# niveathika/siddhi

Hardware: AMD Instinct MI355X
Metric: events/sec ingested + matches/sec (partitioned pattern, 1–8 GPU); % HBM peak (higher is better)
Workload: dtype f64; 1 GPU; P3; events_per_gpu=100000000, keys_per_gpu=10000000, micro_batch=50000896, call_size=1024, parallelism=key-sharded x1, input=prepartitioned

## Files before the change

siddhi_amd/csrc/engine.h:

```cpp
#pragma once
#include <algorithm>
#include <cstring>
#include <memory>
#include <vector>

#include "common.h"
#include "dev_expr.h"

namespace shd {

enum EngineKind { ENG_PATTERN = 1, ENG_WINDOW = 2, ENG_FILTER = 3, ENG_NFA = 4 };

struct OutputBuffer {
  int ncols = 0;
  int64_t count = 0, cap = 0;
  DevBuf chunk, type, ts, vals, nulls, seq, sidx;
  void init(int nc) { ncols = nc; }
  void ensure(int64_t extra, hipStream_t s);
  int64_t* d_chunk() { return chunk.as<int64_t>(); }
  int32_t* d_type() { return type.as<int32_t>(); }
  int64_t* d_ts() { return ts.as<int64_t>(); }
  uint64_t* d_vals() { return vals.as<uint64_t>(); }
  uint8_t* d_nulls() { return nulls.as<uint8_t>(); }
  int64_t* d_seq() { return seq.as<int64_t>(); }
  int32_t* d_sidx() { return sidx.as<int32_t>(); }
  DevBuf lvals, lnul;
  int64_t lcount = 0, lcap = 0;
  void ensure_list(int64_t extra, hipStream_t s);
};

struct Staged {
  int stream = 0;
  int64_t n = 0;
  ColSet cs{};
  std::vector<int64_t> call_offsets;
  bool advance_time = false;
  const uint8_t* skip_start = nullptr;
};

struct SnapW {
  std::vector<uint8_t> b;
  hipStream_t s = nullptr;
  template <class T> void put(const T& v) {
    const size_t o = b.size();
    b.resize(o + sizeof(T));
    std::memcpy(b.data() + o, &v, sizeof(T));
  }
  void bytes(const void* src, size_t n) {
    const size_t o = b.size();
    b.resize(o + n);
    if (n) std::memcpy(b.data() + o, src, n);
  }
  void dev(const void* p, size_t n) {
    put<uint64_t>(n);
    const size_t o = b.size();
    b.resize(o + n);
    if (n) {
      SHD_HIP(hipMemcpyAsync(b.data() + o, p, n, hipMemcpyDeviceToHost, s));
      SHD_HIP(hipStreamSynchronize(s));
    }
  }
};

struct SnapR {
  const uint8_t* p = nullptr;
  size_t n = 0, at = 0;
  hipStream_t s = nullptr;
  void need(size_t k) const {
    if (at + k > n) throw Error(SHD_E_ARG, "snapshot truncated or from a different plan");
  }
  template <class T> T get() {
    need(sizeof(T));
    T v;
    std::memcpy(&v, p + at, sizeof(T));
    at += sizeof(T);
    return v;
  }
  size_t dev(DevBuf& buf, size_t extra_cap = 0) {
    const size_t k = (size_t)get<uint64_t>();
    need(k);
    buf.reserve(std::max<size_t>(k, extra_cap));
    if (k) {
      SHD_HIP(hipMemcpyAsync(buf.p, p + at, k, hipMemcpyHostToDevice, s));
      SHD_HIP(hipStreamSynchronize(s));
    }
    at += k;
    return k;
  }
  void dev_into(void* dst, size_t expect) {
    const size_t k = (size_t)get<uint64_t>();
    if (k != expect) throw Error(SHD_E_ARG, "snapshot section size mismatch");
    need(k);
    if (k) {
      SHD_HIP(hipMemcpyAsync(dst, p + at, k, hipMemcpyHostToDevice, s));
      SHD_HIP(hipStreamSynchronize(s));
    }
    at += k;
  }
};

struct NeedNfa : Error {
  explicit NeedNfa(const std::string& m) : Error(SHD_E_UNSUPPORTED, m) {}
};

struct NeedDissolve : NeedNfa {
  explicit NeedDissolve(const std::string& m) : NeedNfa(m) {}
};

struct Replay {
  int stream = 0;
  int64_t n = 0;
  std::vector<int64_t> ts;
  std::vector<std::vector<uint8_t>> cols, nulls;
  std::vector<uint8_t> skip_start;
};

struct Engine {
  Plan plan;
  DevExprTable ex;
  hipStream_t stream = nullptr;
  OutputBuffer out;
  shd_counters counters{};
  int64_t seq = 0;
  int64_t now = INT64_MIN;
  int64_t chunk_seq = 0;
  hipEvent_t ev0 = nullptr, ev1 = nullptr;
  static constexpr int kMaxStages = 16;
  hipEvent_t sev[kMaxStages + 1] = {};
  const char* stage_name[kMaxStages] = {};
  int n_stages = 0;
  int64_t stage_ns[kMaxStages] = {};
  void stage_begin() { n_stages = 0; mark(nullptr); }
  void mark(const char* name_of_finished_stage);
  void stage_end();

  virtual ~Engine();
  virtual int kind() const = 0;
  virtual void push(const Staged& b) = 0;
  virtual void set_time(int64_t t) {
    if (t >= now) now = t;
  }
  virtual void reset() = 0;
  int64_t start_time = 0;
  int64_t layout_hint = 0;
  virtual void set_option(const std::string& key, int64_t v) {
    if (key == "start_time") {
      start_time = v;
      if (v > now) now = v;
      return;
    }
    throw Error(SHD_E_ARG, "unknown option '" + key + "' for this query");
  }
  virtual void on_loaded() {}
  virtual void save_state(SnapW&) { throw Error(SHD_E_UNSUPPORTED, "engine has no snapshot support"); }
  virtual void load_state(SnapR&) { throw Error(SHD_E_UNSUPPORTED, "engine has no snapshot support"); }
  virtual void export_replay(std::vector<Replay>&) {
    throw Error(SHD_E_UNSUPPORTED, "engine state cannot be handed over");
  }
  bool grouped = false;
  virtual void group_attach(const std::vector<Engine*>&) {
    throw Error(SHD_E_UNSUPPORTED, "this query's engine cannot lead a query group");
  }
  virtual void group_detach() {}
  virtual void group_dissolve() { throw Error(SHD_E_UNSUPPORTED, "this group cannot dissolve"); }

  static constexpr size_t kArgArena = size_t(1) << 20;
  DevBuf arg_dev;
  PinnedBuf arg_host;
  size_t arg_used = 0;
  void args_begin() {
    if (!arg_dev.p) {
      arg_dev.reserve(kArgArena);
      arg_host.reserve(kArgArena);
    }
    SHD_HIP(hipStreamSynchronize(stream));
    arg_used = 0;
  }
  template <class T> const T* dev_args(const T& a) {
    size_t off = (arg_used + 255) & ~size_t(255);
    if (!arg_dev.p || off + sizeof(T) > kArgArena) throw Error(SHD_E_CAPACITY, "kernel argument arena exhausted");
    std::memcpy(arg_host.as<char>() + off, &a, sizeof(T));
    SHD_HIP(hipMemcpyAsync(arg_dev.as<char>() + off, arg_host.as<char>() + off, sizeof(T), hipMemcpyHostToDevice,
                           stream));
    arg_used = off + sizeof(T);
    return reinterpret_cast<const T*>(arg_dev.as<char>() + off);
  }

  template <class... P, class... A>
  void launch_grid(void (*kernel)(P...), unsigned grid, A&&... args) {
    kernel<<<dim3(grid), dim3(kBlock), 0, stream>>>(std::forward<A>(args)...);
    SHD_CHECK_LAUNCH();
  }
  template <class... P, class... A>
  void launch(void (*kernel)(P...), int64_t n, A&&... args) {
    launch_grid(kernel, grid_cover(n), std::forward<A>(args)...);
  }

  uint32_t read_u32(const void* dev, uint32_t* pinned) {
    SHD_HIP(hipMemcpyAsync(pinned, dev, 4, hipMemcpyDeviceToHost, stream));
    SHD_HIP(hipStreamSynchronize(stream));
    return *pinned;
  }
  uint32_t scan(const uint32_t* in, uint32_t* outp, int64_t n, uint32_t* total_dev, uint32_t* total_pinned,
                DevBuf& scratch) {
    if (n <= 0) return 0;
    scan_exclusive_u32(in, outp, n, total_dev, scratch, stream);
    return read_u32(total_dev, total_pinned);
  }

  DExpr dexpr(int e) const { return DExpr{ex.off[e], ex.len[e]}; }
  DExprSet dset() const { return DExprSet{ex.ins.as<int4>(), ex.consts.as<uint64_t>(), ex.nins, ex.nconsts}; }
  DFilters dfilters(const std::vector<int>& ids) const;
  bool fast_atom(int expr_id, FAtom& out) const;
};

std::unique_ptr<Engine> make_pattern_engine(const Plan& p, std::string& why);
std::unique_ptr<Engine> make_logical_pattern_engine(const Plan& p, std::string& why);
std::unique_ptr<Engine> make_absent_engine(const Plan& p, std::string& why);
std::unique_ptr<Engine> make_single_engine(const Plan& p, std::string& why);
std::unique_ptr<Engine> make_window_x_engine(const Plan& p, std::string& why);
std::unique_ptr<Engine> make_nfa_engine(const Plan& p, std::string& why);
std::unique_ptr<Engine> make_nfa_engine(const Plan& p, std::string& why, int64_t list_hint);
void init_engine(Engine& e, const Plan& p);

}
```

siddhi_amd/csrc/engine_pattern.hip:

```cpp
#include <algorithm>
#include <unordered_map>
#include <cmath>
#include <cstdio>
#include <cstdlib>
#include <type_traits>

#include "engine.h"
#include "knobs.h"
#include "pattern_common.h"

namespace shd {

using namespace pat;

namespace {

template <bool FAST>
__global__ __launch_bounds__(kBlock) void k_prepare(const PrepArgs* __restrict__ ap, int64_t n_ext, int64_t stride,
                                                    uint32_t* __restrict__ k32, uint64_t* __restrict__ k64,
                                                    uint32_t* __restrict__ pv, int32_t* __restrict__ tso,
                                                    PrepAgg* __restrict__ blk) {
  const PrepArgs& a = *ap;
  const DExprSet es = a.es;
  PrepAcc acc;
  const int64_t tbase = a.x.batch.ts[0];
  for (int64_t r = (int64_t)blockIdx.x * kBlock + threadIdx.x; r < n_ext; r += stride) {
    uint64_t k;
    uint32_t f;
    int32_t t32;
    prep_row<FAST>(a, es, r, tbase, true, k, f, t32, acc);
    if (a.partitioned) {
      if (a.key64) k64[r] = k;
      else k32[r] = (uint32_t)k;
    }
    pv[r] = (f << kRowBits) | (uint32_t)r;
    tso[r] = t32;
  }
  prep_block_reduce<kBlock>(acc, blk, blockIdx.x);
}

__global__ __launch_bounds__(kBlock) void k_finish_prep(const PrepAgg* blk, int nblk, PrepAgg* out) {
  unsigned long long c = 0, km = 0, ov = 0, um = 0, kn = ULLONG_MAX;
  long long tmin = LLONG_MAX, tmax = LLONG_MIN, ctm = LLONG_MIN;
#pragma unroll 8
  for (int b = threadIdx.x; b < nblk; b += kBlock) {
    ov |= blk[b].ovf;
    um |= blk[b].unmono;
    kn = blk[b].kmin < kn ? blk[b].kmin : kn;
    ctm = blk[b].carry_tmax > ctm ? blk[b].carry_tmax : ctm;
    c += blk[b].n_cand;
    km = blk[b].kmax > km ? blk[b].kmax : km;
    tmin = blk[b].ts_min < tmin ? blk[b].ts_min : tmin;
    tmax = blk[b].ts_max > tmax ? blk[b].ts_max : tmax;
  }
  for (int o = 32; o > 0; o >>= 1) {
    c += __shfl_xor(c, o, 64);
    ov |= __shfl_xor(ov, o, 64);
    um |= __shfl_xor(um, o, 64);
  }
  km = wave_max(km);
  kn = wave_min(kn);
  tmin = wave_min(tmin);
  tmax = wave_max(tmax);
  ctm = wave_max(ctm);
  __shared__ PrepAgg wpart[kBlock / 64];
  if ((threadIdx.x & 63) == 0) wpart[threadIdx.x >> 6] = PrepAgg{c, km, tmin, tmax, ov, um, ctm, kn};
  __syncthreads();
  if (threadIdx.x == 0) {
    PrepAgg r = wpart[0];
    for (int w = 1; w < kBlock / 64; w++) {
      r.ovf |= wpart[w].ovf;
      r.unmono |= wpart[w].unmono;
      r.carry_tmax = wpart[w].carry_tmax > r.carry_tmax ? wpart[w].carry_tmax : r.carry_tmax;
      r.kmin = wpart[w].kmin < r.kmin ? wpart[w].kmin : r.kmin;
      r.n_cand += wpart[w].n_cand;
      r.kmax = wpart[w].kmax > r.kmax ? wpart[w].kmax : r.kmax;
      r.ts_min = wpart[w].ts_min < r.ts_min ? wpart[w].ts_min : r.ts_min;
      r.ts_max = wpart[w].ts_max > r.ts_max ? wpart[w].ts_max : r.ts_max;
    }
    *out = r;
  }
}

__global__ void k_narrow_keys(const uint64_t* in, uint32_t* out, int64_t n) {
  for (int64_t i = (int64_t)blockIdx.x * blockDim.x + threadIdx.x; i < n; i += (int64_t)gridDim.x * blockDim.x)
    out[i] = (uint32_t)in[i];
}

__global__ __launch_bounds__(kBlock) void k_sorted_ts64(const ExtRows* __restrict__ xp,
                                                        const uint32_t* __restrict__ spv, int64_t n,
                                                        int64_t* __restrict__ sts64) {
  const ExtRows& x = *xp;
  for (int64_t p = (int64_t)blockIdx.x * kBlock + threadIdx.x; p < n; p = n) sts64[p] = x.ts(pv_row(spv[p]));
}

__global__ __launch_bounds__(kBlock) void k_slice_coarsen(const ExtRows* __restrict__ xp,
                                                          const int64_t* __restrict__ slice_t, int64_t nslice,
                                                          int cbits, int32_t* __restrict__ ctab) {
  const int64_t tbase = xp->batch.ts[0];
  const int e = (int)blockIdx.x * kBlock + threadIdx.x;
  if (e >= kScanCoarse) return;
  const int64_t per = (int64_t)1 << (cbits - kKsSliceBits);
  const int64_t s0 = e * per, s1 = s0 + per < nslice ? s0 + per : nslice;
  int64_t lo = LLONG_MAX, hi = LLONG_MIN;
  for (int64_t i = s0; i < s1; i++) {
    const int64_t l = slice_t[i], h = slice_t[nslice + i];
    lo = l < lo ? l : lo;
    hi = h > hi ? h : hi;
  }
  ctab[e] = lo == LLONG_MAX ? INT32_MAX : (int32_t)(lo - tbase);
  ctab[kScanCoarse + e] = hi == LLONG_MIN ? INT32_MIN : (int32_t)(hi - tbase);
}

__global__ __launch_bounds__(kBlock) void k_sorted_ts32(const ExtRows* __restrict__ xp,
                                                        const uint32_t* __restrict__ spv, int64_t n,
                                                        int32_t* __restrict__ sts32) {
  const ExtRows& x = *xp;
  const int64_t tbase = x.batch.ts[0];
  for (int64_t p = (int64_t)blockIdx.x * kBlock + threadIdx.x; p < n; p = n)
    sts32[p] = (int32_t)(x.ts(pv_row(spv[p])) - tbase);
}

#include "pattern_walk.h"

__device__ __forceinline__ void scan_block_reduce(uint64_t steps, uint64_t pruned, uint32_t viol, uint32_t nm,
                                                  uint32_t no, ScanOut* blk, int slot, uint32_t* bcnt, int tile,
                                                  int ntile, bool add, uint32_t nd = 0) {
  for (int o2 = 32; o2 > 0; o2 >>= 1) {
    steps += __shfl_xor(steps, o2, 64);
    pruned += __shfl_xor(pruned, o2, 64);
    viol |= __shfl_xor(viol, o2, 64);
    nm += __shfl_xor(nm, o2, 64);
    no += __shfl_xor(no, o2, 64);
    nd += __shfl_xor(nd, o2, 64);
  }
  __shared__ ScanOut wpart[kBlock / 64];
  __shared__ uint32_t wcnt[3][kBlock / 64];
  if ((threadIdx.x & 63) == 0) {
    wpart[threadIdx.x >> 6] = ScanOut{steps, pruned, viol};
    wcnt[0][threadIdx.x >> 6] = nm;
    wcnt[1][threadIdx.x >> 6] = no;
    wcnt[2][threadIdx.x >> 6] = nd;
  }
  __syncthreads();
  if (threadIdx.x == 0) {
    ScanOut r = wpart[0];
    uint32_t tm = wcnt[0][0], to = wcnt[1][0], td = wcnt[2][0];
    for (int w = 1; w < kBlock / 64; w++) {
      r.steps += wpart[w].steps;
      r.pruned += wpart[w].pruned;
      r.violation |= wpart[w].violation;
      tm += wcnt[0][w];
      to += wcnt[1][w];
      td += wcnt[2][w];
    }
    blk[slot] = r;
    if (add) {
      if (tm) atomicAdd(&bcnt[tile], tm);
      if (to) atomicAdd(&bcnt[ntile + tile], to);
    } else {
      bcnt[tile] = tm;
      bcnt[ntile + tile] = to;
      bcnt[2 * ntile + tile] = td;
    }
  }
}

__device__ __forceinline__ void and_carried(const ScanArgs& a, int64_t r, uint32_t& fm, int64_t& ra, int64_t& rb) {
  fm = 0;
  ra = rb = -1;
  if (r < a.x.C) {
    fm = a.carry_half[r];
    const int64_t hr = a.x.C + a.x.batch.n + r;
    if (fm & 1u) ra = hr;
    if (fm & 2u) rb = hr;
  }
}
__device__ __forceinline__ int32_t and_code(uint32_t fm, int64_t ra, int64_t rb) {
  return fm == 0 ? 0 : (int32_t)((fm & 1u ? ra : rb) | ((int64_t)fm << kRowBits));
}
__device__ __forceinline__ int32_t and_open_code(const ScanArgs& a, int64_t r) {
  uint32_t fm;
  int64_t ra, rb;
  and_carried(a, r, fm, ra, rb);
  return and_code(fm, ra, rb);
}

template <bool K64, bool TS64, bool HASH>
__global__ __launch_bounds__(kBlock) void k_forward_scan(const ScanArgs* __restrict__ ap, int64_t n_ext,
                                                         int64_t tile, const uint32_t* __restrict__ skey32,
                                                         const uint64_t* __restrict__ skey64,
                                                         const uint32_t* __restrict__ spv,
                                                         const int32_t* __restrict__ sts32,
                                                         const int64_t* __restrict__ sts64,
                                                         int32_t* __restrict__ match_row, uint8_t* __restrict__ pst,
                                                         uint32_t* __restrict__ bcnt, ScanOut* __restrict__ blk) {
  const ScanArgs& a = *ap;
  const DExprSet es{};
  uint64_t steps = 0, pruned = 0;
  uint32_t viol = 0, nm = 0, no = 0, nd = 0;
  const int64_t t0 = (int64_t)blockIdx.x * tile;
  const int64_t t1 = t0 + tile < n_ext ? t0 + tile : n_ext;
  const int64_t tbase = TS64 ? 0 : a.x.batch.ts[0];
  auto visit = [&](int64_t p, const auto& ld) {
    uint32_t pvp, pq;
    int64_t tsi, tq;
    uint64_t k = 0, kq = 0;
    const int64_t q0 = p + 1 < n_ext ? p + 1 : n_ext - 1;
    ld(p, pvp, tsi, k);
    ld(q0, pq, tq, kq);
    uint8_t out = PS_NONE;
    if (pv_flags(pvp) & F_CAND) {
      int64_t q = p + 1;
      int32_t j = -1;
      uint32_t fm = 0;
      int64_t ra = -1, rb = -1;
      const uint8_t st = walk_partial<true, false, HASH ? 4 : 1>(a, es, n_ext, ld, pv_row(pvp), k, tsi, q, pq, tq,
                                                                 kq, tsi, false, j, steps, viol, fm, ra, rb);
      if (st == ST_DEFER) {
        out = PS_DEFER;
        match_row[p] = (int32_t)q;
        nd++;
      } else if (st == ST_OPEN) {
        out = PS_OPEN;
        no++;
        if (a.logical == 2) match_row[p] = and_open_code(a, pv_row(pvp));
      } else if (st == ST_PRUNED) {
        pruned++;
      }
    }
    pst[p] = out;
  };
  const GlobalPos<K64, TS64> ld{skey32, skey64, spv, sts32, sts64, tbase, a.partitioned};
  for (int64_t p = t0 + threadIdx.x; p < t1; p += kBlock) visit(p, ld);
  scan_block_reduce(steps, pruned, viol, nm, no, blk, blockIdx.x, bcnt, blockIdx.x, gridDim.x, false, nd);
}

constexpr int kSubPerTile = kBlock / 64;
constexpr uint32_t kRecDeferred = 0x80000000u;

constexpr int kRecRing = 128;
__device__ __forceinline__ void wave_lds_order() {
  __builtin_amdgcn_fence(__ATOMIC_RELEASE, "wavefront");
  __builtin_amdgcn_wave_barrier();
  __builtin_amdgcn_fence(__ATOMIC_ACQUIRE, "wavefront");
}
template <bool LEAN>
__global__ __launch_bounds__(kBlock) void k_forward_scan_rec(const ScanArgs* __restrict__ ap, int64_t n_ext,
                                                             int64_t tile, const uint32_t* __restrict__ skey32,
                                                             const uint32_t* __restrict__ spv,
                                                             const int32_t* __restrict__ sts32,
                                                             int32_t* __restrict__ match_row, uint8_t* __restrict__ pst,
                                                             uint32_t* __restrict__ bcnt, ScanOut* __restrict__ blk,
                                                             uint32_t* __restrict__ rkey, uint32_t* __restrict__ rpv,
                                                             int32_t* __restrict__ rts, uint32_t* __restrict__ rpos,
                                                             uint32_t* __restrict__ dlist, uint32_t* __restrict__ scnt) {
  const ScanArgs& a = *ap;
  const DExprSet es{};
  uint64_t steps = 0, pruned = 0;
  uint32_t viol = 0, no = 0, nd = 0;
  const int lane = threadIdx.x & 63, w = threadIdx.x >> 6;
  const int64_t sub = tile / kSubPerTile;
  const int64_t t0 = (int64_t)blockIdx.x * tile;
  const int64_t t1 = t0 + tile < n_ext ? t0 + tile : n_ext;
  const int64_t s0 = t0 + (int64_t)w * sub;
  const int64_t s1 = s0 + sub < t1 ? s0 + sub : t1;
  const int64_t tbase = a.x.batch.ts[0];
  const GlobalPos<false, false> ld{skey32, nullptr, spv, sts32, nullptr, tbase, a.partitioned};
  const RowPos ldr{skey32, spv, a.x.carry.ts, a.x.batch.ts, a.x.C, a.partitioned};
  __shared__ int32_t ctab[LEAN ? 2 * kScanCoarse : 1];
  if constexpr (LEAN) {
    const int nc = (int)((n_ext - 1) >> a.cbits) + 1;
    for (int i = threadIdx.x; i < nc; i += kBlock) {
      ctab[i] = a.ctab[i];
      ctab[kScanCoarse + i] = a.ctab[kScanCoarse + i];
    }
    __syncthreads();
  }
  constexpr int kRecPos = LEAN ? 2 : 3;
  const uint64_t below = ((uint64_t)1 << lane) - 1;
  uint32_t wrec = 0, wdef = 0;
  uint32_t wout = 0;
  __shared__ uint32_t ring[kSubPerTile][LEAN ? 3 : 4][kRecRing];
  uint32_t (*rg)[kRecRing] = ring[w];
  auto flush = [&](uint32_t cnt) {
    wave_lds_order();
    if ((uint32_t)lane < cnt) {
      const uint32_t sl = (wout + (uint32_t)lane) & (kRecRing - 1);
      const int64_t o = s0 + wout + lane;
      rkey[o] = rg[0][sl];
      rpv[o] = rg[1][sl];
      if constexpr (!LEAN) rts[o] = (int32_t)rg[2][sl];
      rpos[o] = rg[kRecPos][sl];
    }
    wave_lds_order();
  };
  for (int64_t c = s0; c < s1; c += 64) {
    const int64_t p = c + lane;
    uint8_t out = PS_NONE;
    uint32_t pvp = 0;
    int64_t tsi = 0;
    uint64_t k = 0;
    if (p < s1) {
      uint32_t pq;
      int64_t tq;
      uint64_t kq = 0;
      const int64_t q0 = p + 1 < n_ext ? p + 1 : n_ext - 1;
      if constexpr (LEAN) {
        pvp = spv[p];
        pq = spv[q0];
        k = skey32[p];
        kq = skey32[q0];
      } else {
        ld(p, pvp, tsi, k);
        ld(q0, pq, tq, kq);
      }
      if (pv_flags(pvp) & F_CAND) {
        int64_t q = p + 1;
        int32_t j = -1;
        uint32_t fm = 0;
        int64_t ra = -1, rb = -1;
        uint8_t st;
        if constexpr (LEAN) {
          const uint32_t fq = pv_flags(pq);
          const int64_t ri = pv_row(pvp), rq = pv_row(pq);
          if (q >= n_ext || (kq != k && !(fq & F_SKIP))) {
            st = ST_OPEN;
          } else {
            bool dead = false;
            if (kq == k && (fq & F_NEW) && !(fq & F_SKIP)) {
              const int64_t hi = ri >= a.x.C ? tbase + ctab[kScanCoarse + (ri >> a.cbits)] : a.carry_tmax;
              const int64_t lo = tbase + ctab[rq >> a.cbits];
              dead = lo > hi && (uint64_t)lo - (uint64_t)hi > (uint64_t)a.within;
            }
            if (dead) {
              st = ST_DEAD;
              steps++;
            } else {
              tsi = ldr.row_ts(ri);
              tq = ldr.row_ts(rq);
              st = walk_partial<true, false, 1>(a, es, n_ext, ldr, ri, k, tsi, q, pq, tq, kq, tsi, false, j, steps,
                                                viol, fm, ra, rb);
            }
          }
        } else {
          st = walk_partial<true, false, 1>(a, es, n_ext, ld, pv_row(pvp), k, tsi, q, pq, tq, kq, tsi, false, j, steps,
                                            viol, fm, ra, rb);
        }
        if (st == ST_DEFER) {
          out = PS_DEFER;
          match_row[p] = (int32_t)q;
          nd++;
        } else if (st == ST_OPEN) {
          out = PS_OPEN;
          no++;
        } else if (st == ST_PRUNED) {
          pruned++;
        }
      }
      pst[p] = out;
    }
    const bool def = out == PS_DEFER, rec = def || out == PS_OPEN;
    const uint64_t mrec = __ballot(rec), mdef = __ballot(def);
    if (rec) {
      const uint32_t sl = (wrec + (uint32_t)__popcll(mrec & below)) & (kRecRing - 1);
      rg[0][sl] = (uint32_t)k;
      rg[1][sl] = pvp;
      if constexpr (!LEAN) rg[2][sl] = (uint32_t)(int32_t)(tsi - tbase);
      rg[kRecPos][sl] = (uint32_t)p | (def ? kRecDeferred : 0u);
    }
    if (def) dlist[s0 + wdef + __popcll(mdef & below)] = (uint32_t)p;
    wrec += (uint32_t)__popcll(mrec);
    wdef += (uint32_t)__popcll(mdef);
    if (wrec - wout >= 64) {
      flush(64);
      wout += 64;
    }
  }
  if (wrec > wout) flush(wrec - wout);
  if (lane == 0) {
    const int64_t nsub = (int64_t)gridDim.x * kSubPerTile;
    const int64_t st = (int64_t)blockIdx.x * kSubPerTile + w;
    scnt[st] = wrec - wdef;
    scnt[nsub + st] = wdef;
    scnt[2 * nsub + st] = wrec;
  }
  scan_block_reduce(steps, pruned, viol, 0u, no, blk, blockIdx.x, bcnt, blockIdx.x, gridDim.x, false, nd);
}

__global__ __launch_bounds__(kBlock) void k_gather_bpos(const ExtRows* __restrict__ xp, const uint32_t* spv,
                                                       int64_t n_ext) {
  const ExtRows& x = *xp;
  for (int64_t p = (int64_t)blockIdx.x * kBlock + threadIdx.x; p < n_ext; p += (int64_t)gridDim.x * kBlock) {
    const int64_t r = pv_row(spv[p]);
    const uint32_t m = r < x.C ? x.apos_mask : (x.bpos_mask | x.apos_mask);
    for (int c = 0; c < x.batch.ncols; c++) {
      if (!((m >> c) & 1u)) continue;
      const Val v = r < x.C ? col_load(x.carry, r, c) : col_load(x.batch, r - x.C, c);
      switch (x.bpos.type[c]) {
        case SHD_T_STRING: case SHD_T_INT: case SHD_T_FLOAT: ((uint32_t*)x.bpos.col[c])[p] = (uint32_t)v.b; break;
        case SHD_T_LONG: case SHD_T_DOUBLE: ((uint64_t*)x.bpos.col[c])[p] = v.b; break;
        case SHD_T_BOOL: ((uint8_t*)x.bpos.col[c])[p] = (uint8_t)v.b; break;
      }
      ((uint8_t*)x.bpos.nul[c])[p] = (uint8_t)v.null;
    }
  }
}

__global__ __launch_bounds__(kBlock) void k_block_sum(const ScanArgs* __restrict__ ap, int64_t n_ext,
                                                     const uint32_t* __restrict__ skey32,
                                                     const uint32_t* __restrict__ spv,
                                                     const int32_t* __restrict__ sts32, BlockSum* __restrict__ out) {
  const ScanArgs& a = *ap;
  const ExtRows& x = a.x;
  const int lane = threadIdx.x & 63;
  const int64_t nblk = (n_ext + 63) >> 6;
  const int64_t tbase = x.batch.ts[0];
  const int attr = a.bs_attr;
  const bool usemax = a.bs_op == SHD_OP_GT || a.bs_op == SHD_OP_GE;
  for (int64_t b = ((int64_t)blockIdx.x * kBlock + threadIdx.x) >> 6; b < nblk;
       b += ((int64_t)gridDim.x * kBlock) >> 6) {
    const int64_t p = (b << 6) + lane;
    const bool valid = p < n_ext;
    const uint32_t pv = valid ? spv[p] : 0u;
    const int64_t t = valid ? tbase + (int64_t)sts32[p] : 0;
    const uint32_t key = (valid && a.partitioned) ? skey32[p] : 0u;
    const uint32_t f = pv_flags(pv);
    const bool keyed = valid && !(f & F_SKIP);
    const bool nw = keyed && (f & F_NEW);
    double dv = usemax ? -__builtin_inf() : __builtin_inf();
    if (nw && (f & F_B)) {
      const int64_t r = pv_row(pv);
      const Val v = ((x.bpos_mask >> attr) & 1u) ? col_load(x.bpos, p, attr)
                    : (r < x.C ? col_load(x.carry, r, attr) : col_load(x.batch, r - x.C, attr));
      if (!v.null) {
        const double d = v_f64(v.b);
        if (d == d) dv = d;
      }
    }
    dv = usemax ? wave_max(dv) : wave_min(dv);
    const uint64_t km = __ballot(keyed), nm = __ballot(nw);
    const uint32_t k0 = km ? __shfl(key, __ffsll((unsigned long long)km) - 1, 64) : 0u;
    const bool uniform = __ballot(keyed && key != k0) == 0;
    int64_t m = nw ? t : INT64_MIN;
#pragma unroll
    for (int o = 1; o < 64; o <<= 1) {
      const int64_t u = __shfl_up(m, o, 64);
      if (lane >= o) m = u > m ? u : m;
    }
    int64_t before = __shfl_up(m, 1, 64);
    if (lane == 0) before = INT64_MIN;
    const bool mono = __ballot(nw && t < before) == 0;
    const int64_t tfirst = nm ? __shfl(t, __ffsll((unsigned long long)nm) - 1, 64) : 0;
    const int64_t tlast = __shfl(m, 63, 64);
    if (lane == 0) {
      BlockSum o;
      o.key = k0;
      o.cnt = (uint16_t)__popcll(nm);
      o.flags = (uint8_t)((uniform ? 1u : 0u) | (mono ? 2u : 0u) | (km ? 0u : 4u));
      o.pad = 0;
      o.tfirst = tfirst;
      o.tlast = tlast;
      o.v = dv;
      o.newmask = nm;
      out[b] = o;
    }
  }
}

static bool block_skip_term(const FPred& fp, int s2, int& ci, int& side, int& op, int& attr) {
  auto is_e2 = [&](const FTerm& t) {
    return t.aop == 0 && t.a.kind == FA_LOAD && t.a.st == s2 && (t.a.idx == 0 || t.a.idx == SHD_IDX_CURRENT) &&
           t.a.cvt_to < 0;
  };
  auto no_e2 = [&](const FTerm& t) {
    auto ok = [&](const FAtom& x) { return x.kind != FA_LOAD || x.st == 0; };
    return ok(t.a) && (t.aop == 0 || ok(t.b));
  };
  auto flip = [](int o) {
    return o == SHD_OP_GT ? SHD_OP_LT : o == SHD_OP_LT ? SHD_OP_GT : o == SHD_OP_GE ? SHD_OP_LE : SHD_OP_GE;
  };
  for (int i = 0; i < fp.n && i < 4; i++) {
    const FCmp& c = fp.c[i];
    if (c.type != SHD_T_DOUBLE) continue;
    if (c.op != SHD_OP_GT && c.op != SHD_OP_GE && c.op != SHD_OP_LT && c.op != SHD_OP_LE) continue;
    if (is_e2(c.l) && no_e2(c.r)) {
      ci = i, side = 0, op = c.op, attr = c.l.a.attr;
      return true;
    }
    if (is_e2(c.r) && no_e2(c.l)) {
      ci = i, side = 1, op = flip(c.op), attr = c.r.a.attr;
      return true;
    }
  }
  return false;
}

static bool split_f2(const FPred& fp, int s2, const ExtRows& x, F2Split& sp) {
  sp = F2Split{};
  if (!fp.ok || fp.n > kSplitMax) return false;
  auto e2dep = [&](const FAtom& t) { return t.kind == FA_LOAD && t.st == s2; };
  auto dep = [&](const FTerm& t) { return e2dep(t.a) || (t.aop != 0 && e2dep(t.b)); };
  for (int i = 0; i < fp.n; i++) {
    const FCmp& c = fp.c[i];
    SplitCmp& o = sp.c[i];
    o.op = c.op;
    o.type = c.type;
    const bool dl = dep(c.l), dr = dep(c.r);
    if (!dl && !dr) {
      o.konst = 1;
      continue;
    }
    if (dl && dr) return false;
    const FTerm& e = dl ? c.l : c.r;
    if (e.aop != 0 || (e.a.idx != 0 && e.a.idx != SHD_IDX_CURRENT)) return false;
    const int attr = e.a.attr;
    if (attr < 0 || attr >= x.batch.ncols || attr >= kMaxCols) return false;
    o.swap = dr ? 1 : 0;
    o.pos = (x.bpos_mask >> attr) & 1u;
    const ColSet& cs = o.pos ? x.bpos : x.batch;
    o.col = cs.col[attr];
    o.nul = cs.nul[attr];
    o.ctype = cs.type[attr];
    o.cvt_from = e.a.cvt_from;
    o.cvt_to = e.a.cvt_to;
    const bool cvt = o.cvt_to >= 0 && o.cvt_to != o.cvt_from;
    const bool rel = c.op == SHD_OP_EQ || c.op == SHD_OP_NE || c.op == SHD_OP_GT || c.op == SHD_OP_GE ||
                     c.op == SHD_OP_LT || c.op == SHD_OP_LE;
    o.kind = SK_GENERIC;
    if (rel && c.type == SHD_T_DOUBLE && o.ctype == SHD_T_FLOAT && cvt && o.cvt_from == SHD_T_FLOAT &&
        o.cvt_to == SHD_T_DOUBLE)
      o.kind = SK_F32_F64;
    else if (rel && c.type == SHD_T_DOUBLE && o.ctype == SHD_T_DOUBLE && !cvt)
      o.kind = SK_F64;
    else if ((c.op == SHD_OP_EQ || c.op == SHD_OP_NE) && c.type == SHD_T_STRING && o.ctype == SHD_T_STRING && !cvt)
      o.kind = SK_STR_EQ;
    else if (rel && c.type == SHD_T_INT && o.ctype == SHD_T_INT && !cvt)
      o.kind = SK_I32;
    if (o.kind != SK_GENERIC && o.swap) {
      switch (c.op) {
        case SHD_OP_GT: o.op = SHD_OP_LT; break;
        case SHD_OP_GE: o.op = SHD_OP_LE; break;
        case SHD_OP_LT: o.op = SHD_OP_GT; break;
        case SHD_OP_LE: o.op = SHD_OP_GE; break;
      }
    }
  }
  sp.n = fp.n;
  sp.ok = 1;
  return true;
}

template <bool FAST, bool SKIP, class Ld>
__device__ __forceinline__ void coop_resume(const ScanArgs& a, const DExprSet& es, int64_t n_ext, const Ld& ld,
                                            int64_t p, bool cont, int32_t* __restrict__ match_row,
                                            int32_t* __restrict__ match_other, uint8_t* __restrict__ pst,
                                            uint64_t& steps, uint64_t& pruned,
                                            uint32_t& viol, uint32_t& nm, uint32_t& no) {
  const int lane = threadIdx.x & 63;
  uint32_t pvp, pd;
  int64_t tsi, td;
  uint64_t k = 0, kd = 0;
  ld(p, pvp, tsi, k);
  int64_t q0 = match_row[p];
  ld(cont ? q0 - 1 : q0, pd, td, kd);
  const int64_t r = pv_row(pvp);
  int64_t prev = td;
  if (cont && (!(pv_flags(pd) & F_NEW) || (pv_flags(pd) & F_SKIP) || (a.partitioned && kd != k))) prev = tsi;
  bool first = !cont;
  uint8_t st = ST_OPEN;
  int32_t j = -1;
  uint32_t fm = 0;
  int64_t ra = -1, rb = -1;
  int32_t other = -1;
  if (a.logical == 2) and_carried(a, r, fm, ra, rb);
  SplitThr sth;
  if (FAST && a.sp.ok && !a.logical) sth = split_prep(a, r, p);
  uint64_t wsteps = 0;
  bool wviol = false;
  bool thr_ok = false;
  Val thr;
  thr.b = 0;
  thr.null = 1;
  while (q0 < n_ext) {
    if (SKIP && !first && (q0 & 63) == 0 && q0 + 64 <= n_ext) {
      if (!thr_ok) {
        thr = skip_threshold(a, r, p);
        thr_ok = true;
      }
      const BlockSum bs = a.bsum[q0 >> 6];
      if (block_skippable(a, bs, k, tsi, prev, thr)) {
        wsteps += bs.cnt;
        if (bs.cnt) prev = bs.tlast;
        q0 += 64;
        continue;
      }
    }
    const int64_t qend = SKIP ? ((q0 | 63) + 1) : q0 + 64;
    const int64_t q = q0 + lane;
    const bool act = q < qend;
    const bool inb = act && q < n_ext;
    uint32_t pq = 0;
    int64_t tq = 0;
    uint64_t kq = 0;
    if (inb) ld(q, pq, tq, kq);
    const uint32_t fq = pv_flags(pq);
    const bool f0 = first && lane == 0;
    const bool skip = (fq & F_SKIP) != 0;
    const bool endkey = inb && !f0 && a.partitioned && kq != k && !skip;
    const bool isnew = inb && !f0 && !endkey && (fq & F_NEW) && !skip;
    int64_t m = isnew ? tq : INT64_MIN;
#pragma unroll
    for (int o = 1; o < 64; o <<= 1) {
      const int64_t t = __shfl_up(m, o, 64);
      if (lane >= o) m = t > m ? t : m;
    }
    int64_t before = __shfl_up(m, 1, 64);
    if (lane == 0) before = INT64_MIN;
    before = before > prev ? before : prev;
    const bool vio = isnew && a.within != INT64_MAX && tq < before;
    const bool expire = isnew && !vio && tq - tsi > a.within;
    const uint64_t stopm = __ballot(act && (!inb || endkey || vio || expire));
    const int sidx = stopm ? __ffsll((unsigned long long)stopm) - 1 : 64;
    bool hit = false;
    int32_t code = 0;
    if (a.logical == 2) {
      const bool cand = lane < sidx && (f0 || (isnew && (fq & F_B)));
      const int64_t r2 = pv_row(pq);
      bool ha = false, hb = false;
      if (cand && !(fm & 1u)) {
        PairCtx cx{&a.x, r, r2, a.s_first};
        cx.q2 = q;
        cx.q1 = p;
        ha = FAST ? eval_fpred(a.f2.fp, cx) : eval_filters(es, a.f2, cx);
      }
      if (cand && !(fm & 2u)) {
        PairCtx cx{&a.x, r, r2, a.s_second};
        cx.q2 = q;
        cx.q1 = p;
        hb = FAST ? eval_fpred(a.f3.fp, cx) : eval_filters(es, a.f3, cx);
      }
      const uint64_t am = __ballot(ha), bm = __ballot(hb);
      int ia = (fm & 1u) ? -1 : (am ? __ffsll((unsigned long long)am) - 1 : 64);
      int ib = (fm & 2u) ? -1 : (bm ? __ffsll((unsigned long long)bm) - 1 : 64);
      if (ia >= 0 && ia < 64) {
        fm |= 1u;
        ra = __shfl(r2, ia, 64);
      }
      if (ib >= 0 && ib < 64) {
        fm |= 2u;
        rb = __shfl(r2, ib, 64);
      }
      const int term2 = fm == 3u ? (ia > ib ? ia : ib) : sidx;
      const uint64_t upto2 = term2 >= 63 ? ~0ull : ((2ull << term2) - 1ull);
      wsteps += (uint64_t)__popcll(__ballot(isnew && !vio) & upto2);
      if (fm == 3u) {
        const int br = ib >= ia ? 1 : 0;
        st = ST_MATCH;
        j = (int32_t)__shfl(r2, term2, 64) | (br << kRowBits);
        other = (int32_t)(br ? ra : rb);
        break;
      }
      if (sidx < 64) {
        const int kind = __shfl(vio ? 2 : (expire ? 1 : 0), sidx, 64);
        if (kind == 2) wviol = true;
        else if (kind == 1) st = ST_DEAD;
        break;
      }
      prev = __shfl(m, 63, 64) > prev ? __shfl(m, 63, 64) : prev;
      first = false;
      q0 = qend;
      continue;
    }
    if (lane < sidx && (f0 || (isnew && (fq & F_B)))) {
      const int64_t r2 = pv_row(pq);
      PairCtx cx{&a.x, r, r2, a.s_first};
      cx.q2 = q;
      cx.q1 = p;
      if (FAST && a.sp.ok && !a.logical) hit = split_eval(a.sp, sth, r2 - a.x.C, q);
      else hit = FAST ? eval_fpred(a.f2.fp, cx) : eval_filters(es, a.f2, cx);
      int32_t br = 0;
      if (!hit && a.logical) {
        cx.s2 = a.s_second;
        hit = FAST ? eval_fpred(a.f3.fp, cx) : eval_filters(es, a.f3, cx);
        br = 1;
      }
      code = (int32_t)r2 | (br << kRowBits);
    }
    const uint64_t hm = __ballot(hit);
    const int fidx = hm ? __ffsll((unsigned long long)hm) - 1 : 64;
    const int term = fidx < sidx ? fidx : sidx;
    const uint64_t upto = term >= 63 ? ~0ull : ((2ull << term) - 1ull);
    wsteps += (uint64_t)__popcll(__ballot(isnew && !vio) & upto);
    if (fidx < sidx) {
      st = ST_MATCH;
      j = __shfl(code, fidx, 64);
      break;
    }
    if (sidx < 64) {
      const int kind = __shfl(vio ? 2 : (expire ? 1 : 0), sidx, 64);
      if (kind == 2) wviol = true;
      else if (kind == 1) st = ST_DEAD;
      break;
    }
    prev = __shfl(m, 63, 64) > prev ? __shfl(m, 63, 64) : prev;
    first = false;
    q0 = qend;
  }
  if (st == ST_OPEN && a.prune && a.t_end - tsi > a.within) st = ST_PRUNED;
  if (lane == 0) {
    steps += wsteps;
    if (wviol) viol = 1;
    uint8_t out = PS_NONE;
    if (st == ST_MATCH) {
      out = PS_MATCH;
      match_row[p] = j;
      if (a.logical == 2) match_other[p] = other;
      nm++;
    } else if (st == ST_OPEN) {
      out = PS_OPEN | PS_PEND;
      no++;
      if (a.logical == 2) match_row[p] = and_code(fm, ra, rb);
    } else if (st == ST_PRUNED) {
      pruned++;
    }
    pst[p] = out;
  }
}

template <bool K64, bool FAST, bool TS64, int MODE, bool SKIP = false>
__global__ __launch_bounds__(kBlock) void k_forward_resume(const ScanArgs* __restrict__ ap, int64_t n_ext,
                                                           int64_t tile, const uint32_t* __restrict__ skey32,
                                                           const uint64_t* __restrict__ skey64,
                                                           const uint32_t* __restrict__ spv,
                                                           const int32_t* __restrict__ sts32,
                                                           const int64_t* __restrict__ sts64,
                                                           int32_t* __restrict__ match_row,
                                                           int32_t* __restrict__ match_other,
                                                           uint8_t* __restrict__ pst, uint32_t* __restrict__ bcnt,
                                                           ScanOut* __restrict__ blk, int slot0) {
  const ScanArgs& a = *ap;
  const DExprSet es = a.es;
  uint64_t steps = 0, pruned = 0;
  uint32_t viol = 0, nm = 0, no = 0;
  const int64_t t0 = (int64_t)blockIdx.x * tile;
  const int64_t t1 = t0 + tile < n_ext ? t0 + tile : n_ext;
  const int64_t tbase = TS64 ? 0 : a.x.batch.ts[0];
  const GlobalPos<K64, TS64> ld{skey32, skey64, spv, sts32, sts64, tbase, a.partitioned};
  auto resume_one = [&](int64_t p) {
      int64_t q = match_row[p];
      uint32_t pvp, pq;
      int64_t tsi, tq;
      uint64_t k = 0, kq = 0;
      ld(p, pvp, tsi, k);
      ld(q, pq, tq, kq);
      int32_t j = -1;
      uint32_t fm = 0;
      int64_t ra = -1, rb = -1;
      if (a.logical == 2) and_carried(a, pv_row(pvp), fm, ra, rb);
      const uint8_t st = walk_partial<false, FAST, 1, GlobalPos<K64, TS64>, 0, SKIP>(a, es, n_ext, ld, pv_row(pvp), k, tsi, q, pq, tq, kq, tq, true,
                                                      j, steps, viol, fm, ra, rb, p);
      uint8_t out = PS_NONE;
      if (st == ST_MATCH) {
        out = PS_MATCH;
        match_row[p] = j;
        if (a.logical == 2) match_other[p] = (int32_t)((j >> kRowBits) ? ra : rb);
        nm++;
      } else if (st == ST_OPEN) {
        out = PS_OPEN | PS_PEND;
        no++;
        if (a.logical == 2) match_row[p] = and_code(fm, ra, rb);
      } else if (st == ST_PRUNED) {
        pruned++;
      }
      pst[p] = out;
  };
  if constexpr (MODE == 2) {
    const int lane = threadIdx.x & 63, w = threadIdx.x >> 6;
    for (int64_t base = t0 + (int64_t)w * 64; base < t1; base += kBlock) {
      const int64_t pp = base + lane;
      const uint8_t o = pp < t1 ? pst[pp] : (uint8_t)PS_NONE;
      uint64_t dm = __ballot(o == PS_DEFER || o == PS_CONT);
      const uint64_t cm = __ballot(o == PS_CONT);
      while (dm) {
        const int b = __ffsll((unsigned long long)dm) - 1;
        dm &= dm - 1;
        coop_resume<FAST, SKIP>(a, es, n_ext, ld, base + b, (cm >> b) & 1ull, match_row, match_other, pst, steps, pruned,
                          viol, nm, no);
      }
    }
  } else if constexpr (MODE == 3) {
    for (int64_t p = t0 + threadIdx.x; p < t1; p += kBlock) {
      if (pst[p] != PS_DEFER) continue;
      int64_t q = match_row[p];
      uint32_t pvp, pq;
      int64_t tsi, tq;
      uint64_t k = 0, kq = 0;
      ld(p, pvp, tsi, k);
      ld(q, pq, tq, kq);
      int32_t j = -1;
      uint32_t fm = 0;
      int64_t ra = -1, rb = -1;
      const uint8_t st = walk_partial<false, FAST, 1, GlobalPos<K64, TS64>, 64, SKIP>(
          a, es, n_ext, ld, pv_row(pvp), k, tsi, q, pq, tq, kq, tq, true, j, steps, viol, fm, ra, rb, p);
      uint8_t out = PS_NONE;
      if (st == ST_MATCH) {
        out = PS_MATCH;
        match_row[p] = j;
        nm++;
      } else if (st == ST_OPEN) {
        out = PS_OPEN | PS_PEND;
        no++;
      } else if (st == ST_PRUNED) {
        pruned++;
      } else if (st == ST_YIELD) {
        out = PS_CONT;
        match_row[p] = (int32_t)q;
      }
      pst[p] = out;
    }
  } else if constexpr (MODE == 1) {
    for (int64_t p = t0 + threadIdx.x; p < t1; p += kBlock)
      if (pst[p] == PS_DEFER) resume_one(p);
  } else {
    for (int64_t c0 = t0; c0 < t1; c0 += kBlock * 16) {
      const int64_t pb = c0 + (int64_t)threadIdx.x * 16;
      if (pb >= t1) continue;
      const uint4 raw = *reinterpret_cast<const uint4*>(pst + pb);
      const uint32_t wv[4] = {raw.x, raw.y, raw.z, raw.w};
      uint32_t hit = 0;
#pragma unroll
      for (int i = 0; i < 16; i++)
        if (((wv[i >> 2] >> ((i & 3) * 8)) & 255u) == PS_DEFER && pb + i < t1) hit |= 1u << i;
      while (hit) {
        const int64_t p = pb + __ffs(hit) - 1;
        hit &= hit - 1;
        resume_one(p);
      }
    }
  }
  scan_block_reduce(steps, pruned, viol, nm, no, blk, slot0 + blockIdx.x, bcnt, blockIdx.x, gridDim.x, true);
}

template <bool K64, bool FAST, bool TS64, bool SUB = false, bool ROWT = false>
__global__ __launch_bounds__(kBlock) void k_resume_list(const ScanArgs* __restrict__ ap, int64_t n_ext, int64_t tile,
                                                        int ntile, const uint32_t* __restrict__ skey32,
                                                        const uint64_t* __restrict__ skey64,
                                                        const uint32_t* __restrict__ spv,
                                                        const int32_t* __restrict__ sts32,
                                                        const int64_t* __restrict__ sts64,
                                                        int32_t* __restrict__ match_row,
                                                        int32_t* __restrict__ match_other, uint8_t* __restrict__ pst,
                                                        uint32_t* __restrict__ bcnt, ScanOut* __restrict__ blk,
                                                        int slot0, const uint32_t* __restrict__ dlist,
                                                        const uint32_t* __restrict__ dcount,
                                                        const uint32_t* __restrict__ doff, int nsub, int64_t sub,
                                                        uint32_t* __restrict__ sopen) {
  const ScanArgs& a = *ap;
  const DExprSet es = a.es;
  uint64_t steps = 0, pruned = 0;
  uint32_t viol = 0;
  const int64_t tbase = (TS64 || ROWT) ? 0 : a.x.batch.ts[0];
  typedef typename std::conditional<ROWT, RowPos, GlobalPos<K64, TS64>>::type Ld;
  const Ld ld = [&] {
    if constexpr (ROWT) return RowPos{skey32, spv, a.x.carry.ts, a.x.batch.ts, a.x.C, a.partitioned};
    else return GlobalPos<K64, TS64>{skey32, skey64, spv, sts32, sts64, tbase, a.partitioned};
  }();
  const int64_t cnt = *dcount;
  for (int64_t i = (int64_t)blockIdx.x * kBlock + threadIdx.x; i < cnt; i += (int64_t)gridDim.x * kBlock) {
    int sti = 0;
    int64_t p;
    if (SUB) {
      int lo = 0, hi = nsub;
      while (lo < hi) {
        const int mid = (lo + hi) >> 1;
        if ((int64_t)doff[mid] <= i) lo = mid + 1; else hi = mid;
      }
      sti = lo - 1;
      p = dlist[(int64_t)sti * sub + (i - (int64_t)doff[sti])];
    } else {
      p = dlist[i];
    }
    int64_t q = match_row[p];
    uint32_t pvp, pq;
    int64_t tsi, tq;
    uint64_t k = 0, kq = 0;
    ld(p, pvp, tsi, k);
    ld(q, pq, tq, kq);
    int32_t j = -1;
    uint32_t fm = 0;
    int64_t ra = -1, rb = -1;
    if (a.logical == 2) and_carried(a, pv_row(pvp), fm, ra, rb);
    const uint8_t st = walk_partial<false, FAST, 1, Ld, 0, false>(
        a, es, n_ext, ld, pv_row(pvp), k, tsi, q, pq, tq, kq, tq, true, j, steps, viol, fm, ra, rb, p);
    uint8_t out = PS_NONE;
    const int t = (int)(p / tile);
    if (st == ST_MATCH) {
      out = PS_MATCH;
      match_row[p] = j;
      if (a.logical == 2) match_other[p] = (int32_t)((j >> kRowBits) ? ra : rb);
      atomicAdd(&bcnt[t], 1u);
    } else if (st == ST_OPEN) {
      out = PS_OPEN | PS_PEND;
      if (a.logical == 2) match_row[p] = and_code(fm, ra, rb);
      if (SUB) atomicAdd(&sopen[sti], 1u);
      else atomicAdd(&bcnt[ntile + t], 1u);
    } else if (st == ST_PRUNED) {
      pruned++;
    }
    pst[p] = out;
  }
  scan_block_reduce(steps, pruned, viol, 0u, 0u, blk, slot0 + blockIdx.x, bcnt, 0, ntile, true);
}

template <bool TS64>
__global__ __launch_bounds__(kBlock, 8) void k_lockstep_walk(const ScanArgs* __restrict__ ap, int64_t n_ext, int64_t tile,
                                                          const uint32_t* __restrict__ skey32,
                                                          const uint32_t* __restrict__ spv,
                                                          const int32_t* __restrict__ sts32,
                                                          const int64_t* __restrict__ sts64,
                                                          int32_t* __restrict__ match_row, uint8_t* __restrict__ pst,
                                                          uint32_t* __restrict__ bcnt, ScanOut* __restrict__ blk) {
  const ScanArgs& a = *ap;
  uint64_t steps = 0, pruned = 0;
  uint32_t viol = 0, nm = 0, no = 0;
  const int64_t t0 = (int64_t)blockIdx.x * tile;
  const int64_t t1 = t0 + tile < n_ext ? t0 + tile : n_ext;
  const int64_t tbase = TS64 ? 0 : a.x.batch.ts[0];
  const GlobalPos<false, TS64> ld{skey32, nullptr, spv, sts32, sts64, tbase, a.partitioned};
  for (int64_t p = t0 + threadIdx.x; p < t1; p += kBlock) {
    uint32_t pvp;
    int64_t tsi;
    uint64_t k = 0;
    ld(p, pvp, tsi, k);
    uint8_t out = PS_NONE;
    if (pv_flags(pvp) & F_CAND) {
      const int64_t r = pv_row(pvp);
      uint8_t st = ST_OPEN;
      bool metb = false;
      SplitThr sth;
      if (a.sp.ok) sth = split_prep(a, r, p);
      int32_t j = -1;
      int64_t prev = tsi;
      int64_t q = p + 1;
      uint32_t pn = 0;
      int64_t tn = 0;
      uint64_t kn = 0;
      if (q < n_ext) ld(q, pn, tn, kn);
      for (int d = 0; q < n_ext; q++, d++) {
        if (d >= 64 && metb) {
          st = ST_YIELD;
          break;
        }
        const uint32_t pq = pn;
        const int64_t tq = tn;
        const uint64_t kq = kn;
        if (q + 1 < n_ext) ld(q + 1, pn, tn, kn);
        const uint32_t fq = pv_flags(pq);
        if (fq & F_SKIP) continue;
        if (kq != k) break;
        if (!(fq & F_NEW)) continue;
        if (a.within != INT64_MAX && tq < prev) {
          viol = 1;
          break;
        }
        prev = tq;
        steps++;
        if (tq - tsi > a.within) {
          st = ST_DEAD;
          break;
        }
        if (fq & F_B) {
          bool hit;
          if (a.sp.ok) {
            hit = split_eval(a.sp, sth, (int64_t)pv_row(pq) - a.x.C, q);
          } else {
            PairCtx cx{&a.x, r, (int64_t)pv_row(pq), a.s_first};
            cx.q2 = q;
            cx.q1 = p;
            hit = eval_fpred(a.f2.fp, cx);
          }
          metb = true;
          if (hit) {
            st = ST_MATCH;
            j = (int32_t)pv_row(pq);
            break;
          }
        }
      }
      if (st == ST_OPEN && a.prune && a.t_end - tsi > a.within) st = ST_PRUNED;
      if (st == ST_MATCH) {
        out = PS_MATCH;
        match_row[p] = j;
        nm++;
      } else if (st == ST_OPEN) {
        out = metb ? (uint8_t)(PS_OPEN | PS_PEND) : (uint8_t)PS_OPEN;
        no++;
      } else if (st == ST_PRUNED) {
        pruned++;
      } else if (st == ST_YIELD) {
        out = PS_CONT;
        match_row[p] = (int32_t)q;
      }
    }
    pst[p] = out;
  }
  scan_block_reduce(steps, pruned, viol, nm, no, blk, blockIdx.x, bcnt, blockIdx.x, gridDim.x, false);
}

__global__ __launch_bounds__(kBlock) void k_tile_count(const uint8_t* __restrict__ pst, int64_t n, int64_t tile,
                                                       uint32_t* __restrict__ bcnt) {
  const int64_t t0 = (int64_t)blockIdx.x * tile;
  const int64_t t1 = t0 + tile < n ? t0 + tile : n;
  uint32_t nm = 0, no = 0;
  for (int64_t pb = t0 + (int64_t)threadIdx.x * 16; pb < t1; pb += kBlock * 16) {
    const uint4 raw = *reinterpret_cast<const uint4*>(pst + pb);
    const uint32_t wv[4] = {raw.x, raw.y, raw.z, raw.w};
#pragma unroll
    for (int i = 0; i < 16; i++) {
      const uint32_t o = (wv[i >> 2] >> ((i & 3) * 8)) & 255u;
      const bool in = pb + i < t1;
      nm += (in && o == PS_MATCH) ? 1u : 0u;
      no += (in && (o & 0x7Fu) == PS_OPEN) ? 1u : 0u;
    }
  }
  for (int o = 32; o > 0; o >>= 1) {
    nm += __shfl_xor(nm, o, 64);
    no += __shfl_xor(no, o, 64);
  }
  __shared__ uint32_t ws[2][kBlock / 64];
  if ((threadIdx.x & 63) == 0) {
    ws[0][threadIdx.x >> 6] = nm;
    ws[1][threadIdx.x >> 6] = no;
  }
  __syncthreads();
  if (threadIdx.x == 0) {
    uint32_t a = 0, b = 0;
    for (int k = 0; k < kBlock / 64; k++) {
      a += ws[0][k];
      b += ws[1][k];
    }
    bcnt[blockIdx.x] = a;
    bcnt[gridDim.x + blockIdx.x] = b;
  }
}

constexpr int kCompactPad = kBlock * 16;
template <class F>
__device__ __forceinline__ void tile_compact(const uint8_t* __restrict__ pst, int64_t t0, int64_t t1, uint8_t want,
                                             uint32_t base, F&& emit) {
  __shared__ uint32_t wsum[kBlock / 64];
  const int lane = threadIdx.x & 63, w = threadIdx.x >> 6;
  for (int64_t c0 = t0; c0 < t1; c0 += kBlock * 16) {
    const int64_t pb = c0 + (int64_t)threadIdx.x * 16;
    uint32_t wv[4] = {0u, 0u, 0u, 0u};
    if (pb < t1) {
      const uint4 raw = *reinterpret_cast<const uint4*>(pst + pb);
      wv[0] = raw.x;
      wv[1] = raw.y;
      wv[2] = raw.z;
      wv[3] = raw.w;
    }
    uint32_t hit = 0;
#pragma unroll
    for (int i = 0; i < 16; i++)
      if (((wv[i >> 2] >> ((i & 3) * 8)) & 127u) == want && pb + i < t1) hit |= 1u << i;
    const uint32_t cnt = (uint32_t)__popc(hit);
    uint32_t inc = cnt;
#pragma unroll
    for (int o = 1; o < 64; o <<= 1) {
      const uint32_t t = __shfl_up(inc, o, 64);
      if (lane >= o) inc += t;
    }
    if (lane == 63) wsum[w] = inc;
    __syncthreads();
    uint32_t pre = base + inc - cnt, tot = 0;
#pragma unroll
    for (int k = 0; k < kBlock / 64; k++) {
      if (k < w) pre += wsum[k];
      tot += wsum[k];
    }
    while (hit) {
      const int i = __ffs(hit) - 1;
      hit &= hit - 1;
      emit(pb + i, pre++);
    }
    base += tot;
    __syncthreads();
  }
}

__global__ __launch_bounds__(kBlock) void k_finish_scan(const ScanOut* blk, int nblk, ScanOut* out) {
  unsigned long long st = 0, pr = 0;
  uint32_t v = 0;
#pragma unroll 8
  for (int b = threadIdx.x; b < nblk; b += kBlock) {
    st += blk[b].steps;
    pr += blk[b].pruned;
    v |= blk[b].violation;
  }
  for (int o = 32; o > 0; o >>= 1) {
    st += __shfl_xor(st, o, 64);
    pr += __shfl_xor(pr, o, 64);
    v |= __shfl_xor(v, o, 64);
  }
  __shared__ ScanOut wpart[kBlock / 64];
  if ((threadIdx.x & 63) == 0) wpart[threadIdx.x >> 6] = ScanOut{st, pr, v};
  __syncthreads();
  if (threadIdx.x == 0) {
    ScanOut r = wpart[0];
    for (int w = 1; w < kBlock / 64; w++) {
      r.steps += wpart[w].steps;
      r.pruned += wpart[w].pruned;
      r.violation |= wpart[w].violation;
    }
    *out = r;
  }
}

__global__ __launch_bounds__(kBlock) void k_emit_pairs(const uint8_t* pst, const uint32_t* boff,
                                                       const int32_t* match_row, const uint32_t* spv, int64_t n,
                                                       int64_t tile, int logical, const int32_t* match_other,
                                                       uint32_t* pj, uint32_t* pi, uint32_t* se1, int32_t* sot) {
  const int64_t t0 = (int64_t)blockIdx.x * tile;
  const int64_t t1 = t0 + tile < n ? t0 + tile : n;
  tile_compact(pst, t0, t1, PS_MATCH, boff[blockIdx.x], [&](int64_t p, uint32_t o) {
    const uint32_t mr = (uint32_t)match_row[p];
    pj[o] = logical ? ((mr & kRowMask) << 1) | (mr >> kRowBits) : mr;
    if (logical == 2) {
      pi[o] = o;
      se1[o] = pv_row(spv[p]);
      sot[o] = match_other[p];
      return;
    }
    pi[o] = pv_row(spv[p]);
  });
}

struct ProjArgs {
  ExtRows x;
  DExprSet es;
  DExpr outs[kMaxCols];
  int nout;
  int multi;
  int logical;
  int s_first, s_second;
  const uint32_t* se1;
  const int32_t* sot;
  int64_t chunk0;
  int64_t row0;
  int fast;
  FAtom oat[kMaxCols];
};

__global__ __launch_bounds__(kBlock) void k_project(const ProjArgs* __restrict__ ap, const uint32_t* pj,
                                                    const uint32_t* pi, int64_t m, int64_t* o_chunk, int32_t* o_type,
                                                    int64_t* o_ts, uint64_t* o_vals, uint8_t* o_nul, int64_t* o_seq,
                                                    int32_t* o_sidx) {
  const ProjArgs& a = *ap;
  const DExprSet es = a.es;
  const ExtRows& x = a.x;
  for (int64_t k = (int64_t)blockIdx.x * kBlock + threadIdx.x; k < m; k = m) {
    int64_t j = pj[k], i = pi[k];
    int br = 0;
    if (a.logical) {
      br = (int)(j & 1);
      j >>= 1;
    }
    int64_t other = -1;
    if (a.logical == 2) {
      other = a.sot[i];
      i = a.se1[i];
    }
    PairCtx cx{&x, i, j, br ? a.s_second : a.s_first, true, other, br ? a.s_first : a.s_second};
    int64_t row = a.row0 + k;
    for (int c = 0; c < a.nout; c++) {
      const Val v = a.fast ? fp_atom(a.oat[c], cx) : eval_expr(es.ins + a.outs[c].off, a.outs[c].len, es.consts, cx);
      o_vals[row * a.nout + c] = v.b;
      o_nul[row * a.nout + c] = (uint8_t)v.null;
    }
    o_ts[row] = x.ts(j);
    o_type[row] = 0;
    o_seq[row] = x.seq(j);
    o_sidx[row] = br ? a.s_second : a.s_first;
    o_chunk[row] = a.logical ? 2 * x.seq(j) + br : (a.multi ? x.seq(j) : a.chunk0 + k);
  }
}

constexpr int kGroupMax = 64;
constexpr int kGroupWaveItems = 8;

struct GroupSelArgs {
  ExtRows x;
  int G;
  DExprSet es[kGroupMax];
  DFilters f1[kGroupMax];
};

__global__ __launch_bounds__(kBlock) void k_group_mask(const GroupSelArgs* __restrict__ ap, const uint32_t* pi,
                                                       int64_t m, uint64_t* __restrict__ mask) {
  const GroupSelArgs& a = *ap;
  for (int64_t k = (int64_t)blockIdx.x * kBlock + threadIdx.x; k < m; k = m) {
    PairCtx cx{&a.x, (int64_t)pi[k], -1, 1, false, -1, -1};
    uint64_t b = 0;
    for (int g = 0; g < a.G; g++)
      if (eval_filters(a.es[g], a.f1[g], cx)) b |= 1ull << g;
    mask[k] = b;
  }
}

template <bool SCATTER>
__global__ __launch_bounds__(kBlock) void k_group_split(const uint64_t* __restrict__ mask, const uint32_t* pj,
                                                        const uint32_t* pi, int64_t m, int G, int64_t nw,
                                                        uint32_t* __restrict__ cnt, uint32_t* __restrict__ gpj,
                                                        uint32_t* __restrict__ gpi) {
  const int lane = threadIdx.x & 63;
  const int64_t w = ((int64_t)blockIdx.x * kBlock + threadIdx.x) >> 6;
  if (w >= nw) return;
  const uint64_t below = (1ull << lane) - 1ull;
  uint64_t mk[kGroupWaveItems];
  uint32_t vj[kGroupWaveItems], vi[kGroupWaveItems];
  for (int s = 0; s < kGroupWaveItems; s++) {
    const int64_t k = w * (64 * kGroupWaveItems) + s * 64 + lane;
    mk[s] = k < m ? mask[k] : 0ull;
    if (SCATTER) {
      vj[s] = k < m ? pj[k] : 0u;
      vi[s] = k < m ? pi[k] : 0u;
    }
  }
  for (int g = 0; g < G; g++) {
    uint32_t base = SCATTER ? cnt[(int64_t)g * nw + w] : 0u;
    for (int s = 0; s < kGroupWaveItems; s++) {
      const bool on = (mk[s] >> g) & 1ull;
      const uint64_t bal = __ballot(on);
      if (SCATTER && on) {
        const uint32_t pos = base + (uint32_t)__popcll(bal & below);
        gpj[pos] = vj[s];
        gpi[pos] = vi[s];
      }
      base += (uint32_t)__popcll(bal);
    }
    if (!SCATTER && lane == 0) cnt[(int64_t)g * nw + w] = base;
  }
}

__global__ void k_group_bases(const uint32_t* __restrict__ off, const uint32_t* __restrict__ cnt, int G, int64_t nw,
                              uint32_t* __restrict__ bases) {
  const int g = threadIdx.x;
  if (g < G) bases[g] = off[(int64_t)g * nw];
  if (g == G) bases[G] = off[(int64_t)G * nw - 1] + cnt[(int64_t)G * nw - 1];
}

struct GatherArgs {
  ExtRows x;
  int ncols;
  int partitioned;
  int key64;
  int32_t types[kMaxCols];
  void* dcol[kMaxCols];
  uint8_t* dnul[kMaxCols];
  int64_t* dts;
  uint64_t* dkey;
  int64_t* dseq;
  uint32_t amask;
  const int32_t* sts32;
  const int64_t* sts64;
  int key_attr;
  uint8_t* dpend;
  const uint8_t* pend_old;
  int and_mode;
  const int32_t* match_row;
  uint8_t* dhalf;
  int ncolsB;
  int32_t typesB[kMaxCols];
  void* dcolB[kMaxCols];
  uint8_t* dnulB[kMaxCols];
  int64_t* dtsB;
  int64_t* dseqB;
};

__device__ __forceinline__ void store_col(void* dst, int type, int64_t o, uint64_t b) {
  switch (type) {
    case SHD_T_STRING: case SHD_T_INT: case SHD_T_FLOAT: ((uint32_t*)dst)[o] = (uint32_t)b; break;
    case SHD_T_LONG: case SHD_T_DOUBLE: ((uint64_t*)dst)[o] = b; break;
    case SHD_T_BOOL: ((uint8_t*)dst)[o] = (uint8_t)b; break;
  }
}

__global__ __launch_bounds__(kBlock) void k_gather_carry(const GatherArgs* __restrict__ ap, const uint8_t* pst,
                                                         const uint32_t* boff, const uint32_t* spv,
                                                         const uint32_t* skey32, const uint64_t* skey64, int64_t n,
                                                         int64_t tile) {
  const GatherArgs& a = *ap;
  const ExtRows& x = a.x;
  const int64_t t0 = (int64_t)blockIdx.x * tile;
  const int64_t t1 = t0 + tile < n ? t0 + tile : n;
  tile_compact(pst, t0, t1, PS_OPEN, boff[gridDim.x + blockIdx.x], [&](int64_t p, uint32_t o32) {
    const int64_t o = o32;
    int64_t r = pv_row(spv[p]);
    const ColSet& cs = x.cs(r);
    int64_t row = x.row(r);
    for (int c = 0; c < a.ncols; c++) {
      Val v = col_load(cs, row, c);
      switch (a.types[c]) {
        case SHD_T_STRING: case SHD_T_INT: case SHD_T_FLOAT: ((uint32_t*)a.dcol[c])[o] = (uint32_t)v.b; break;
        case SHD_T_LONG: case SHD_T_DOUBLE: ((uint64_t*)a.dcol[c])[o] = v.b; break;
        case SHD_T_BOOL: ((uint8_t*)a.dcol[c])[o] = (uint8_t)v.b; break;
      }
      a.dnul[c][o] = (uint8_t)v.null;
    }
    a.dts[o] = x.ts(r);
    a.dkey[o] = !a.partitioned ? 0 : (a.key64 ? skey64[p] : (uint64_t)skey32[p]);
    a.dseq[o] = x.seq(r);
    a.dpend[o] = (uint8_t)(((pst[p] & PS_PEND) || (r < x.C && a.pend_old[r])) ? 1 : 0);
    if (a.and_mode) {
      const uint32_t mr = (uint32_t)a.match_row[p];
      const uint32_t fm = mr >> kRowBits;
      a.dhalf[o] = (uint8_t)fm;
      if (fm) {
        const int64_t hr = mr & kRowMask;
        const ColSet& hc = x.cs(hr);
        const int64_t hrow = x.row(hr);
        for (int c = 0; c < a.ncolsB; c++) {
          const Val v = col_load(hc, hrow, c);
          store_col(a.dcolB[c], a.typesB[c], o, v.b);
          a.dnulB[c][o] = (uint8_t)v.null;
        }
        a.dtsB[o] = x.ts(hr);
        a.dseqB[o] = x.seq(hr);
      }
    }
  });
}

__global__ __launch_bounds__(kBlock) void k_open_list(const uint8_t* __restrict__ pst, const uint32_t* __restrict__ boff,
                                                      int64_t n, int64_t tile, uint32_t* __restrict__ olist,
                                                      uint32_t val, int which) {
  const int64_t t0 = (int64_t)blockIdx.x * tile;
  const int64_t t1 = t0 + tile < n ? t0 + tile : n;
  constexpr int kOlU = 4;
  constexpr int kW = kBlock / 64;
  constexpr int kChunk = 4 * kBlock;
  __shared__ uint32_t wsum[kOlU][kW];
  const int lane = threadIdx.x & 63, w = threadIdx.x >> 6;
  uint32_t base = boff[which * gridDim.x + blockIdx.x];
  for (int64_t c0 = t0; c0 < t1; c0 += kOlU * kChunk) {
    uint32_t word[kOlU];
#pragma unroll
    for (int u = 0; u < kOlU; u++) {
      const int64_t p = c0 + u * kChunk + 4 * threadIdx.x;
      word[u] = p < t1 ? *reinterpret_cast<const uint32_t*>(pst + p) : 0u;
    }
    uint32_t hm[kOlU], ex[kOlU];
#pragma unroll
    for (int u = 0; u < kOlU; u++) {
      const int64_t p = c0 + u * kChunk + 4 * threadIdx.x;
      uint32_t m = 0;
#pragma unroll
      for (int b = 0; b < 4; b++)
        m |= ((((word[u] >> (8 * b)) & 0x7Fu) == val) && p + b < t1 ? 1u : 0u) << b;
      hm[u] = m;
      const uint32_t c = (uint32_t)__popc(m);
      uint32_t inc = c;
#pragma unroll
      for (int o = 1; o < 64; o <<= 1) {
        const uint32_t t = __shfl_up(inc, o, 64);
        if (lane >= o) inc += t;
      }
      ex[u] = inc - c;
      if (lane == 63) wsum[u][w] = inc;
    }
    __syncthreads();
#pragma unroll
    for (int u = 0; u < kOlU; u++) {
      uint32_t pre = 0, tot = 0;
#pragma unroll
      for (int k = 0; k < kW; k++) {
        pre += k < w ? wsum[u][k] : 0u;
        tot += wsum[u][k];
      }
      uint32_t o = base + pre + ex[u];
      const uint32_t p = (uint32_t)(c0 + u * kChunk + 4 * threadIdx.x);
#pragma unroll
      for (int b = 0; b < 4; b++)
        if ((hm[u] >> b) & 1u) olist[o++] = p + (uint32_t)b;
      base += tot;
    }
    __syncthreads();
  }
}

__device__ __forceinline__ void gather_open_row(const GatherArgs& a, int64_t o, int64_t r, uint64_t kk, bool sts,
                                                bool pend_now) {
  const ExtRows& x = a.x;
  if (r < x.C) {
    for (int c = 0; c < a.ncols; c++) {
      if (!((a.amask >> c) & 1u)) continue;
      if (c == a.key_attr) {
        store_col(a.dcol[c], a.types[c], o, kk);
        a.dnul[c][o] = 0;
        continue;
      }
      const Val v = col_load(x.carry, r, c);
      store_col(a.dcol[c], a.types[c], o, v.b);
      a.dnul[c][o] = (uint8_t)v.null;
    }
    if (!sts) a.dts[o] = gld(x.carry.ts, r);
    a.dseq[o] = x.carry_seq[r];
  } else {
    const int64_t br = r - x.C;
    for (int c = 0; c < a.ncols; c++) {
      if (!((a.amask >> c) & 1u)) continue;
      if (c == a.key_attr) {
        store_col(a.dcol[c], a.types[c], o, kk);
        a.dnul[c][o] = 0;
        continue;
      }
      const Val v = col_load(x.batch, br, c);
      store_col(a.dcol[c], a.types[c], o, v.b);
      a.dnul[c][o] = (uint8_t)v.null;
    }
    if (!sts) a.dts[o] = gld(x.batch.ts, br);
    a.dseq[o] = x.seq0 + br;
  }
  a.dkey[o] = kk;
  a.dpend[o] = (uint8_t)((pend_now || (r < x.C && a.pend_old[r])) ? 1 : 0);
}

__global__ __launch_bounds__(kBlock) void k_gather_list(const GatherArgs* __restrict__ ap,
                                                        const uint32_t* __restrict__ olist, int64_t n_open,
                                                        const uint8_t* __restrict__ pst,
                                                        const uint32_t* __restrict__ spv,
                                                        const uint32_t* __restrict__ skey32,
                                                        const uint64_t* __restrict__ skey64) {
  const GatherArgs& a = *ap;
  const ExtRows& x = a.x;
  for (int64_t oi = (int64_t)blockIdx.x * kBlock + threadIdx.x; oi < n_open; oi = n_open) {
    const int64_t p = olist[oi];
    const int64_t o = oi;
    const int64_t r = pv_row(spv[p]);
    const uint64_t kk = !a.partitioned ? 0 : (a.key64 ? skey64[p] : (uint64_t)skey32[p]);
    const bool sts = a.sts32 || a.sts64;
    gather_open_row(a, o, r, kk, sts, (pst[p] & PS_PEND) != 0);
    if (sts) a.dts[o] = a.sts64 ? a.sts64[p] : gld(x.batch.ts, 0) + (int64_t)a.sts32[p];
  }
}

template <bool LEAN>
__global__ __launch_bounds__(kBlock) void k_gather_rec(const GatherArgs* __restrict__ ap, int64_t sub, int nsub,
                                                       const uint32_t* __restrict__ rkey,
                                                       const uint32_t* __restrict__ rpv,
                                                       const int32_t* __restrict__ rts,
                                                       const uint32_t* __restrict__ rpos,
                                                       const uint32_t* __restrict__ scnt,
                                                       const uint32_t* __restrict__ soff,
                                                       const uint8_t* __restrict__ pst) {
  const GatherArgs& a = *ap;
  const int lane = threadIdx.x & 63;
  const int st = (int)blockIdx.x * kSubPerTile + (threadIdx.x >> 6);
  const int64_t base = (int64_t)st * sub;
  const uint32_t nrec = scnt[2 * (int64_t)nsub + st];
  const int64_t tbase = LEAN ? 0 : gld(a.x.batch.ts, 0);
  const uint64_t below = ((uint64_t)1 << lane) - 1;
  int64_t o0 = soff[st];
  for (uint32_t i0 = 0; i0 < nrec; i0 += 64) {
    const uint32_t i = i0 + lane;
    bool valid = false, pend = false;
    if (i < nrec) {
      const uint32_t rp = rpos[base + i];
      valid = true;
      if (rp & kRecDeferred) {
        const uint8_t ps = pst[rp & ~kRecDeferred];
        valid = (ps & 0x7Fu) == PS_OPEN;
        pend = (ps & PS_PEND) != 0;
      }
    }
    const uint64_t mv = __ballot(valid);
    if (valid) {
      const int64_t o = o0 + __popcll(mv & below);
      gather_open_row(a, o, pv_row(rpv[base + i]), a.partitioned ? (uint64_t)rkey[base + i] : 0, !LEAN, pend);
      if constexpr (!LEAN) a.dts[o] = tbase + (int64_t)rts[base + i];
    }
    o0 += __popcll(mv);
  }
}

struct CarryTable {
  DevBuf col[kMaxCols], nul[kMaxCols], ts, key, seq;
  DevBuf pend;
  DevBuf half, bcol[kMaxCols], bnul[kMaxCols], bts, bseq;
  void reserve_b(int64_t n, const std::vector<int>& types) {
    n = std::max<int64_t>(n, 1);
    half.reserve(n);
    for (size_t c = 0; c < types.size(); c++) {
      bcol[c].reserve(n * type_size(types[c]));
      bnul[c].reserve(n);
    }
    bts.reserve(n * 8);
    bseq.reserve(n * 8);
  }
  ColSet colset_b(const std::vector<int>& types, int64_t n) const {
    ColSet cs{};
    cs.ncols = (int)types.size();
    for (size_t c = 0; c < types.size(); c++) {
      cs.col[c] = bcol[c].p;
      cs.nul[c] = bnul[c].as<uint8_t>();
      cs.type[c] = (int32_t)types[c];
    }
    cs.ts = bts.as<int64_t>();
    cs.n = n;
    return cs;
  }
  void reserve(int64_t n, const std::vector<int>& types) {
    for (size_t c = 0; c < types.size(); c++) {
      col[c].reserve(std::max<int64_t>(n, 1) * type_size(types[c]));
      nul[c].reserve(std::max<int64_t>(n, 1));
    }
    ts.reserve(std::max<int64_t>(n, 1) * 8);
    key.reserve(std::max<int64_t>(n, 1) * 8);
    seq.reserve(std::max<int64_t>(n, 1) * 8);
    pend.reserve(std::max<int64_t>(n, 1));
  }
  ColSet colset(const std::vector<int>& types) const {
    ColSet cs{};
    cs.ncols = (int)types.size();
    for (size_t c = 0; c < types.size(); c++) {
      cs.col[c] = col[c].p;
      cs.nul[c] = nul[c].as<uint8_t>();
      cs.type[c] = (int32_t)types[c];
    }
    cs.ts = ts.as<int64_t>();
    return cs;
  }
};

bool expr_reads_only(const Plan& p, int e, int st) {
  for (auto& in : p.exprs[e])
    if ((in.op == SHD_OP_LOAD || in.op == SHD_OP_EVNULL || in.op == SHD_OP_TS) && in.a != st) return false;
  return true;
}

int plain_load_attr(const Plan& p, int e) {
  auto& code = p.exprs[e];
  if (code.size() == 1 && code[0].op == SHD_OP_LOAD) return code[0].c & 0xFFFF;
  return -1;
}

bool find_key_equality(const Plan& p, const std::vector<int>& filters, int& attr_a, int& attr_b, int& type) {
  for (int e : filters) {
    const auto& code = p.exprs[e];
    std::vector<int> st;
    std::vector<std::pair<int, int>> kid(code.size(), {-1, -1});
    bool ok = true;
    for (int i = 0; i < (int)code.size() && ok; i++) {
      const int op = code[i].op;
      if (op == SHD_OP_LOAD || op == SHD_OP_CONST || op == SHD_OP_NULL || op == SHD_OP_EVNULL || op == SHD_OP_TS ||
          op == SHD_OP_AGG) {
        st.push_back(i);
      } else if (op == SHD_OP_CVT || op == SHD_OP_NOT || op == SHD_OP_ISNULL) {
        if (st.empty()) ok = false;
        else { kid[i].first = st.back(); st.back() = i; }
      } else if (op >= SHD_OP_ADD && op <= SHD_OP_OR) {
        if (st.size() < 2) { ok = false; break; }
        kid[i] = {st[st.size() - 2], st.back()};
        st.pop_back();
        st.back() = i;
      } else if (op != SHD_OP_END) {
        ok = false;
      }
    }
    if (!ok || st.size() != 1) continue;
    std::vector<int> todo{st[0]};
    while (!todo.empty()) {
      const int n = todo.back();
      todo.pop_back();
      const Instr& in = code[n];
      if (in.op == SHD_OP_AND) {
        todo.push_back(kid[n].first);
        todo.push_back(kid[n].second);
        continue;
      }
      if (in.op != SHD_OP_EQ) continue;
      const Instr& l = code[kid[n].first];
      const Instr& r = code[kid[n].second];
      if (l.op != SHD_OP_LOAD || r.op != SHD_OP_LOAD) continue;
      auto cur = [](const Instr& x) { return x.b == 0 || x.b == SHD_IDX_CURRENT; };
      if (!cur(l) || !cur(r)) continue;
      const Instr& la = l.a == 0 ? l : r;
      const Instr& lb = l.a == 0 ? r : l;
      if (la.a != 0 || lb.a != 1) continue;
      const int ta = la.c >> 16, tb = lb.c >> 16;
      if (ta != tb || in.a != ta || !(ta == SHD_T_STRING || ta == SHD_T_INT || ta == SHD_T_LONG)) continue;
      attr_a = la.c & 0xFFFF;
      attr_b = lb.c & 0xFFFF;
      type = ta;
      return true;
    }
  }
  return false;
}


}

struct PatternEngine : Engine {
  int sA = 0, sB = 0;
  std::vector<int> f1, f2;
  int logical = 0;
  std::vector<int> f3;
  std::vector<int> typesB;
  bool and_indep = false;
  uint32_t bpos_mask = 0;
  uint32_t apos_mask = 0;
  DevBuf d_bpos[kMaxCols], d_bpos_nul[kMaxCols];
  DevBuf d_bsum;
  int s_first = 1, s_second = -1;
  int64_t W = INT64_MAX;
  bool partitioned = false;
  bool implicit_key = false;
  int key_expr[2] = {-1, -1}, key_col[2] = {-1, -1}, key_type[2] = {0, 0};
  std::vector<int> outs;
  std::vector<int> typesA;
  CarryTable carry[2];
  int cur = 0;
  int64_t C = 0;
  bool have_horizon = false;
  int64_t horizon = INT64_MIN;
  int64_t t_last = INT64_MIN;
  int64_t last_b_seq = -1;
  static constexpr int64_t kPruneMinRows = 1 << 16;
  DevBuf d_kps;
  DevBuf d_slice;
  DevBuf d_ctab;
  hipEvent_t ev_pg = nullptr, ev_pt = nullptr;
  const int32_t* fin_sts32 = nullptr;
  const int64_t* fin_sts64 = nullptr;
  struct ScanRecs {
    bool on = false;
    uint32_t *key = nullptr, *pv = nullptr, *pos = nullptr;
    int32_t* ts = nullptr;
    bool lean = false;
    int64_t sub = 0;
    int nsub = 0;
  } fin_rec;
  DevBuf d_k32, d_k32_alt, d_k64, d_k64_alt, d_pv, d_pv_alt, d_ts, d_ts_alt, d_ts64, d_match, d_pst, d_bcnt, d_boff, d_pj,
      d_pi, d_pj_alt, d_pi_alt, d_sort, d_scan, d_blk, d_mother, d_se1, d_sot, d_olist, d_dlist;
  uint32_t carry_mask = ~0u;
  ReadbackBlock<PatternTotals, PatternTotalsHost> agg;

  int kind() const override { return ENG_PATTERN; }

  void reset() override {
    C = 0;
    last_b_seq = -1;
    seq = 0;
    now = INT64_MIN;
    chunk_seq = 0;
    out.count = 0;
    counters = shd_counters{};
    have_horizon = false;
    horizon = INT64_MIN;
    t_last = INT64_MIN;
  }

  void export_replay(std::vector<Replay>& parts) override {
    SHD_HIP(hipStreamSynchronize(stream));
    const CarryTable& t = carry[cur];
    std::vector<int64_t> ts(C), sq(C);
    if (C > 0) {
      SHD_HIP(hipMemcpy(ts.data(), t.ts.p, C * 8, hipMemcpyDeviceToHost));
      SHD_HIP(hipMemcpy(sq.data(), t.seq.p, C * 8, hipMemcpyDeviceToHost));
    }
    auto host_cols = [&](const std::vector<int>& types, const DevBuf* dcol, const DevBuf* dnul,
                         std::vector<std::vector<uint8_t>>& col, std::vector<std::vector<uint8_t>>& nul) {
      col.assign(types.size(), {});
      nul.assign(types.size(), {});
      for (size_t c = 0; c < types.size(); c++) {
        col[c].resize((size_t)C * type_size(types[c]));
        nul[c].resize((size_t)C);
        if (C > 0) {
          SHD_HIP(hipMemcpy(col[c].data(), dcol[c].p, col[c].size(), hipMemcpyDeviceToHost));
          SHD_HIP(hipMemcpy(nul[c].data(), dnul[c].p, (size_t)C, hipMemcpyDeviceToHost));
        }
      }
    };
    std::vector<std::vector<uint8_t>> col, nul, bcol, bnul;
    host_cols(typesA, t.col, t.nul, col, nul);
    std::vector<uint8_t> half;
    std::vector<int64_t> bts, bsq;
    if (logical == 2 && C > 0) {
      half.resize(C);
      bts.resize(C);
      bsq.resize(C);
      SHD_HIP(hipMemcpy(half.data(), t.half.p, C, hipMemcpyDeviceToHost));
      SHD_HIP(hipMemcpy(bts.data(), t.bts.p, C * 8, hipMemcpyDeviceToHost));
      SHD_HIP(hipMemcpy(bsq.data(), t.bseq.p, C * 8, hipMemcpyDeviceToHost));
      host_cols(typesB, t.bcol, t.bnul, bcol, bnul);
    }
    std::vector<uint8_t> pend(C, 0);
    if (C > 0) SHD_HIP(hipMemcpy(pend.data(), t.pend.p, C, hipMemcpyDeviceToHost));
    std::vector<uint64_t> keyv(C, 0);
    if (C > 0 && partitioned) SHD_HIP(hipMemcpy(keyv.data(), t.key.p, C * 8, hipMemcpyDeviceToHost));
    struct Ev { int64_t seq; int src; int64_t i; };
    std::vector<Ev> evs;
    std::unordered_map<uint64_t, int64_t> newest;
    for (int64_t i = 0; i < C; i++) {
      if (!(partitioned || W == INT64_MAX || t_last == INT64_MIN || !(t_last - ts[i] > W))) continue;
      evs.push_back({sq[i], 0, i});
      if (!half.empty() && half[i]) evs.push_back({bsq[i], 1, i});
      const uint64_t k = partitioned ? keyv[i] : 0;
      auto it = newest.find(k);
      if (it == newest.end() || sq[i] > sq[it->second]) newest[k] = i;
    }
    for (auto& kv : newest) {
      const int64_t i = kv.second;
      const bool moved = partitioned ? pend[i] != 0 : (last_b_seq >= 0 && last_b_seq > sq[i]);
      if (moved) evs.push_back({sq[i], 2, i});
    }
    std::stable_sort(evs.begin(), evs.end(), [](const Ev& a, const Ev& b) {
      return a.seq != b.seq ? a.seq < b.seq : a.src < b.src;
    });
    parts.clear();
    for (size_t k = 0; k < evs.size(); k++) {
      const Ev& e = evs[k];
      if (k > 0 && evs[k - 1].seq == e.seq && e.src != 2) continue;
      const int stream_e = e.src == 1 ? sB : sA;
      const std::vector<int>& types = e.src == 1 ? typesB : typesA;
      const auto& cc = e.src == 1 ? bcol : col;
      const auto& nn = e.src == 1 ? bnul : nul;
      if (parts.empty() || parts.back().stream != stream_e) {
        parts.emplace_back();
        Replay& r = parts.back();
        r.stream = stream_e;
        r.cols.assign(types.size(), {});
        r.nulls.assign(types.size(), {});
      }
      Replay& r = parts.back();
      r.ts.push_back(e.src == 1 ? bts[e.i] : ts[e.i]);
      for (size_t c = 0; c < types.size(); c++) {
        const int w = type_size(types[c]);
        r.cols[c].insert(r.cols[c].end(), cc[c].begin() + e.i * w, cc[c].begin() + (e.i + 1) * w);
        r.nulls[c].push_back(nn[c][e.i]);
      }
      r.skip_start.push_back((uint8_t)e.src);
      r.n++;
    }
  }

  void save_state(SnapW& w) override {
    w.put<int64_t>(C);
    w.put<int32_t>(have_horizon ? 1 : 0);
    w.put<int64_t>(horizon);
    w.put<int64_t>(t_last);
    w.put<int64_t>(last_b_seq);
    w.put<int32_t>((int32_t)typesA.size());
    const CarryTable& t = carry[cur];
    for (size_t c = 0; c < typesA.size(); c++) {
      w.dev(t.col[c].p, (size_t)C * type_size(typesA[c]));
      w.dev(t.nul[c].p, (size_t)C);
    }
    w.dev(t.ts.p, (size_t)C * 8);
    w.dev(t.key.p, (size_t)C * 8);
    w.dev(t.seq.p, (size_t)C * 8);
    w.dev(t.pend.p, (size_t)C);
    if (logical == 2) {
      w.dev(t.half.p, (size_t)C);
      for (size_t c = 0; c < typesB.size(); c++) {
        w.dev(t.bcol[c].p, (size_t)C * type_size(typesB[c]));
        w.dev(t.bnul[c].p, (size_t)C);
      }
      w.dev(t.bts.p, (size_t)C * 8);
      w.dev(t.bseq.p, (size_t)C * 8);
    }
  }
  void load_state(SnapR& r) override {
    const int64_t c0 = r.get<int64_t>();
    have_horizon = r.get<int32_t>() != 0;
    horizon = r.get<int64_t>();
    t_last = r.get<int64_t>();
    last_b_seq = r.get<int64_t>();
    if (r.get<int32_t>() != (int32_t)typesA.size() || c0 < 0) throw Error(SHD_E_ARG, "snapshot of a different plan");
    cur = 0;
    CarryTable& t = carry[0];
    t.reserve(c0, typesA);
    for (size_t c = 0; c < typesA.size(); c++) {
      r.dev_into(t.col[c].p, (size_t)c0 * type_size(typesA[c]));
      r.dev_into(t.nul[c].p, (size_t)c0);
    }
    r.dev_into(t.ts.p, (size_t)c0 * 8);
    r.dev_into(t.key.p, (size_t)c0 * 8);
    r.dev_into(t.seq.p, (size_t)c0 * 8);
    r.dev_into(t.pend.p, (size_t)c0);
    if (logical == 2) {
      t.reserve_b(c0, typesB);
      r.dev_into(t.half.p, (size_t)c0);
      for (size_t c = 0; c < typesB.size(); c++) {
        r.dev_into(t.bcol[c].p, (size_t)c0 * type_size(typesB[c]));
        r.dev_into(t.bnul[c].p, (size_t)c0);
      }
      r.dev_into(t.bts.p, (size_t)c0 * 8);
      r.dev_into(t.bseq.p, (size_t)c0 * 8);
    }
    C = c0;
    counters.carry = C;
  }

  ColSet carry_cs() const {
    ColSet cs = carry[cur].colset(typesA);
    cs.n = C;
    return cs;
  }

  static bool type_key64(int t) { return t == SHD_T_LONG || t == SHD_T_DOUBLE || t == SHD_T_FLOAT; }

  int hashed_bucket_bits(const PrepAgg& pg, int64_t n_ext, int key_bits, bool prune) const {
    if (knob_on(Knob::NO_HASH)) return 0;
    if (!prune || pg.unmono || (C > 0 && pg.carry_tmax > pg.ts_min) || pg.ts_max < pg.ts_min) return 0;
    if (int b; knob_int(Knob::HASH_BITS, b)) {
      return b > 0 && b <= 32 ? b : 0;
    }
    const int exact_passes = (key_bits + 7) / 8;
    const double span = (double)(pg.ts_max - pg.ts_min) + 1.0;
    const double per_w = std::min((double)n_ext, (double)n_ext * ((double)W + 1.0) / span);
    double best = exact_passes;
    int best_b = 0;
    for (int p = 1; p < exact_passes; p++) {
      const double e = per_w / std::ldexp(1.0, 8 * p);
      const double cost = p + 0.7 * e;
      if (cost < best) {
        best = cost;
        best_b = 8 * p;
      }
    }
    return best_b;
  }

  ~PatternEngine() override {
    if (ev_pg) (void)hipEventDestroy(ev_pg);
    if (ev_pt) (void)hipEventDestroy(ev_pt);
  }

  void push(const Staged& b) override {
    if (b.n <= 0) return;
    fin_sts32 = nullptr;
    fin_sts64 = nullptr;
    fin_rec = ScanRecs{};
    sort_push(b);
  }

  void sort_push(const Staged& b) {
    const int64_t n = b.n;
    if (n <= 0) return;
    const bool isA = b.stream == sA, isB = b.stream == sB;
    const int64_t n_ext = C + n;
    if (n_ext + (logical == 2 ? C : 0) > (int64_t)kRowMask)
      throw Error(SHD_E_CAPACITY, "pattern batch + carried partials exceed 2^28 rows");
    hipStream_t s = stream;
    SHD_HIP(hipEventRecord(ev0, s));
    stage_begin();
    const int slot = isA ? 0 : 1;
    const bool keyed = partitioned || implicit_key;
    const bool key64 = keyed && type_key64(key_type[slot]);
    d_pv.reserve(n_ext * 4);
    d_ts.reserve(n_ext * 4);
    if (keyed) {
      if (key64) d_k64.reserve(n_ext * 8);
      d_k32.reserve(n_ext * 4);
    }
    d_match.reserve(n_ext * 4);
    d_pst.reserve(n_ext + kCompactPad);
    agg.reserve();

    ExtRows x{};
    x.carry = carry_cs();
    x.batch = b.cs;
    x.C = C;
    x.seq0 = seq;
    x.carry_seq = carry[cur].seq.as<int64_t>();
    if (logical == 2) {
      carry[cur].reserve_b(C, typesB);
      x.half = carry[cur].colset_b(typesB, C);
      x.half_seq = carry[cur].bseq.as<int64_t>();
      d_mother.reserve(n_ext * 4);
    }

    PrepArgs pa{};
    pa.x = x;
    pa.es = dset();
    pa.f1 = dfilters(f1);
    pa.is_a = isA;
    pa.is_b = isB;
    pa.partitioned = keyed;
    pa.null_skip = partitioned;
    pa.key64 = key64;
    if (keyed) {
      if (key_expr[slot] >= 0) pa.key_expr = dexpr(key_expr[slot]);
      pa.key_col = key_col[slot];
      pa.key_type = key_type[slot];
    } else {
      pa.key_col = -1;
    }
    pa.carry_key = carry[cur].key.as<uint64_t>();
    PrepAgg init{0, 0, LLONG_MAX, LLONG_MIN, 0, 0, LLONG_MIN, ULLONG_MAX};
    PatternTotalsHost& h_agg = agg.host();
    PrepAgg* d_pa = &agg.dev()->prep;
    ScanOut* d_so = &agg.dev()->scan;
    h_agg.prep = init;
    h_agg.scan = ScanOut{};
    SHD_HIP(hipMemcpyAsync(agg.dev(), &h_agg, offsetof(PatternTotals, n_match), hipMemcpyHostToDevice, s));
    const int nblk = grid_for(n_ext, 1, 4096);
    d_blk.reserve((size_t)3 * nblk * std::max(sizeof(PrepAgg), sizeof(ScanOut)));
    const PrepArgs* d_pa_args = dev_args(pa);
    const bool fast1 = (!isA || pa.f1.fp.ok) && (!keyed || pa.key_col >= 0);
    const int fs_force = knob_force(Knob::FUSED_SORT);
    const int fattr = keyed_sort_f1_attr(pa.f1, isA);
    const bool fused = partitioned && !key64 && pa.key_col >= 0 && fattr >= -1 &&
                       (key_type[slot] == SHD_T_STRING || key_type[slot] == SHD_T_INT) && n_ext >= 2 &&
                       (fs_force >= 0 ? fs_force != 0 : n_ext >= ((int64_t)1 << 20));
    KsInfo* d_ksi = &agg.dev()->ks;
    int lean_mode = KS_LEAN_OFF;
    if (fused && !knob_on(Knob::NO_LEAN_SORT)) {
      int m = 0;
      const bool scan_lists = W != INT64_MAX && logical != 2 && !knob_on(Knob::TS64) &&
                              !knob_on(Knob::NO_RESUME_LIST) && !knob_on(Knob::NO_SCAN_LISTS) &&
                              knob_force(Knob::LOCKSTEP) <= 0 && (!knob_int(Knob::RESUME_MODE, m) || m == 0);
      lean_mode = knob_on(Knob::LEAN_SORT) ? KS_LEAN_ON : (scan_lists ? KS_LEAN_AUTO : KS_LEAN_OFF);
    }
    bool lean = false;
    if (fused) {
      if (!ev_pg) SHD_HIP(hipEventCreateWithFlags(&ev_pg, hipEventDisableTiming));
      if (!ev_pt) SHD_HIP(hipEventCreateWithFlags(&ev_pt, hipEventDisableTiming));
      keyed_sort_front(s, d_pa_args, pa, n_ext, d_kps, d_pa, d_ksi, lean_mode, W);
      agg.fetch(&PatternTotals::prep, s);
      if (lean_mode != KS_LEAN_OFF) {
        agg.fetch(&PatternTotals::ks, s);
        d_slice.reserve((size_t)2 * keyed_sort_slices(n_ext) * sizeof(int64_t));
      }
      SHD_HIP(hipEventRecord(ev_pg, s));
      keyed_sort_pass0(s, d_pa_args, pa, fattr, n_ext, d_kps, d_ksi, d_k32.as<uint32_t>(), d_pv.as<uint32_t>(),
                       d_ts.as<uint32_t>(), d_slice.as<int64_t>(), d_pa);
      SHD_HIP(hipMemcpyAsync(&h_agg.prep_pass0, d_pa, sizeof(PrepAgg), hipMemcpyDeviceToHost, s));
      SHD_HIP(hipEventRecord(ev_pt, s));
      SHD_HIP(hipEventSynchronize(ev_pg));
      lean = lean_mode != KS_LEAN_OFF && h_agg.ks.lean != 0;
    } else if (fast1)
      hipLaunchKernelGGL(k_prepare<true>, dim3(nblk), dim3(kBlock), 0, s, d_pa_args, n_ext, (int64_t)nblk * kBlock,
                         d_k32.as<uint32_t>(), d_k64.as<uint64_t>(), d_pv.as<uint32_t>(), d_ts.as<int32_t>(),
                         d_blk.as<PrepAgg>());
    else
      hipLaunchKernelGGL(k_prepare<false>, dim3(nblk), dim3(kBlock), 0, s, d_pa_args, n_ext, (int64_t)nblk * kBlock,
                         d_k32.as<uint32_t>(), d_k64.as<uint64_t>(), d_pv.as<uint32_t>(), d_ts.as<int32_t>(),
                         d_blk.as<PrepAgg>());
    if (!fused) {
      SHD_CHECK_LAUNCH();
      hipLaunchKernelGGL(k_finish_prep, dim3(1), dim3(kBlock), 0, s, (const PrepAgg*)d_blk.as<PrepAgg>(), nblk, d_pa);
      SHD_CHECK_LAUNCH();
      agg.fetch(&PatternTotals::prep, s);
      SHD_HIP(hipStreamSynchronize(s));
    }
    PrepAgg pg = h_agg.prep;
    mark("prepare");
    if (have_horizon && (int64_t)pg.ts_min < horizon)
      throw NeedNfa("pattern engine: an event precedes the retirement horizon of an earlier push");

    const uint32_t* skey32 = nullptr;
    const uint64_t* skey64 = nullptr;
    const uint32_t* spv = d_pv.as<uint32_t>();
    const int32_t* sts32 = d_ts.as<int32_t>();
    const int64_t* sts64 = nullptr;
    bool sorted64 = false;
    const bool prune = n_ext >= kPruneMinRows && W != INT64_MAX && !partitioned;
    const bool grouped = partitioned || (implicit_key && !pg.unmono && (C == 0 || pg.carry_tmax <= pg.ts_min));
    uint32_t hash_mask = 0;
    bool sorted_alt = false;
    counters.group_bits = 0;
    if (grouped) {
      const uint64_t kmin = pg.kmin <= pg.kmax ? pg.kmin : 0;
      uint64_t kmax = pg.kmax;
      int bits = 0;
      while (bits < 64 && (kmax >> bits)) bits++;
      uint32_t kbase = 0;
      if (bits <= 32 && !type_key64(key_type[slot])) {
        int rb = 0;
        while (rb < 64 && ((kmax - kmin) >> rb)) rb++;
        if (rb < bits) {
          bits = rb > 0 ? rb : 1;
          kbase = (uint32_t)kmin;
        }
      }
      bool in_alt = false;
      if (bits <= 32) {
        const int hb = hashed_bucket_bits(pg, n_ext, bits, prune && !partitioned);
        if (hb > 0) {
          bits = hb;
          hash_mask = hb >= 32 ? 0xFFFFFFFFu : ((1u << hb) - 1u);
        }
      }
      d_pv_alt.reserve(n_ext * 4);
      if (!lean) d_ts_alt.reserve(n_ext * 4);
      if (key64 && bits <= 32) {
        hipLaunchKernelGGL(k_narrow_keys, dim3(grid_for(n_ext)), dim3(kBlock), 0, s, d_k64.as<uint64_t>(),
                           d_k32.as<uint32_t>(), n_ext);
        SHD_CHECK_LAUNCH();
      }
      if (fused && (hash_mask || bits > 32))
        throw Error(SHD_E_DEVICE, "pattern engine: fused key sort on a hashed or wide key");
      if (bits <= 32) {
        d_k32_alt.reserve(n_ext * 4);
        if (fused)
          keyed_sort_rest(s, n_ext, bits, kbase, d_k32.as<uint32_t>(), d_pv.as<uint32_t>(), d_ts.as<uint32_t>(),
                          d_k32_alt.as<uint32_t>(), d_pv_alt.as<uint32_t>(), d_ts_alt.as<uint32_t>(), d_kps, d_sort,
                          in_alt, lean);
        else
          radix_sort_triples_u32(d_k32.as<uint32_t>(), d_pv.as<uint32_t>(), d_ts.as<uint32_t>(),
                                 d_k32_alt.as<uint32_t>(), d_pv_alt.as<uint32_t>(), d_ts_alt.as<uint32_t>(), n_ext,
                                 bits, d_sort, s, in_alt, hash_mask != 0, hash_mask ? 0u : kbase);
        skey32 = in_alt ? d_k32_alt.as<uint32_t>() : d_k32.as<uint32_t>();
      } else {
        d_k64_alt.reserve(n_ext * 8);
        radix_sort_triples_u64(d_k64.as<uint64_t>(), d_pv.as<uint32_t>(), d_ts.as<uint32_t>(),
                               d_k64_alt.as<uint64_t>(), d_pv_alt.as<uint32_t>(), d_ts_alt.as<uint32_t>(), n_ext,
                               bits, d_sort, s, in_alt);
        skey64 = in_alt ? d_k64_alt.as<uint64_t>() : d_k64.as<uint64_t>();
        sorted64 = true;
      }
      spv = in_alt ? d_pv_alt.as<uint32_t>() : d_pv.as<uint32_t>();
      sts32 = in_alt ? d_ts_alt.as<int32_t>() : d_ts.as<int32_t>();
      sorted_alt = in_alt;
      mark("key_sort");
      counters.group_bits = bits;
    }
    if (fused) {
      SHD_HIP(hipEventSynchronize(ev_pt));
      pg = h_agg.prep_pass0;
    }
    if (pg.ovf || knob_on(Knob::TS64)) {
      d_ts64.reserve(n_ext * 8);
      hipLaunchKernelGGL(k_sorted_ts64, dim3(grid_cover(n_ext)), dim3(kBlock), 0, s, dev_args(x), spv, n_ext,
                         d_ts64.as<int64_t>());
      SHD_CHECK_LAUNCH();
      sts64 = d_ts64.as<int64_t>();
    }

    ScanArgs sa{};
    sa.x = x;
    sa.es = dset();
    sa.f2 = dfilters(f2);
    sa.logical = logical;
    sa.s_first = s_first;
    sa.s_second = s_second;
    if (logical) sa.f3 = dfilters(f3);
    if (logical == 2) sa.carry_half = carry[cur].half.as<uint8_t>();
    sa.within = W;
    sa.partitioned = grouped;
    sa.prune = prune;
    sa.hash_mask = hash_mask;
    const int64_t t_end = (int64_t)pg.ts_max;
    sa.t_end = t_end;
    if (lean) {
      int cbits = kKsSliceBits;
      while (((n_ext - 1) >> cbits) >= kScanCoarse) cbits++;
      d_ctab.reserve((size_t)2 * kScanCoarse * sizeof(int32_t));
      sa.ctab = d_ctab.as<int32_t>();
      sa.cbits = cbits;
      sa.carry_tmax = (int64_t)pg.carry_tmax;
    }
    const bool fast2 = sa.f2.fp.ok != 0 && (!logical || sa.f3.fp.ok != 0);
    const int64_t tile = ceil_div(ceil_div(n_ext, nblk), kBlock) * kBlock;
    const int ntile = (int)ceil_div(n_ext, tile);
    const int nsub = ntile * kSubPerTile;
    d_bcnt.reserve(((size_t)3 * ntile + (size_t)3 * nsub) * 4);
    d_boff.reserve(((size_t)3 * ntile + (size_t)3 * nsub) * 4);
    uint32_t* d_scnt = d_bcnt.as<uint32_t>() + 3 * ntile;
    uint32_t* d_soff = d_boff.as<uint32_t>() + 3 * ntile;
    const bool ts64 = sts64 != nullptr;
    bool dense = !grouped;
    double e_key = 0.0;
    if (grouped) {
      const double span = (double)(pg.ts_max - pg.ts_min) + 1.0;
      const double per_w = W == INT64_MAX ? (double)n_ext : std::min((double)n_ext, (double)n_ext * ((double)W + 1.0) / span);
      const double nkeys = hash_mask ? (double)hash_mask + 1.0 : (double)(pg.kmax - std::min(pg.kmin, pg.kmax)) + 1.0;
      e_key = per_w / nkeys;
      dense = e_key >= 0.25;
    }
    int rmode = dense ? (hash_mask ? 1 : (logical != 2 ? 3 : (and_indep ? 2 : 1))) : 0;
    if (int m; knob_int(Knob::RESUME_MODE, m)) {
      if (m >= 0 && m <= 3 && !(m >= 2 && (hash_mask || (logical == 2 && (m == 3 || !and_indep))))) rmode = m;
    }
    const int ls_force = knob_force(Knob::LOCKSTEP);
    const bool lockstep = grouped && !hash_mask && !sorted64 && logical == 0 && isB && fast2 && e_key < 64.0 &&
                          (ls_force >= 0 ? ls_force != 0 : rmode == 3);
    if (grouped && (rmode != 0 || lockstep) && isB && bpos_mask && !knob_on(Knob::NO_BPOS) &&
        (e_key >= 8.0 || knob_on(Knob::BPOS))) {
      uint32_t apos = apos_mask & carry_mask;
      for (int c = 0; c < kMaxCols; c++)
        if (((apos >> c) & 1u) && (c >= b.cs.ncols || c >= (int)typesA.size() || typesA[c] != b.cs.type[c]))
          apos &= ~(1u << c);
      sa.x.bpos = b.cs;
      sa.x.bpos.n = n_ext;
      sa.x.apos_mask = apos;
      for (int c = 0; c < b.cs.ncols; c++) {
        if (!(((bpos_mask | apos) >> c) & 1u)) continue;
        d_bpos[c].reserve(n_ext * type_size(b.cs.type[c]));
        d_bpos_nul[c].reserve(n_ext);
        sa.x.bpos.col[c] = d_bpos[c].p;
        sa.x.bpos.nul[c] = d_bpos_nul[c].as<uint8_t>();
      }
      sa.x.bpos_mask = bpos_mask;
      hipLaunchKernelGGL(k_gather_bpos, dim3(grid_for(n_ext, 1, 4096)), dim3(kBlock), 0, s, dev_args(sa.x), spv, n_ext);
      SHD_CHECK_LAUNCH();
    }
    sa.sp = F2Split{};
    if (fast2 && logical == 0 && !knob_on(Knob::NO_SPLIT)) split_f2(sa.f2.fp, s_first, sa.x, sa.sp);
    sa.bsum = nullptr;
    const bool skip_ok = grouped && !hash_mask && !sorted64 && !ts64 && isB && logical == 0 && rmode != 0 && !lockstep &&
                         sa.f2.fp.ok && !knob_on(Knob::NO_BLOCK_SKIP) && (e_key >= 64.0 || knob_on(Knob::BLOCK_SKIP));
    if (skip_ok && block_skip_term(sa.f2.fp, s_first, sa.bs_ci, sa.bs_side, sa.bs_op, sa.bs_attr)) {
      d_bsum.reserve(ceil_div(n_ext, 64) * (int64_t)sizeof(BlockSum));
      sa.bsum = d_bsum.as<BlockSum>();
    }
    const ScanArgs* d_sa = dev_args(sa);
    const bool rlist = rmode == 0 && !lockstep && !sa.bsum && !sorted64 && !knob_on(Knob::NO_RESUME_LIST);
    const bool slists = rlist && grouped && !hash_mask && !ts64 && logical != 2 && !knob_on(Knob::NO_SCAN_LISTS);
    const bool lean_scan = lean && slists && !prune && W != INT64_MAX;
    if (lean && !lean_scan && !ts64) {
      d_ts.reserve(n_ext * 4);
      d_ts_alt.reserve(n_ext * 4);
      int32_t* ts_out = sorted_alt ? d_ts_alt.as<int32_t>() : d_ts.as<int32_t>();
      hipLaunchKernelGGL(k_sorted_ts32, dim3(grid_cover(n_ext)), dim3(kBlock), 0, s, dev_args(x), spv, n_ext, ts_out);
      SHD_CHECK_LAUNCH();
      sts32 = ts_out;
    }
    if (lean_scan) {
      sts32 = nullptr;
      hipLaunchKernelGGL(k_slice_coarsen, dim3(kScanCoarse / kBlock), dim3(kBlock), 0, s, dev_args(x),
                         (const int64_t*)d_slice.as<int64_t>(), keyed_sort_slices(n_ext), sa.cbits, d_ctab.as<int32_t>());
      SHD_CHECK_LAUNCH();
    }
    const int nlb = (int)std::max<int64_t>(1, std::min<int64_t>(1024, ceil_div(n_ext, (int64_t)64 * kBlock)));
    if (sa.bsum) {
      hipLaunchKernelGGL(k_block_sum, dim3(grid_for(ceil_div(n_ext, 64) * 64, 1, 4096)), dim3(kBlock), 0, s, d_sa,
                         n_ext, skey32, spv, sts32, d_bsum.as<BlockSum>());
      SHD_CHECK_LAUNCH();
    }
#define SHD_LAUNCH_SCAN(K64, TS64, H)                                                                           \
  hipLaunchKernelGGL((k_forward_scan<K64, TS64, H>), dim3(ntile), dim3(kBlock), 0, s, d_sa, n_ext, tile, skey32,    \
                     skey64, spv, sts32, sts64, d_match.as<int32_t>(), d_pst.as<uint8_t>(), d_bcnt.as<uint32_t>(), \
                     d_blk.as<ScanOut>())
#define SHD_LAUNCH_RESUME_D(K64, FAST, TS64, D, SLOT)                                                           \
  hipLaunchKernelGGL((k_forward_resume<K64, FAST, TS64, D>), dim3(ntile), dim3(kBlock), 0, s, d_sa, n_ext, tile, \
                     skey32, skey64, spv, sts32, sts64, d_match.as<int32_t>(), d_mother.as<int32_t>(),           \
                     d_pst.as<uint8_t>(), d_bcnt.as<uint32_t>(), d_blk.as<ScanOut>(), SLOT)
#define SHD_LAUNCH_RESUME(K64, FAST, TS64)                                                                      \
  do {                                                                                                          \
    if (rmode == 3) {                                                                                           \
      SHD_LAUNCH_RESUME_D(K64, FAST, TS64, 3, ntile);                                                           \
      SHD_CHECK_LAUNCH();                                                                                       \
      SHD_LAUNCH_RESUME_D(K64, FAST, TS64, 2, 2 * ntile);                                                       \
    } else if (rmode == 2) SHD_LAUNCH_RESUME_D(K64, FAST, TS64, 2, ntile);                                      \
    else if (rmode == 1) SHD_LAUNCH_RESUME_D(K64, FAST, TS64, 1, ntile);                                        \
    else SHD_LAUNCH_RESUME_D(K64, FAST, TS64, 0, ntile);                                                        \
  } while (0)
#define SHD_LAUNCH_RESUME2(K64, FAST) \
  if (ts64) SHD_LAUNCH_RESUME(K64, FAST, true); else SHD_LAUNCH_RESUME(K64, FAST, false)
#define SHD_LAUNCH_SKIP(D, SLOT)                                                                                 \
  hipLaunchKernelGGL((k_forward_resume<false, true, false, D, true>), dim3(ntile), dim3(kBlock), 0, s, d_sa, n_ext, \
                     tile, skey32, skey64, spv, sts32, sts64, d_match.as<int32_t>(), d_mother.as<int32_t>(),      \
                     d_pst.as<uint8_t>(), d_bcnt.as<uint32_t>(), d_blk.as<ScanOut>(), SLOT)
    if (sorted64) {
      if (ts64) SHD_LAUNCH_SCAN(true, true, false); else SHD_LAUNCH_SCAN(true, false, false);
      SHD_CHECK_LAUNCH();
      if (fast2) { SHD_LAUNCH_RESUME2(true, true); }
      else { SHD_LAUNCH_RESUME2(true, false); }
    } else {
      if (lockstep) {
        if (ts64)
          hipLaunchKernelGGL(k_lockstep_walk<true>, dim3(ntile), dim3(kBlock), 0, s, d_sa, n_ext, tile, skey32, spv,
                             sts32, sts64, d_match.as<int32_t>(), d_pst.as<uint8_t>(), d_bcnt.as<uint32_t>(),
                             d_blk.as<ScanOut>());
        else
          hipLaunchKernelGGL(k_lockstep_walk<false>, dim3(ntile), dim3(kBlock), 0, s, d_sa, n_ext, tile, skey32, spv,
                             sts32, sts64, d_match.as<int32_t>(), d_pst.as<uint8_t>(), d_bcnt.as<uint32_t>(),
                             d_blk.as<ScanOut>());
      } else if (hash_mask) {
        if (ts64) SHD_LAUNCH_SCAN(false, true, true); else SHD_LAUNCH_SCAN(false, false, true);
      } else if (slists) {
        fin_rec.on = true;
        fin_rec.key = sorted_alt ? d_k32.as<uint32_t>() : d_k32_alt.as<uint32_t>();
        fin_rec.pv = sorted_alt ? d_pv.as<uint32_t>() : d_pv_alt.as<uint32_t>();
        fin_rec.lean = lean_scan;
        fin_rec.ts = lean_scan ? nullptr : (sorted_alt ? d_ts.as<int32_t>() : d_ts_alt.as<int32_t>());
        d_olist.reserve((size_t)n_ext * 4);
        d_dlist.reserve((size_t)n_ext * 4);
        fin_rec.pos = d_olist.as<uint32_t>();
        fin_rec.sub = tile / kSubPerTile;
        fin_rec.nsub = nsub;
#define SHD_LAUNCH_SCAN_REC(LEAN)                                                                                  \
  hipLaunchKernelGGL(k_forward_scan_rec<LEAN>, dim3(ntile), dim3(kBlock), 0, s, d_sa, n_ext, tile, skey32, spv,    \
                     sts32, d_match.as<int32_t>(), d_pst.as<uint8_t>(), d_bcnt.as<uint32_t>(),                     \
                     d_blk.as<ScanOut>(), fin_rec.key, fin_rec.pv, fin_rec.ts, fin_rec.pos, d_dlist.as<uint32_t>(), \
                     d_scnt)
        if (lean_scan) SHD_LAUNCH_SCAN_REC(true); else SHD_LAUNCH_SCAN_REC(false);
#undef SHD_LAUNCH_SCAN_REC
      } else {
        if (ts64) SHD_LAUNCH_SCAN(false, true, false); else SHD_LAUNCH_SCAN(false, false, false);
      }
      SHD_CHECK_LAUNCH();
      if (lockstep) {
        if (ts64) SHD_LAUNCH_RESUME_D(false, true, true, 2, ntile);
        else SHD_LAUNCH_RESUME_D(false, true, false, 2, ntile);
      } else if (sa.bsum) {
        if (rmode == 3) {
          SHD_LAUNCH_SKIP(3, ntile);
          SHD_CHECK_LAUNCH();
          SHD_LAUNCH_SKIP(2, 2 * ntile);
        } else if (rmode == 2) SHD_LAUNCH_SKIP(2, ntile);
        else SHD_LAUNCH_SKIP(1, ntile);
      } else if (slists) {
        uint32_t* d_ndef = &agg.dev()->n_deferred;
        scan_exclusive_u32(d_scnt + nsub, d_soff + nsub, nsub, d_ndef, d_scan, s);
#define SHD_LAUNCH_RSUB(FAST, ROWT)                                                                                \
  hipLaunchKernelGGL((k_resume_list<false, FAST, false, true, ROWT>), dim3(nlb), dim3(kBlock), 0, s, d_sa, n_ext, tile, \
                     ntile, skey32, skey64, spv, sts32, sts64, d_match.as<int32_t>(), d_mother.as<int32_t>(),      \
                     d_pst.as<uint8_t>(), d_bcnt.as<uint32_t>(), d_blk.as<ScanOut>(), ntile,                       \
                     (const uint32_t*)d_dlist.as<uint32_t>(), (const uint32_t*)d_ndef,                             \
                     (const uint32_t*)(d_soff + nsub), nsub, fin_rec.sub, d_scnt)
        if (lean_scan) {
          if (fast2) SHD_LAUNCH_RSUB(true, true); else SHD_LAUNCH_RSUB(false, true);
        } else {
          if (fast2) SHD_LAUNCH_RSUB(true, false); else SHD_LAUNCH_RSUB(false, false);
        }
#undef SHD_LAUNCH_RSUB
      } else if (rlist) {
        uint32_t* d_ndef = &agg.dev()->n_deferred;
        scan_exclusive_u32(d_bcnt.as<uint32_t>() + 2 * ntile, d_boff.as<uint32_t>() + 2 * ntile, ntile, d_ndef, d_scan,
                           s);
        d_dlist.reserve((size_t)n_ext * 4);
        hipLaunchKernelGGL(k_open_list, dim3(ntile), dim3(kBlock), 0, s, (const uint8_t*)d_pst.as<uint8_t>(),
                           (const uint32_t*)d_boff.as<uint32_t>(), n_ext, tile, d_dlist.as<uint32_t>(),
                           (uint32_t)PS_DEFER, 2);
        SHD_CHECK_LAUNCH();
#define SHD_LAUNCH_RLIST(FAST, TS64)                                                                               \
  hipLaunchKernelGGL((k_resume_list<false, FAST, TS64>), dim3(nlb), dim3(kBlock), 0, s, d_sa, n_ext, tile, ntile,     \
                     skey32, skey64, spv, sts32, sts64, d_match.as<int32_t>(), d_mother.as<int32_t>(),              \
                     d_pst.as<uint8_t>(), d_bcnt.as<uint32_t>(), d_blk.as<ScanOut>(), ntile,                        \
                     (const uint32_t*)d_dlist.as<uint32_t>(), (const uint32_t*)d_ndef, (const uint32_t*)nullptr, 0,  \
                     (int64_t)0, (uint32_t*)nullptr)
        if (fast2) {
          if (ts64) SHD_LAUNCH_RLIST(true, true); else SHD_LAUNCH_RLIST(true, false);
        } else {
          if (ts64) SHD_LAUNCH_RLIST(false, true); else SHD_LAUNCH_RLIST(false, false);
        }
#undef SHD_LAUNCH_RLIST
      } else if (fast2) { SHD_LAUNCH_RESUME2(false, true); }
      else { SHD_LAUNCH_RESUME2(false, false); }
    }
#undef SHD_LAUNCH_RESUME2
#undef SHD_LAUNCH_SKIP
#undef SHD_LAUNCH_RESUME_D
#undef SHD_LAUNCH_RESUME
#undef SHD_LAUNCH_SCAN
    SHD_CHECK_LAUNCH();
    hipLaunchKernelGGL(k_finish_scan, dim3(1), dim3(kBlock), 0, s, (const ScanOut*)d_blk.as<ScanOut>(),
                       rlist ? ntile + nlb : (rmode == 3 && !lockstep ? 3 : 2) * ntile,
                       d_so);
    SHD_CHECK_LAUNCH();
    mark("forward_scan");

    scan_exclusive_u32(d_bcnt.as<uint32_t>(), d_boff.as<uint32_t>(), ntile, &agg.dev()->n_match, d_scan, s);
    if (slists)
      scan_exclusive_u32(d_scnt, d_soff, nsub, &agg.dev()->n_open, d_scan, s);
    else
      scan_exclusive_u32(d_bcnt.as<uint32_t>() + ntile, d_boff.as<uint32_t>() + ntile, ntile, &agg.dev()->n_open,
                         d_scan, s);
    mark("compact");
    agg.fetch(&PatternTotals::scan, &PatternTotals::tail_, s);
    SHD_HIP(hipMemcpyAsync(&h_agg.t_last, b.cs.ts + (n - 1), 8, hipMemcpyDeviceToHost, s));
    SHD_HIP(hipStreamSynchronize(s));
    const ScanOut so = h_agg.scan;
    const uint32_t m = h_agg.n_match;
    const uint32_t n_open = h_agg.n_open;
    if (so.violation)
      throw NeedNfa("pattern engine: event timestamps decrease within a key under `within`");
    if (so.pruned) {
      have_horizon = true;
      horizon = std::max(horizon, t_end);
    }
    fin_sts32 = sts32;
    fin_sts64 = sts64;
    finish(b, x, n_ext, tile, ntile, spv, skey32, skey64, sorted64, keyed, grouped, key64, m, n_open, so, t_end,
           pg.n_cand);
  }

  void finish(const Staged& b, const ExtRows& x, int64_t n_ext, int64_t tile, int ntile, const uint32_t* spv,
              const uint32_t* skey32, const uint64_t* skey64, bool sorted64, bool keyed, bool grouped, bool key64,
              uint32_t m, uint32_t n_open, const ScanOut& so, int64_t t_end, uint64_t n_cand) {
    hipStream_t s = stream;
    const int64_t n = b.n;
    if (m > 0) {
      d_pj.reserve((int64_t)m * 4);
      d_pi.reserve((int64_t)m * 4);
      d_pj_alt.reserve((int64_t)m * 4);
      d_pi_alt.reserve((int64_t)m * 4);
      if (logical == 2) {
        d_se1.reserve((int64_t)m * 4);
        d_sot.reserve((int64_t)m * 4);
      }
      hipLaunchKernelGGL(k_emit_pairs, dim3(ntile), dim3(kBlock), 0, s, (const uint8_t*)d_pst.as<uint8_t>(),
                         (const uint32_t*)d_boff.as<uint32_t>(), (const int32_t*)d_match.as<int32_t>(), spv, n_ext,
                         tile, logical, (const int32_t*)d_mother.as<int32_t>(), d_pj.as<uint32_t>(),
                         d_pi.as<uint32_t>(), d_se1.as<uint32_t>(), d_sot.as<int32_t>());
      SHD_CHECK_LAUNCH();
      int bits = 0;
      while (bits < 32 && ((uint64_t)n_ext >> bits)) bits++;
      if (logical) bits++;
      bool in_alt = false;
      radix_sort_pairs_u32(d_pj.as<uint32_t>(), d_pi.as<uint32_t>(), d_pj_alt.as<uint32_t>(),
                           d_pi_alt.as<uint32_t>(), m, bits, d_sort, s, in_alt);
      const uint32_t* pj = in_alt ? d_pj_alt.as<uint32_t>() : d_pj.as<uint32_t>();
      const uint32_t* pi = in_alt ? d_pi_alt.as<uint32_t>() : d_pi.as<uint32_t>();
      if (!gmembers.empty()) {
        group_emit(b, x, pj, pi, m);
        mark("order_project");
      } else {
        out.ensure(m, s);
        ProjArgs pr{};
        pr.x = x;
        pr.es = dset();
        pr.nout = (int)outs.size();
        pr.fast = 1;
        for (size_t c = 0; c < outs.size(); c++) {
          pr.outs[c] = dexpr(outs[c]);
          if (!fast_atom(outs[c], pr.oat[c])) pr.fast = 0;
        }
        pr.multi = (sA == sB);
        pr.logical = logical;
        pr.s_first = s_first;
        pr.s_second = s_second;
        pr.se1 = d_se1.as<uint32_t>();
        pr.sot = d_sot.as<int32_t>();
        pr.chunk0 = chunk_seq;
        pr.row0 = out.count;
        hipLaunchKernelGGL(k_project, dim3(grid_cover(m)), dim3(kBlock), 0, s, dev_args(pr), pj, pi, (int64_t)m,
                           out.d_chunk(), out.d_type(), out.d_ts(), out.d_vals(), out.d_nulls(), out.d_seq(),
                           out.d_sidx());
        SHD_CHECK_LAUNCH();
        out.count += m;
        if (sA != sB && !logical) chunk_seq += m;
        mark("order_project");
      }
    }

    int nxt = cur ^ 1;
    carry[nxt].reserve(n_open, typesA);
    if (n_open > 0) {
      GatherArgs ga{};
      ga.x = x;
      ga.ncols = (int)typesA.size();
      ga.partitioned = keyed;
      ga.key64 = sorted64;
      for (size_t c = 0; c < typesA.size(); c++) {
        ga.types[c] = (int32_t)typesA[c];
        ga.dcol[c] = carry[nxt].col[c].p;
        ga.dnul[c] = carry[nxt].nul[c].as<uint8_t>();
      }
      ga.dts = carry[nxt].ts.as<int64_t>();
      ga.dkey = carry[nxt].key.as<uint64_t>();
      ga.dseq = carry[nxt].seq.as<int64_t>();
      carry[cur].pend.reserve(std::max<int64_t>(C, 1));
      ga.dpend = carry[nxt].pend.as<uint8_t>();
      ga.pend_old = carry[cur].pend.as<uint8_t>();
      if (logical == 2) {
        carry[nxt].reserve_b(n_open, typesB);
        ga.and_mode = 1;
        ga.match_row = d_match.as<int32_t>();
        ga.dhalf = carry[nxt].half.as<uint8_t>();
        ga.ncolsB = (int)typesB.size();
        for (size_t c = 0; c < typesB.size(); c++) {
          ga.typesB[c] = (int32_t)typesB[c];
          ga.dcolB[c] = carry[nxt].bcol[c].p;
          ga.dnulB[c] = carry[nxt].bnul[c].as<uint8_t>();
        }
        ga.dtsB = carry[nxt].bts.as<int64_t>();
        ga.dseqB = carry[nxt].bseq.as<int64_t>();
      }
      if (keyed && !grouped) {
        ga.key64 = key64;
        skey32 = d_k32.as<uint32_t>();
        skey64 = d_k64.as<uint64_t>();
      }
      if (logical != 2) {
        ga.amask = carry_mask;
        if (grouped) {
          ga.sts32 = fin_sts32;
          ga.sts64 = fin_sts64;
          ga.key_attr = (partitioned && !sorted64 && key_col[0] >= 0 &&
                         (key_type[0] == SHD_T_STRING || key_type[0] == SHD_T_INT)) ? key_col[0] : -1;
        } else {
          ga.key_attr = -1;
        }
        if (fin_rec.on) {
#define SHD_LAUNCH_GATHER_REC(LEAN)                                                                               \
  hipLaunchKernelGGL(k_gather_rec<LEAN>, dim3(ntile), dim3(kBlock), 0, s, dev_args(ga), fin_rec.sub, fin_rec.nsub, \
                     (const uint32_t*)fin_rec.key, (const uint32_t*)fin_rec.pv, (const int32_t*)fin_rec.ts,        \
                     (const uint32_t*)fin_rec.pos, (const uint32_t*)(d_bcnt.as<uint32_t>() + 3 * ntile),           \
                     (const uint32_t*)(d_boff.as<uint32_t>() + 3 * ntile), (const uint8_t*)d_pst.as<uint8_t>())
          if (fin_rec.lean) SHD_LAUNCH_GATHER_REC(true); else SHD_LAUNCH_GATHER_REC(false);
#undef SHD_LAUNCH_GATHER_REC
        } else {
          d_olist.reserve((size_t)n_open * 4);
          hipLaunchKernelGGL(k_open_list, dim3(ntile), dim3(kBlock), 0, s, (const uint8_t*)d_pst.as<uint8_t>(),
                             (const uint32_t*)d_boff.as<uint32_t>(), n_ext, tile, d_olist.as<uint32_t>(),
                             (uint32_t)PS_OPEN, 1);
          SHD_CHECK_LAUNCH();
          hipLaunchKernelGGL(k_gather_list, dim3(grid_cover((int64_t)n_open)), dim3(kBlock), 0, s, dev_args(ga),
                             (const uint32_t*)d_olist.as<uint32_t>(), (int64_t)n_open,
                             (const uint8_t*)d_pst.as<uint8_t>(), spv, skey32, skey64);
        }
      } else {
        hipLaunchKernelGGL(k_gather_carry, dim3(ntile), dim3(kBlock), 0, s, dev_args(ga),
                           (const uint8_t*)d_pst.as<uint8_t>(), (const uint32_t*)d_boff.as<uint32_t>(), spv, skey32,
                           skey64, n_ext, tile);
      }
      SHD_CHECK_LAUNCH();
      mark("carry");
    }
    SHD_HIP(hipEventRecord(ev1, s));
    stage_end();
    SHD_HIP(hipEventSynchronize(ev1));
    float ms = 0.f;
    SHD_HIP(hipEventElapsedTime(&ms, ev0, ev1));
    cur = nxt;
    C = n_open;
    if (b.stream == sB) last_b_seq = seq + n - 1;
    seq += n;
    if (b.advance_time && t_end > now) now = t_end;
    t_last = agg.host().t_last;
    counters.events += n;
    counters.matches += m;
    counters.partial_scans += (int64_t)so.steps;
    counters.carry = C;
    counters.kernel_ns = (int64_t)(ms * 1e6);
    counters.partials += (int64_t)n_cand;
    for (PatternEngine* g : gmembers) {
      g->seq = seq;
      if (b.advance_time && t_end > g->now) g->now = t_end;
      g->counters.events += n;
      g->counters.kernel_ns = 0;
    }
  }

  std::vector<PatternEngine*> gmembers;
  DevBuf d_gmask, d_gcnt, d_goff, d_gscan, d_gpj, d_gpi, d_gbase;
  PinnedBuf h_gbase;

  static bool same_expr(const Plan& p, int e, const Plan& q, int f) {
    if (e < 0 || f < 0) return e == f;
    const auto& A = p.exprs[e];
    const auto& B = q.exprs[f];
    if (A.size() != B.size()) return false;
    for (size_t i = 0; i < A.size(); i++) {
      if (A[i].op != B[i].op || A[i].b != B[i].b || A[i].c != B[i].c) return false;
      if (A[i].op == SHD_OP_CONST ? p.consts[A[i].a] != q.consts[B[i].a] : A[i].a != B[i].a) return false;
    }
    return true;
  }

  void group_attach(const std::vector<Engine*>& ms) override {
    if (grouped) throw Error(SHD_E_ARG, "the leader already belongs to a group");
    if (ms.empty() || ms.size() > (size_t)kGroupMax) throw Error(SHD_E_ARG, "a group holds 1..64 member queries");
    if (logical != 0) throw Error(SHD_E_UNSUPPORTED, "query groups: logical patterns are not shared");
    if (counters.events != 0 || C != 0) throw Error(SHD_E_ARG, "the group leader must be fresh");
    std::vector<PatternEngine*> v;
    for (Engine* e : ms) {
      auto* m = dynamic_cast<PatternEngine*>(e);
      if (!m || m == this || m->grouped) throw Error(SHD_E_ARG, "group member: not a free pattern-engine query");
      for (PatternEngine* o : v)
        if (o == m) throw Error(SHD_E_ARG, "group member listed twice");
      bool ok = m->logical == 0 && m->sA == sA && m->sB == sB && m->W == W && m->partitioned == partitioned &&
                m->implicit_key == implicit_key && m->typesA == typesA && m->f2.size() == f2.size() &&
                m->plan.stream_types == plan.stream_types && (m->carry_mask & ~carry_mask) == 0;
      for (int k = 0; ok && k < 2; k++)
        ok = m->key_col[k] == key_col[k] && m->key_type[k] == key_type[k] &&
             same_expr(plan, key_expr[k], m->plan, m->key_expr[k]);
      for (size_t k = 0; ok && k < f2.size(); k++) ok = same_expr(plan, f2[k], m->plan, m->f2[k]);
      if (!ok)
        throw Error(SHD_E_ARG, "group member differs from the leader beyond the e1 filter and the selector");
      if (m->counters.events != 0 || m->C != 0 || m->out.count != 0)
        throw Error(SHD_E_ARG, "group members must be fresh (reset, no unpolled rows)");
      v.push_back(m);
    }
    gmembers = v;
    grouped = true;
    for (PatternEngine* m : gmembers) m->grouped = true;
  }

  void group_detach() override {
    for (PatternEngine* m : gmembers) m->grouped = false;
    gmembers.clear();
    grouped = false;
  }

  void group_emit(const Staged& b, const ExtRows& x, const uint32_t* pj, const uint32_t* pi, uint32_t m) {
    hipStream_t s = stream;
    const int G = (int)gmembers.size();
    if ((uint64_t)m * (uint64_t)G >= (1ull << 32))
      throw Error(SHD_E_CAPACITY, "query group: too many matches in one push for 32-bit pair lists (split the batch)");
    const int64_t per_wave = 64 * kGroupWaveItems;
    const int64_t nw = ((int64_t)m + per_wave - 1) / per_wave;
    GroupSelArgs ga{};
    ga.x = x;
    ga.G = G;
    for (int g = 0; g < G; g++) {
      ga.es[g] = gmembers[g]->dset();
      ga.f1[g] = gmembers[g]->dfilters(gmembers[g]->f1);
    }
    d_gmask.reserve((size_t)m * 8);
    d_gcnt.reserve((size_t)G * nw * 4);
    d_goff.reserve((size_t)G * nw * 4);
    d_gbase.reserve((size_t)(G + 1) * 4);
    h_gbase.reserve((size_t)(G + 1) * 4);
    hipLaunchKernelGGL(k_group_mask, dim3(grid_cover(m)), dim3(kBlock), 0, s, dev_args(ga), pi, (int64_t)m,
                       d_gmask.as<uint64_t>());
    SHD_CHECK_LAUNCH();
    const int split_blocks = (int)((nw * 64 + kBlock - 1) / kBlock);
    hipLaunchKernelGGL(k_group_split<false>, dim3(split_blocks), dim3(kBlock), 0, s,
                       (const uint64_t*)d_gmask.as<uint64_t>(), pj, pi, (int64_t)m, G, nw, d_gcnt.as<uint32_t>(),
                       (uint32_t*)nullptr, (uint32_t*)nullptr);
    SHD_CHECK_LAUNCH();
    scan_exclusive_u32(d_gcnt.as<uint32_t>(), d_goff.as<uint32_t>(), (int64_t)G * nw, nullptr, d_gscan, s);
    hipLaunchKernelGGL(k_group_bases, dim3(1), dim3(128), 0, s, (const uint32_t*)d_goff.as<uint32_t>(),
                       (const uint32_t*)d_gcnt.as<uint32_t>(), G, nw, d_gbase.as<uint32_t>());
    SHD_CHECK_LAUNCH();
    SHD_HIP(hipMemcpyAsync(h_gbase.p, d_gbase.p, (size_t)(G + 1) * 4, hipMemcpyDeviceToHost, s));
    SHD_HIP(hipStreamSynchronize(s));
    const uint32_t* base = h_gbase.as<uint32_t>();
    const uint32_t total = base[G];
    if (total == 0) return;
    d_gpj.reserve((size_t)total * 4);
    d_gpi.reserve((size_t)total * 4);
    hipLaunchKernelGGL(k_group_split<true>, dim3(split_blocks), dim3(kBlock), 0, s,
                       (const uint64_t*)d_gmask.as<uint64_t>(), pj, pi, (int64_t)m, G, nw, d_goff.as<uint32_t>(),
                       d_gpj.as<uint32_t>(), d_gpi.as<uint32_t>());
    SHD_CHECK_LAUNCH();
    for (int g = 0; g < G; g++) {
      PatternEngine& e = *gmembers[g];
      const uint32_t mq = base[g + 1] - base[g];
      if (mq == 0) continue;
      e.out.ensure(mq, s);
      ProjArgs pr{};
      pr.x = x;
      pr.es = e.dset();
      pr.nout = (int)e.outs.size();
      pr.fast = 1;
      for (size_t c = 0; c < e.outs.size(); c++) {
        pr.outs[c] = e.dexpr(e.outs[c]);
        if (!e.fast_atom(e.outs[c], pr.oat[c])) pr.fast = 0;
      }
      pr.multi = (sA == sB);
      pr.logical = 0;
      pr.s_first = e.s_first;
      pr.s_second = e.s_second;
      pr.chunk0 = e.chunk_seq;
      pr.row0 = e.out.count;
      hipLaunchKernelGGL(k_project, dim3(grid_cover(mq)), dim3(kBlock), 0, s, dev_args(pr),
                         (const uint32_t*)d_gpj.as<uint32_t>() + base[g], (const uint32_t*)d_gpi.as<uint32_t>() + base[g],
                         (int64_t)mq, e.out.d_chunk(), e.out.d_type(), e.out.d_ts(), e.out.d_vals(), e.out.d_nulls(),
                         e.out.d_seq(), e.out.d_sidx());
      SHD_CHECK_LAUNCH();
      e.out.count += mq;
      if (sA != sB) e.chunk_seq += mq;
      e.counters.matches += mq;
    }
    (void)b;
  }
};

std::unique_ptr<Engine> finish_pattern_engine(const Plan& p, const PNode& a, const PNode& b, const PNode* c,
                                              std::string& why);

std::unique_ptr<Engine> make_pattern_engine(const Plan& p, std::string& why) {
  if (p.kind != SHD_KIND_STATE || p.state_type != 0) { why = "not a pattern"; return nullptr; }
  const PNode& r = p.root;
  if (r.kind != SHD_NODE_NEXT || r.kids.size() != 2) { why = "not a two-state chain"; return nullptr; }
  const PNode& ev = r.kids[0];
  const PNode& b = r.kids[1];
  if (ev.kind != SHD_NODE_EVERY || ev.kids.size() != 1 || ev.kids[0].kind != SHD_NODE_STREAM ||
      b.kind != SHD_NODE_STREAM) {
    why = "not every e1 -> e2";
    return nullptr;
  }
  const PNode& a = ev.kids[0];
  if (a.absent || b.absent || a.state_id != 0 || b.state_id != 1) { why = "absent / unexpected state ids"; return nullptr; }
  return finish_pattern_engine(p, a, b, nullptr, why);
}

std::unique_ptr<Engine> make_logical_pattern_engine(const Plan& p, std::string& why) {
  if (p.kind != SHD_KIND_STATE || p.state_type != 0) { why = "not a pattern"; return nullptr; }
  const PNode& r = p.root;
  if (r.kind != SHD_NODE_NEXT || r.kids.size() != 2) { why = "not a two-state chain"; return nullptr; }
  const PNode& ev = r.kids[0];
  const PNode& lg = r.kids[1];
  if (ev.kind != SHD_NODE_EVERY || ev.kids.size() != 1 || ev.kids[0].kind != SHD_NODE_STREAM ||
      lg.kind != SHD_NODE_LOGICAL || (lg.ltype != 0 && lg.ltype != 1) || lg.kids.size() != 2) {
    why = "not every e1 -> (e2 or|and e3)";
    return nullptr;
  }
  const PNode& a = ev.kids[0];
  const PNode& b = lg.kids[0];
  const PNode& c = lg.kids[1];
  if (b.kind != SHD_NODE_STREAM || c.kind != SHD_NODE_STREAM || a.absent || b.absent || c.absent ||
      a.state_id != 0 || b.stream != c.stream) {
    why = "logical operands: absent / different streams";
    return nullptr;
  }
  return finish_pattern_engine(p, a, b, &c, why);
}

std::unique_ptr<Engine> finish_pattern_engine(const Plan& p, const PNode& a, const PNode& b, const PNode* c,
                                              std::string& why) {
  if (!p.aggs.empty() || !p.group_by.empty() || p.having >= 0) { why = "aggregating selector"; return nullptr; }
  if (!p.current_on) { why = "pattern without current events output"; return nullptr; }
  if (p.outputs.size() > (size_t)kMaxCols || a.filters.size() > 4 || b.filters.size() > 4 ||
      (c && c->filters.size() > 4)) {
    why = "too many outputs / filters";
    return nullptr;
  }
  for (int f : a.filters)
    if (!expr_reads_only(p, f, 0)) { why = "e1 filter reads other states"; return nullptr; }
  if (p.stream_types[a.stream].size() > (size_t)kMaxCols || p.stream_types[b.stream].size() > (size_t)kMaxCols) {
    why = "too many attributes";
    return nullptr;
  }
  auto e = std::make_unique<PatternEngine>();
  e->sA = a.stream;
  e->sB = b.stream;
  e->f1 = a.filters;
  e->f2 = b.filters;
  if (c) {
    e->logical = p.root.kids[1].ltype == 1 ? 1 : 2;
    e->f3 = c->filters;
    e->typesB = p.stream_types[b.stream];
    auto reads_only = [&](const std::vector<int>& fs, int own) {
      for (int f : fs)
        for (auto& in : p.exprs[f])
          if ((in.op == SHD_OP_LOAD || in.op == SHD_OP_EVNULL || in.op == SHD_OP_TS) && in.a != 0 && in.a != own)
            return false;
      return true;
    };
    e->and_indep = reads_only(b.filters, b.state_id) && reads_only(c->filters, c->state_id);
    e->s_first = b.state_id;
    e->s_second = c->state_id;
  }
  e->W = p.within >= 0 ? p.within : INT64_MAX;
  e->typesA = p.stream_types[a.stream];
  {
    auto scan = [&](const std::vector<int>& fs, int st) {
      for (int f : fs)
        for (auto& in : p.exprs[f])
          if (in.op == SHD_OP_LOAD && in.a == st && (in.c & 0xFFFF) < kMaxCols) e->bpos_mask |= 1u << (in.c & 0xFFFF);
    };
    scan(b.filters, b.state_id);
    if (c) scan(c->filters, c->state_id);
    for (const std::vector<int>* fs : {&b.filters, c ? &c->filters : nullptr})
      if (fs)
        for (int f : *fs)
          for (auto& in : p.exprs[f])
            if (in.op == SHD_OP_LOAD && in.a == 0 && (in.c & 0xFFFF) < kMaxCols) e->apos_mask |= 1u << (in.c & 0xFFFF);
  }
  for (auto& o : p.outputs) e->outs.push_back(o.second);
  e->partitioned = !p.part_keys.empty();
  if (!e->partitioned && !c && !knob_on(Knob::NO_IMPLICIT_KEY)) {
    int aa, ab, t;
    if (find_key_equality(p, b.filters, aa, ab, t) && (a.stream != b.stream || aa == ab)) {
      e->implicit_key = true;
      e->key_col[0] = aa;
      e->key_col[1] = ab;
      e->key_type[0] = e->key_type[1] = t;
    }
  }
  if (e->partitioned) {
    int cls = -1;
    for (auto& pk : p.part_keys) {
      int slot = pk.first == a.stream ? 0 : (pk.first == b.stream ? 1 : -1);
      if (slot < 0) continue;
      int t = expr_result_type(p, pk.second, {});
      if (cls >= 0 && t != cls) { why = "partition keys of different types"; return nullptr; }
      cls = t;
      e->key_expr[slot] = pk.second;
      e->key_col[slot] = plain_load_attr(p, pk.second);
      e->key_type[slot] = t;
      if (a.stream == b.stream) {
        e->key_expr[1 - slot] = pk.second;
        e->key_col[1 - slot] = e->key_col[slot];
        e->key_type[1 - slot] = t;
      }
    }
    if (e->key_expr[0] < 0 || e->key_expr[1] < 0) { why = "partition key missing for a stream"; return nullptr; }
  }
  uint32_t mask = 0;
  auto add = [&](int ex) {
    if (ex < 0) return;
    for (const Instr& in : p.exprs[ex])
      if (in.op == SHD_OP_LOAD && in.a == 0) mask |= 1u << (in.c & 0xFFFF);
  };
  for (int f : e->f1) add(f);
  for (int f : e->f2) add(f);
  for (int f : e->f3) add(f);
  for (int o : e->outs) add(o);
  add(e->key_expr[0]);
  add(e->key_expr[1]);
  e->carry_mask = mask;
  return e;
}

}
```

siddhi_amd/csrc/knobs.h:

```cpp
#pragma once
#include <cassert>
#include <cstdlib>

namespace shd {

#define SHD_KNOBS(X)                                                                                                  \
                                                                                                     \
  X(SYNC_CHECK, "SHD_SYNC_CHECK", FLAG, PROCESS, "synchronize after every kernel launch so a fault names its launch") \
  X(NO_FAST_PRED, "SHD_NO_FAST_PRED", FLAG, PUSH, "filters run on the expression interpreter, never pre-decoded")     \
  X(FORCE_NFA, "SHD_FORCE_NFA", FLAG, LOAD, "every state plan runs on the generic NFA engine")                        \
  X(NO_LOGICAL_SCAN, "SHD_NO_LOGICAL_SCAN", FLAG, LOAD, "`every e1 -> (e2 or/and e3)` runs on the generic NFA engine") \
  X(NO_ABSENT_SCAN, "SHD_NO_ABSENT_SCAN", FLAG, LOAD, "`every e1 -> not X for t` runs on the generic NFA engine")     \
                                                                                              \
  X(NO_HASH, "SHD_NO_HASH", FLAG, PUSH, "pattern: never sort by hashed buckets")                                      \
  X(HASH_BITS, "SHD_HASH_BITS", INT, PUSH, "pattern: sort by this many hashed-bucket bits (outside 1..32: none)")     \
  X(FUSED_SORT, "SHD_FUSED_SORT", TRISTATE, PUSH, "pattern: fused prepare + first sort pass off / on at any push size") \
  X(TS64, "SHD_TS64", FLAG, PUSH, "pattern: 64-bit sorted timestamps even when 32-bit offsets fit")                   \
  X(RESUME_MODE, "SHD_RESUME_MODE", INT, PUSH, "pattern: deferred-walk mode 0..3 (ignored where the mode cannot run)") \
  X(LOCKSTEP, "SHD_LOCKSTEP", TRISTATE, PUSH, "pattern: lockstep walks off / on wherever they can run")               \
  X(NO_BPOS, "SHD_NO_BPOS", FLAG, PUSH, "pattern: never copy e2 attributes into position order (wins over SHD_BPOS)") \
  X(BPOS, "SHD_BPOS", FLAG, PUSH, "pattern: position-major e2 attributes whenever walks are dense")                   \
  X(NO_SPLIT, "SHD_NO_SPLIT", FLAG, PUSH, "pattern: f2 through eval_fpred per step, not split per comparison")        \
  X(NO_BLOCK_SKIP, "SHD_NO_BLOCK_SKIP", FLAG, PUSH, "pattern: walks never skip 64-position blocks (wins over SHD_BLOCK_SKIP)") \
  X(BLOCK_SKIP, "SHD_BLOCK_SKIP", FLAG, PUSH, "pattern: block skipping at any key density")                           \
  X(NO_RESUME_LIST, "SHD_NO_RESUME_LIST", FLAG, PUSH, "pattern: sparse deferred walks without the compacted list")    \
  X(NO_SCAN_LISTS, "SHD_NO_SCAN_LISTS", FLAG, PUSH, "pattern: open and deferred lists by the list passes, not from the scan") \
  X(NO_IMPLICIT_KEY, "SHD_NO_IMPLICIT_KEY", FLAG, LOAD, "pattern: a key equality in f2 does not partition the plan")  \
  X(NO_LEAN_SORT, "SHD_NO_LEAN_SORT", FLAG, PUSH, "pattern: never the lean (two-word) key sort (wins over SHD_LEAN_SORT)") \
  X(LEAN_SORT, "SHD_LEAN_SORT", FLAG, PUSH, "pattern: the lean key sort wherever it can run, at any key density")     \
                                                                                                  \
  X(KS_GENERIC_F1, "SHD_KS_GENERIC_F1", FLAG, PUSH, "fused sort: f1 through eval_fpred per row, not pre-decoded")     \
                                                                                                  \
  X(NFA_DEBUG, "SHD_NFA_DEBUG", FLAG, LOAD, "NFA: print window-lane decisions (and phase clocks in the prof build)")  \
  X(NFA_CHUNK, "SHD_NFA_CHUNK", INT, PUSH, "NFA: window-lane chunk length in events (at least 1)")                    \
  X(NFA_HASH1_ZERO, "SHD_NFA_HASH1_ZERO", FLAG, PUSH, "NFA: zero the first window-lane state hash (forces the fallback)") \
  X(NFA_WINDOW, "SHD_NFA_WINDOW", TRISTATE, LOAD, "NFA: 0 turns window lanes off")                                    \
  X(NFA_LIST, "SHD_NFA_LIST", INT, LOAD, "NFA: pending-list capacity per key (> 0)")                                  \
  X(NFA_PARTIALS, "SHD_NFA_PARTIALS", INT, LOAD, "NFA: partial capacity per key (> 0)")                               \
  X(NFA_EVENTS, "SHD_NFA_EVENTS", INT, LOAD, "NFA: event capacity per key (> 0)")                                     \
  X(NFA_RECORDS, "SHD_NFA_RECORDS", INT, LOAD, "NFA: record capacity per key (> 0)")                                  \
  X(NFA_TIMERS, "SHD_NFA_TIMERS", INT, LOAD, "NFA: timer capacity per key (> 0)")                                     \
                                                                                               \
  X(DEBUG_ARGS, "SHD_DEBUG_ARGS", FLAG, PUSH, "filter: print k_filter's arguments and stop before the launch")        \
  X(WCHUNK, "SHD_WCHUNK", FLAG, PUSH, "windows: the chunked walk (opt-in)")                                           \
  X(NO_WCHUNK, "SHD_NO_WCHUNK", FLAG, PUSH, "windows: never the chunked walk (wins over SHD_WCHUNK)")                 \
  X(NO_CALLWIN, "SHD_NO_CALLWIN", FLAG, PUSH, "windows: never the call-window path")                                  \
  X(FOLD_LANE, "SHD_FOLD_LANE", FLAG, PUSH, "group fold: one lane per group at any segment length")                   \
  X(FOLD_GENERIC, "SHD_FOLD_GENERIC", FLAG, PUSH, "group fold: the generic fold, not the sum + count one")            \
  X(EXACT_AGGREGATES, "SHD_EXACT_AGGREGATES", FLAG, LOAD, "aggregates: the in-order running fold, not segmented scans") \
  X(GROUP_DICT, "SHD_GROUP_DICT", FLAG, LOAD, "group by: the group dictionary for every key, dense ids for none")

enum class Knob : int {
#define X(id, name, kind, when, doc) id,
  SHD_KNOBS(X)
#undef X
};

enum class KnobKind { FLAG, TRISTATE, INT };
enum class KnobWhen { PROCESS, LOAD, PUSH };

struct KnobInfo {
  const char* name;
  KnobKind kind;
  KnobWhen when;
  const char* doc;
};

inline constexpr KnobInfo kKnobs[] = {
#define X(id, name, kind, when, doc) {name, KnobKind::kind, KnobWhen::when, doc},
    SHD_KNOBS(X)
#undef X
};
inline constexpr int kNumKnobs = (int)(sizeof(kKnobs) / sizeof(kKnobs[0]));

inline const char* knob_value(Knob k, KnobKind kind) {
  const KnobInfo& info = kKnobs[(int)k];
  assert(info.kind == kind);
  (void)kind;
  const char* v = std::getenv(info.name);
  return v && *v ? v : nullptr;
}

inline bool knob_on(Knob k) {
  const char* v = knob_value(k, KnobKind::FLAG);
  return v && *v != '0';
}

inline int knob_force(Knob k) {
  const char* v = knob_value(k, KnobKind::TRISTATE);
  return !v ? -1 : *v == '0' ? 0 : 1;
}

inline bool knob_int(Knob k, int& out) {
  const char* v = knob_value(k, KnobKind::INT);
  if (v) out = std::atoi(v);
  return v != nullptr;
}

}
```

siddhi_amd/csrc/pattern_common.h:

```cpp
#pragma once
#include "engine.h"

namespace shd {
namespace pat {

enum : uint32_t { F_CAND = 1, F_NEW = 2, F_B = 4, F_SKIP = 8 };
enum : uint8_t { ST_NONE = 0, ST_OPEN = 1, ST_DEAD = 2, ST_MATCH = 3, ST_DEFER = 4, ST_PRUNED = 5, ST_YIELD = 6 };
enum : uint8_t { PS_NONE = 0, PS_OPEN = 1, PS_MATCH = 2, PS_DEFER = 3, PS_CONT = 4 };
constexpr uint8_t PS_PEND = 0x80;

constexpr int kRowBits = 28;
constexpr uint32_t kRowMask = (1u << kRowBits) - 1;
__device__ __forceinline__ uint32_t pv_row(uint32_t pv) { return pv & kRowMask; }
__device__ __forceinline__ uint32_t pv_flags(uint32_t pv) { return pv >> kRowBits; }

struct ExtRows {
  ColSet carry;
  ColSet batch;
  int64_t C;
  int64_t seq0;
  const int64_t* carry_seq;
  ColSet half;
  const int64_t* half_seq;
  ColSet bpos;
  uint32_t bpos_mask;
  uint32_t apos_mask;
  __device__ __forceinline__ const ColSet& cs(int64_t r) const { return r < C ? carry : (r < C + batch.n ? batch : half); }
  __device__ __forceinline__ int64_t row(int64_t r) const { return r < C ? r : (r < C + batch.n ? r - C : r - C - batch.n); }
  __device__ __forceinline__ int64_t ts(int64_t r) const {
#ifdef SHD_DEBUG
    if (r < 0 || r >= C + batch.n) {
      printf("SHD_DEBUG ExtRows.ts: row %lld C %lld n %lld\n", (long long)r, (long long)C, (long long)batch.n);
      return 0;
    }
#endif
    if (r < C) return gld(carry.ts, r);
    if (r < C + batch.n) return gld(batch.ts, r - C);
    return gld(half.ts, r - C - batch.n);
  }
  __device__ __forceinline__ int64_t seq(int64_t r) const {
    return r < C ? carry_seq[r] : (r < C + batch.n ? seq0 + (r - C) : half_seq[r - C - batch.n]);
  }
};

struct PairCtx {
  const ExtRows* x;
  int64_t r1, r2;
  int s2 = 1;
  bool matched = false;
  int64_t r3 = -1;
  int s3 = -1;
  int64_t q2 = -1;
  int64_t q1 = -1;
  __device__ __forceinline__ int64_t slot(int st, int idx) const {
    int64_t r = st == 0 ? r1 : (st == s2 ? r2 : (st == s3 ? r3 : -1));
    if (r < 0) return -1;
    return (idx == 0 || idx == SHD_IDX_CURRENT) ? r : -1;
  }
  __device__ __forceinline__ Val load(int st, int idx, int attr) const {
    int64_t r = slot(st, idx);
    if (r < 0) {
      Val v;
      v.b = 0;
      v.null = 1;
      return v;
    }
    if (st == s2 && q2 >= 0 && ((x->bpos_mask >> attr) & 1u)) return col_load(x->bpos, q2, attr);
    if (st == 0 && q1 >= 0 && ((x->apos_mask >> attr) & 1u)) return col_load(x->bpos, q1, attr);
    if (r < x->C) return col_load(x->carry, r, attr);
    if (r < x->C + x->batch.n) return col_load(x->batch, r - x->C, attr);
    return col_load(x->half, r - x->C - x->batch.n, attr);
  }
  __device__ __forceinline__ bool evnull(int st, int idx) const { return slot(st, idx) < 0; }
  __device__ __forceinline__ int64_t ts(int, int) const { return x->ts(matched ? r2 : r1); }
  __device__ __forceinline__ Val agg(int) const {
    Val v;
    v.b = 0;
    v.null = 1;
    return v;
  }
};

struct BlockSum {
  uint32_t key;
  uint16_t cnt;
  uint8_t flags, pad;
  int64_t tfirst, tlast;
  double v;
  uint64_t newmask;
};

struct SplitCmp {
  const void* col;
  const uint8_t* nul;
  int32_t ctype, pos, cvt_from, cvt_to;
  int32_t op, type;
  int32_t swap;
  int32_t konst;
  int32_t kind;
};
enum : int32_t { SK_GENERIC = 0, SK_F32_F64 = 1, SK_F64 = 2, SK_STR_EQ = 3, SK_I32 = 4 };
constexpr int kSplitMax = 3;
struct F2Split {
  int32_t ok, n;
  SplitCmp c[kSplitMax];
};

constexpr int kKsSliceBits = 10;
struct ScanArgs {
  ExtRows x;
  DExprSet es;
  DFilters f2;
  DFilters f3;
  int logical;
  int s_first, s_second;
  const uint8_t* carry_half;
  int64_t within;
  int partitioned;
  int prune;
  int64_t t_end;
  uint32_t hash_mask;
  const BlockSum* bsum;
  int bs_ci, bs_side, bs_op, bs_attr;
  F2Split sp;
  const int32_t* ctab;
  int cbits;
  int64_t carry_tmax;
};
constexpr int kScanCoarse = 2048;

struct ScanOut {
  unsigned long long steps;
  unsigned long long pruned;
  uint32_t violation;
};
struct BatchRowCtx {
  const ColSet* cs;
  int64_t row;
  __device__ __forceinline__ Val load(int st, int idx, int attr) const {
    if (st != 0 || !(idx == 0 || idx == SHD_IDX_CURRENT)) {
      Val v;
      v.b = 0;
      v.null = 1;
      return v;
    }
    return col_load(*cs, row, attr);
  }
  __device__ __forceinline__ bool evnull(int st, int idx) const { return !(st == 0 && (idx == 0 || idx == SHD_IDX_CURRENT)); }
  __device__ __forceinline__ int64_t ts(int st, int idx) const { return evnull(st, idx) ? 0 : cs->ts[row]; }
  __device__ __forceinline__ Val agg(int) const {
    Val v;
    v.b = 0;
    v.null = 1;
    return v;
  }
};

__device__ __forceinline__ uint64_t canon_key(Val v, int type) {
  switch (type) {
    case SHD_T_FLOAT: return p_f64((double)v_f32(v.b));
    default: return v.b;
  }
}

struct PrepAgg {
  unsigned long long n_cand;
  unsigned long long kmax;
  long long ts_min;
  long long ts_max;
  unsigned long long ovf;
  unsigned long long unmono;
  long long carry_tmax;
  unsigned long long kmin;
};

struct PrepArgs {
  ExtRows x;
  DExprSet es;
  DFilters f1;
  int is_a, is_b;
  int partitioned;
  int null_skip;
  int key64;
  DExpr key_expr;
  int key_type;
  int key_col;
  const uint64_t* carry_key;
};

template <class T>
__device__ __forceinline__ T wave_max(T v) {
  for (int o = 32; o > 0; o >>= 1) {
    T t = __shfl_xor(v, o, 64);
    v = t > v ? t : v;
  }
  return v;
}
template <class T>
__device__ __forceinline__ T wave_min(T v) {
  for (int o = 32; o > 0; o >>= 1) {
    T t = __shfl_xor(v, o, 64);
    v = t < v ? t : v;
  }
  return v;
}

struct PrepAcc {
  unsigned long long created = 0, kmax = 0, ovf = 0, unmono = 0, kmin = ULLONG_MAX;
  long long tmin = LLONG_MAX, tmax = LLONG_MIN, ctmax = LLONG_MIN;
};

template <bool FAST>
__device__ __forceinline__ void prep_row(const PrepArgs& a, const DExprSet& es, int64_t r, int64_t tbase,
                                         bool count, uint64_t& k, uint32_t& f, int32_t& tso, PrepAcc& acc) {
  const ExtRows& x = a.x;
  long long t;
  k = 0;
  if (r < x.C) {
    k = a.partitioned ? gld(a.carry_key, r) : 0;
    f = F_CAND;
    t = (long long)gld(x.carry.ts, r);
    if (count) acc.ctmax = t > acc.ctmax ? t : acc.ctmax;
  } else {
    const int64_t br = r - x.C;
    BatchRowCtx cx{&x.batch, br};
    t = (long long)gld(x.batch.ts, br);
    const long long tprev = br > 0 ? (long long)gld(x.batch.ts, br - 1) : t;
    Val kv;
    kv.b = 0;
    kv.null = 0;
    if (a.partitioned) {
      if (FAST || a.key_col >= 0) kv = col_load(x.batch, br, a.key_col);
      else kv = eval_expr(es.ins + a.key_expr.off, a.key_expr.len, es.consts, cx);
    }
    const bool p1 = a.is_a && (FAST ? eval_fpred(a.f1.fp, cx) : eval_filters(es, a.f1, cx));
    f = F_NEW;
    if (kv.null && a.null_skip) {
      f |= F_SKIP;
      k = (uint64_t)r;
    } else {
      if (a.is_b) f |= F_B;
      if (p1) {
        f |= F_CAND;
        acc.created += count ? 1u : 0u;
      }
      k = kv.null ? 0 : canon_key(kv, a.key_type);
    }
    if (count) {
      acc.tmin = t < acc.tmin ? t : acc.tmin;
      acc.tmax = t > acc.tmax ? t : acc.tmax;
      acc.unmono |= tprev > t;
    }
  }
  if (a.partitioned) {
    if (!a.key64) k = (uint32_t)k;
    if (count && !(f & F_SKIP)) {
      acc.kmax = k > acc.kmax ? k : acc.kmax;
      acc.kmin = k < acc.kmin ? k : acc.kmin;
    }
  }
  const int64_t dt = (int64_t)t - tbase;
  if (count) acc.ovf |= dt != (int64_t)(int32_t)dt;
  tso = (int32_t)dt;
}

template <int NT>
__device__ __forceinline__ void prep_block_reduce(PrepAcc acc, PrepAgg* blk, int slot) {
  for (int o = 32; o > 0; o >>= 1) {
    acc.created += __shfl_xor(acc.created, o, 64);
    acc.ovf |= __shfl_xor(acc.ovf, o, 64);
    acc.unmono |= __shfl_xor(acc.unmono, o, 64);
  }
  acc.kmax = wave_max(acc.kmax);
  acc.kmin = wave_min(acc.kmin);
  acc.tmin = wave_min(acc.tmin);
  acc.tmax = wave_max(acc.tmax);
  acc.ctmax = wave_max(acc.ctmax);
  __shared__ PrepAgg wpart[NT / 64];
  if ((threadIdx.x & 63) == 0)
    wpart[threadIdx.x >> 6] = PrepAgg{acc.created, acc.kmax, acc.tmin, acc.tmax, acc.ovf, acc.unmono, acc.ctmax, acc.kmin};
  __syncthreads();
  if (threadIdx.x == 0) {
    PrepAgg r = wpart[0];
    for (int w = 1; w < NT / 64; w++) {
      r.ovf |= wpart[w].ovf;
      r.unmono |= wpart[w].unmono;
      r.carry_tmax = wpart[w].carry_tmax > r.carry_tmax ? wpart[w].carry_tmax : r.carry_tmax;
      r.kmin = wpart[w].kmin < r.kmin ? wpart[w].kmin : r.kmin;
      r.n_cand += wpart[w].n_cand;
      r.kmax = wpart[w].kmax > r.kmax ? wpart[w].kmax : r.kmax;
      r.ts_min = wpart[w].ts_min < r.ts_min ? wpart[w].ts_min : r.ts_min;
      r.ts_max = wpart[w].ts_max > r.ts_max ? wpart[w].ts_max : r.ts_max;
    }
    blk[slot] = r;
  }
}

struct KsInfo {
  uint32_t kb;
  int32_t bits;
  int32_t lean;
  int32_t pad_;
};
enum : int { KS_LEAN_OFF = 0, KS_LEAN_AUTO = 1, KS_LEAN_ON = 2 };

struct PatternTotals {
  PrepAgg prep;
  ScanOut scan;
  char scan_pad_[64 - sizeof(ScanOut)];
  uint32_t n_match;
  uint32_t n_open;
  uint32_t tail_[2];
  char pad_[232 - 144];
  KsInfo ks;
  uint32_t n_deferred;
};
static_assert(offsetof(PatternTotals, prep) == 0 && offsetof(PatternTotals, scan) == 64 &&
                  offsetof(PatternTotals, n_match) == 128 && offsetof(PatternTotals, n_open) == 132 &&
                  offsetof(PatternTotals, tail_) + sizeof(uint32_t[2]) == 64 + 80 &&
                  offsetof(PatternTotals, ks) == 232 && offsetof(PatternTotals, n_deferred) == 248 &&
                  sizeof(PatternTotals) <= 256,
              "PatternTotals device layout");
struct PatternTotalsHost : PatternTotals {
  int64_t t_last;
  PrepAgg prep_pass0;
};

int keyed_sort_f1_attr(const DFilters& f1, bool is_a);
void keyed_sort_front(hipStream_t s, const PrepArgs* d_pa, const PrepArgs& pa, int64_t n_ext, DevBuf& scratch,
                      PrepAgg* d_pg, KsInfo* d_info, int lean_mode, int64_t within);
int64_t keyed_sort_slices(int64_t n_ext);
void keyed_sort_pass0(hipStream_t s, const PrepArgs* d_pa, const PrepArgs& pa, int fattr, int64_t n_ext,
                      DevBuf& scratch, const KsInfo* d_info, uint32_t* k32, uint32_t* pv, uint32_t* ts,
                      int64_t* slice_t, PrepAgg* d_pg);
void keyed_sort_rest(hipStream_t s, int64_t n_ext, int bits, uint32_t kb, uint32_t* k32, uint32_t* pv, uint32_t* ts,
                     uint32_t* k32_alt, uint32_t* pv_alt, uint32_t* ts_alt, DevBuf& scratch, DevBuf& sort_scratch,
                     bool& in_alt, bool lean);

}
}
```

Measured before the change: 25.06 billion events/s.

## Defer lean-scan walks to resume list, batch arg uploads, overlap carry gather

The lean forward scan no longer walks undecided candidates from their rows. It defers them, packing the coarse time table into a 16-bit span, and a new HOT resume-list variant walks them starting at the next row; the old behaviour is kept behind a knob. The last-timestamp readback now rides in the totals struct, written by k_finish_scan, which removes a separate D2H copy. The carry gather is launched before the host waits on the scan totals, and several kernel-argument uploads are staged into one batched copy. Together these aim to cut per-batch host syncs and small copies and to shorten scan work. The cost is more code paths, and saturated spans become 'unknown' and fall back to full walks.

```diff
diff --git a/siddhi_amd/csrc/engine.h b/siddhi_amd/csrc/engine.h
--- a/siddhi_amd/csrc/engine.h
+++ b/siddhi_amd/csrc/engine.h
@@ -175,6 +175,23 @@
     }
     SHD_HIP(hipStreamSynchronize(stream));
     arg_used = 0;
+    arg_staged = kNoneStaged;
+  }
+  static constexpr size_t kNoneStaged = ~size_t(0);
+  size_t arg_staged = kNoneStaged;
+  template <class T> const T* args_stage(const T& a) {
+    size_t off = (arg_used + 255) & ~size_t(255);
+    if (!arg_dev.p || off + sizeof(T) > kArgArena) throw Error(SHD_E_CAPACITY, "kernel argument arena exhausted");
+    std::memcpy(arg_host.as<char>() + off, &a, sizeof(T));
+    if (arg_staged == kNoneStaged) arg_staged = off;
+    arg_used = off + sizeof(T);
+    return reinterpret_cast<const T*>(arg_dev.as<char>() + off);
+  }
+  void args_send() {
+    if (arg_staged == kNoneStaged) return;
+    SHD_HIP(hipMemcpyAsync(arg_dev.as<char>() + arg_staged, arg_host.as<char>() + arg_staged, arg_used - arg_staged,
+                           hipMemcpyHostToDevice, stream));
+    arg_staged = kNoneStaged;
   }
   template <class T> const T* dev_args(const T& a) {
     size_t off = (arg_used + 255) & ~size_t(255);
diff --git a/siddhi_amd/csrc/engine_pattern.hip b/siddhi_amd/csrc/engine_pattern.hip
--- a/siddhi_amd/csrc/engine_pattern.hip
+++ b/siddhi_amd/csrc/engine_pattern.hip
@@ -245,7 +245,7 @@
   __builtin_amdgcn_wave_barrier();
   __builtin_amdgcn_fence(__ATOMIC_ACQUIRE, "wavefront");
 }
-template <bool LEAN>
+template <bool LEAN, bool ROWW = false>
 __global__ __launch_bounds__(kBlock) void k_forward_scan_rec(const ScanArgs* __restrict__ ap, int64_t n_ext,
                                                              int64_t tile, const uint32_t* __restrict__ skey32,
                                                              const uint32_t* __restrict__ spv,
@@ -268,12 +268,20 @@
   const int64_t tbase = a.x.batch.ts[0];
   const GlobalPos<false, false> ld{skey32, nullptr, spv, sts32, nullptr, tbase, a.partitioned};
   const RowPos ldr{skey32, spv, a.x.carry.ts, a.x.batch.ts, a.x.C, a.partitioned};
-  __shared__ int32_t ctab[LEAN ? 2 * kScanCoarse : 1];
+  constexpr bool PACKED = LEAN && !ROWW;
+  __shared__ int32_t ctab[LEAN ? (PACKED ? 1 : 2) * kScanCoarse : 1];
+  __shared__ uint16_t cspan[PACKED ? kScanCoarse : 1];
   if constexpr (LEAN) {
     const int nc = (int)((n_ext - 1) >> a.cbits) + 1;
     for (int i = threadIdx.x; i < nc; i += kBlock) {
-      ctab[i] = a.ctab[i];
-      ctab[kScanCoarse + i] = a.ctab[kScanCoarse + i];
+      const int32_t lo = a.ctab[i], hi = a.ctab[kScanCoarse + i];
+      ctab[i] = lo;
+      if constexpr (PACKED) {
+        const int64_t sp = (int64_t)hi - (int64_t)lo;
+        cspan[i] = (uint16_t)(sp < 0 || sp > 0xFFFF ? 0xFFFF : sp);
+      } else {
+        ctab[kScanCoarse + i] = hi;
+      }
     }
     __syncthreads();
   }
@@ -329,18 +337,30 @@
           } else {
             bool dead = false;
             if (kq == k && (fq & F_NEW) && !(fq & F_SKIP)) {
-              const int64_t hi = ri >= a.x.C ? tbase + ctab[kScanCoarse + (ri >> a.cbits)] : a.carry_tmax;
+              int64_t hi;
+              bool known = true;
+              if (ri < a.x.C) {
+                hi = a.carry_tmax;
+              } else if constexpr (PACKED) {
+                const uint32_t sp = cspan[ri >> a.cbits];
+                known = sp != 0xFFFFu;
+                hi = tbase + ctab[ri >> a.cbits] + (int64_t)sp;
+              } else {
+                hi = tbase + ctab[kScanCoarse + (ri >> a.cbits)];
+              }
               const int64_t lo = tbase + ctab[rq >> a.cbits];
-              dead = lo > hi && (uint64_t)lo - (uint64_t)hi > (uint64_t)a.within;
+              dead = known && lo > hi && (uint64_t)lo - (uint64_t)hi > (uint64_t)a.within;
             }
             if (dead) {
               st = ST_DEAD;
               steps++;
-            } else {
+            } else if constexpr (ROWW) {
               tsi = ldr.row_ts(ri);
               tq = ldr.row_ts(rq);
               st = walk_partial<true, false, 1>(a, es, n_ext, ldr, ri, k, tsi, q, pq, tq, kq, tsi, false, j, steps,
                                                 viol, fm, ra, rb);
+            } else {
+              st = ST_DEFER;
             }
           }
         } else {
@@ -349,7 +369,7 @@
         }
         if (st == ST_DEFER) {
           out = PS_DEFER;
-          match_row[p] = (int32_t)q;
+          if constexpr (!PACKED) match_row[p] = (int32_t)q;
           nd++;
         } else if (st == ST_OPEN) {
           out = PS_OPEN;
@@ -842,7 +862,7 @@
   scan_block_reduce(steps, pruned, viol, nm, no, blk, slot0 + blockIdx.x, bcnt, blockIdx.x, gridDim.x, true);
 }
 
-template <bool K64, bool FAST, bool TS64, bool SUB = false, bool ROWT = false>
+template <bool K64, bool FAST, bool TS64, bool SUB = false, bool ROWT = false, bool HOT = false>
 __global__ __launch_bounds__(kBlock) void k_resume_list(const ScanArgs* __restrict__ ap, int64_t n_ext, int64_t tile,
                                                         int ntile, const uint32_t* __restrict__ skey32,
                                                         const uint64_t* __restrict__ skey64,
@@ -881,7 +901,7 @@
     } else {
       p = dlist[i];
     }
-    int64_t q = match_row[p];
+    int64_t q = HOT ? p + 1 : (int64_t)match_row[p];
     uint32_t pvp, pq;
     int64_t tsi, tq;
     uint64_t k = 0, kq = 0;
@@ -891,8 +911,16 @@
     uint32_t fm = 0;
     int64_t ra = -1, rb = -1;
     if (a.logical == 2) and_carried(a, pv_row(pvp), fm, ra, rb);
-    const uint8_t st = walk_partial<false, FAST, 1, Ld, 0, false>(
-        a, es, n_ext, ld, pv_row(pvp), k, tsi, q, pq, tq, kq, tq, true, j, steps, viol, fm, ra, rb, p);
+    uint8_t st = ST_DEFER;
+    if constexpr (HOT) {
+      st = walk_partial<true, false, 1>(a, es, n_ext, ld, pv_row(pvp), k, tsi, q, pq, tq, kq, tsi, false, j, steps,
+                                        viol, fm, ra, rb);
+      if (st == ST_DEFER && q != p + 1) ld(q, pq, tq, kq);
+    }
+    const bool met_b = st == ST_DEFER;
+    if (met_b)
+      st = walk_partial<false, FAST, 1, Ld, 0, false>(a, es, n_ext, ld, pv_row(pvp), k, tsi, q, pq, tq, kq, tq, true, j,
+                                                      steps, viol, fm, ra, rb, p);
     uint8_t out = PS_NONE;
     const int t = (int)(p / tile);
     if (st == ST_MATCH) {
@@ -901,7 +929,7 @@
       if (a.logical == 2) match_other[p] = (int32_t)((j >> kRowBits) ? ra : rb);
       atomicAdd(&bcnt[t], 1u);
     } else if (st == ST_OPEN) {
-      out = PS_OPEN | PS_PEND;
+      out = met_b ? (PS_OPEN | PS_PEND) : PS_OPEN;
       if (a.logical == 2) match_row[p] = and_code(fm, ra, rb);
       if (SUB) atomicAdd(&sopen[sti], 1u);
       else atomicAdd(&bcnt[ntile + t], 1u);
@@ -1090,7 +1118,8 @@
   }
 }
 
-__global__ __launch_bounds__(kBlock) void k_finish_scan(const ScanOut* blk, int nblk, ScanOut* out) {
+__global__ __launch_bounds__(kBlock) void k_finish_scan(const ScanOut* blk, int nblk, ScanOut* out,
+                                                        const int64_t* ts_last, long long* t_last) {
   unsigned long long st = 0, pr = 0;
   uint32_t v = 0;
 #pragma unroll 8
@@ -1115,6 +1144,7 @@
       r.violation |= wpart[w].violation;
     }
     *out = r;
+    *t_last = (long long)*ts_last;
   }
 }
 
@@ -1633,6 +1663,8 @@
   DevBuf d_slice;
   DevBuf d_ctab;
   hipEvent_t ev_pg = nullptr, ev_pt = nullptr;
+  hipEvent_t ev_scan = nullptr;
+  const ProjArgs* d_proj = nullptr;
   const int32_t* fin_sts32 = nullptr;
   const int64_t* fin_sts64 = nullptr;
   struct ScanRecs {
@@ -1838,6 +1870,7 @@
   ~PatternEngine() override {
     if (ev_pg) (void)hipEventDestroy(ev_pg);
     if (ev_pt) (void)hipEventDestroy(ev_pt);
+    if (ev_scan) (void)hipEventDestroy(ev_scan);
   }
 
   void push(const Staged& b) override {
@@ -1907,7 +1940,6 @@
     ScanOut* d_so = &agg.dev()->scan;
     h_agg.prep = init;
     h_agg.scan = ScanOut{};
-    SHD_HIP(hipMemcpyAsync(agg.dev(), &h_agg, offsetof(PatternTotals, n_match), hipMemcpyHostToDevice, s));
     const int nblk = grid_for(n_ext, 1, 4096);
     d_blk.reserve((size_t)3 * nblk * std::max(sizeof(PrepAgg), sizeof(ScanOut)));
     const PrepArgs* d_pa_args = dev_args(pa);
@@ -1917,6 +1949,8 @@
     const bool fused = partitioned && !key64 && pa.key_col >= 0 && fattr >= -1 &&
                        (key_type[slot] == SHD_T_STRING || key_type[slot] == SHD_T_INT) && n_ext >= 2 &&
                        (fs_force >= 0 ? fs_force != 0 : n_ext >= ((int64_t)1 << 20));
+    if (!fused)
+      SHD_HIP(hipMemcpyAsync(agg.dev(), &h_agg, offsetof(PatternTotals, n_match), hipMemcpyHostToDevice, s));
     KsInfo* d_ksi = &agg.dev()->ks;
     int lean_mode = KS_LEAN_OFF;
     if (fused && !knob_on(Knob::NO_LEAN_SORT)) {
@@ -2123,17 +2157,18 @@
     const bool rlist = rmode == 0 && !lockstep && !sa.bsum && !sorted64 && !knob_on(Knob::NO_RESUME_LIST);
     const bool slists = rlist && grouped && !hash_mask && !ts64 && logical != 2 && !knob_on(Knob::NO_SCAN_LISTS);
     const bool lean_scan = lean && slists && !prune && W != INT64_MAX;
+    const bool row_walk = knob_on(Knob::SCAN_ROW_WALK);
     if (lean && !lean_scan && !ts64) {
       d_ts.reserve(n_ext * 4);
       d_ts_alt.reserve(n_ext * 4);
       int32_t* ts_out = sorted_alt ? d_ts_alt.as<int32_t>() : d_ts.as<int32_t>();
-      hipLaunchKernelGGL(k_sorted_ts32, dim3(grid_cover(n_ext)), dim3(kBlock), 0, s, dev_args(x), spv, n_ext, ts_out);
+      hipLaunchKernelGGL(k_sorted_ts32, dim3(grid_cover(n_ext)), dim3(kBlock), 0, s, &d_sa->x, spv, n_ext, ts_out);
       SHD_CHECK_LAUNCH();
       sts32 = ts_out;
     }
     if (lean_scan) {
       sts32 = nullptr;
-      hipLaunchKernelGGL(k_slice_coarsen, dim3(kScanCoarse / kBlock), dim3(kBlock), 0, s, dev_args(x),
+      hipLaunchKernelGGL(k_slice_coarsen, dim3(kScanCoarse / kBlock), dim3(kBlock), 0, s, &d_sa->x,
                          (const int64_t*)d_slice.as<int64_t>(), keyed_sort_slices(n_ext), sa.cbits, d_ctab.as<int32_t>());
       SHD_CHECK_LAUNCH();
     }
@@ -2195,12 +2230,15 @@
         fin_rec.pos = d_olist.as<uint32_t>();
         fin_rec.sub = tile / kSubPerTile;
         fin_rec.nsub = nsub;
+#define SHD_ARG(...) __VA_ARGS__
 #define SHD_LAUNCH_SCAN_REC(LEAN)                                                                                  \
-  hipLaunchKernelGGL(k_forward_scan_rec<LEAN>, dim3(ntile), dim3(kBlock), 0, s, d_sa, n_ext, tile, skey32, spv,    \
+  hipLaunchKernelGGL((k_forward_scan_rec<LEAN>), dim3(ntile), dim3(kBlock), 0, s, d_sa, n_ext, tile, skey32, spv,  \
                      sts32, d_match.as<int32_t>(), d_pst.as<uint8_t>(), d_bcnt.as<uint32_t>(),                     \
                      d_blk.as<ScanOut>(), fin_rec.key, fin_rec.pv, fin_rec.ts, fin_rec.pos, d_dlist.as<uint32_t>(), \
                      d_scnt)
-        if (lean_scan) SHD_LAUNCH_SCAN_REC(true); else SHD_LAUNCH_SCAN_REC(false);
+        if (lean_scan && row_walk) SHD_LAUNCH_SCAN_REC(SHD_ARG(true, true));
+        else if (lean_scan) SHD_LAUNCH_SCAN_REC(SHD_ARG(true, false));
+        else SHD_LAUNCH_SCAN_REC(false);
 #undef SHD_LAUNCH_SCAN_REC
       } else {
         if (ts64) SHD_LAUNCH_SCAN(false, true, false); else SHD_LAUNCH_SCAN(false, false, false);
@@ -2219,18 +2257,21 @@
       } else if (slists) {
         uint32_t* d_ndef = &agg.dev()->n_deferred;
         scan_exclusive_u32(d_scnt + nsub, d_soff + nsub, nsub, d_ndef, d_scan, s);
-#define SHD_LAUNCH_RSUB(FAST, ROWT)                                                                                \
-  hipLaunchKernelGGL((k_resume_list<false, FAST, false, true, ROWT>), dim3(nlb), dim3(kBlock), 0, s, d_sa, n_ext, tile, \
+#define SHD_LAUNCH_RSUB(FAST, ROWT, HOT)                                                                           \
+  hipLaunchKernelGGL((k_resume_list<false, FAST, false, true, ROWT, HOT>), dim3(nlb), dim3(kBlock), 0, s, d_sa, n_ext, tile, \
                      ntile, skey32, skey64, spv, sts32, sts64, d_match.as<int32_t>(), d_mother.as<int32_t>(),      \
                      d_pst.as<uint8_t>(), d_bcnt.as<uint32_t>(), d_blk.as<ScanOut>(), ntile,                       \
                      (const uint32_t*)d_dlist.as<uint32_t>(), (const uint32_t*)d_ndef,                             \
                      (const uint32_t*)(d_soff + nsub), nsub, fin_rec.sub, d_scnt)
-        if (lean_scan) {
-          if (fast2) SHD_LAUNCH_RSUB(true, true); else SHD_LAUNCH_RSUB(false, true);
+        if (lean_scan && !row_walk) {
+          if (fast2) SHD_LAUNCH_RSUB(true, true, true); else SHD_LAUNCH_RSUB(false, true, true);
+        } else if (lean_scan) {
+          if (fast2) SHD_LAUNCH_RSUB(true, true, false); else SHD_LAUNCH_RSUB(false, true, false);
         } else {
-          if (fast2) SHD_LAUNCH_RSUB(true, false); else SHD_LAUNCH_RSUB(false, false);
+          if (fast2) SHD_LAUNCH_RSUB(true, false, false); else SHD_LAUNCH_RSUB(false, false, false);
         }
 #undef SHD_LAUNCH_RSUB
+#undef SHD_ARG
       } else if (rlist) {
         uint32_t* d_ndef = &agg.dev()->n_deferred;
         scan_exclusive_u32(d_bcnt.as<uint32_t>() + 2 * ntile, d_boff.as<uint32_t>() + 2 * ntile, ntile, d_ndef, d_scan,
@@ -2263,7 +2304,7 @@
     SHD_CHECK_LAUNCH();
     hipLaunchKernelGGL(k_finish_scan, dim3(1), dim3(kBlock), 0, s, (const ScanOut*)d_blk.as<ScanOut>(),
                        rlist ? ntile + nlb : (rmode == 3 && !lockstep ? 3 : 2) * ntile,
-                       d_so);
+                       d_so, (const int64_t*)(b.cs.ts + (n - 1)), &agg.dev()->t_last);
     SHD_CHECK_LAUNCH();
     mark("forward_scan");
 
@@ -2274,9 +2315,18 @@
       scan_exclusive_u32(d_bcnt.as<uint32_t>() + ntile, d_boff.as<uint32_t>() + ntile, ntile, &agg.dev()->n_open,
                          d_scan, s);
     mark("compact");
-    agg.fetch(&PatternTotals::scan, &PatternTotals::tail_, s);
-    SHD_HIP(hipMemcpyAsync(&h_agg.t_last, b.cs.ts + (n - 1), 8, hipMemcpyDeviceToHost, s));
-    SHD_HIP(hipStreamSynchronize(s));
+    agg.fetch(&PatternTotals::scan, &PatternTotals::t_last, s);
+    fin_sts32 = sts32;
+    fin_sts64 = sts64;
+    if (fin_rec.on) {
+      if (!ev_scan) SHD_HIP(hipEventCreateWithFlags(&ev_scan, hipEventDisableTiming));
+      SHD_HIP(hipEventRecord(ev_scan, s));
+      const int64_t bound = std::min<int64_t>(C + (int64_t)pg.n_cand, n_ext);
+      gather_open(b, x, n_ext, tile, ntile, spv, skey32, skey64, sorted64, keyed, grouped, key64, bound, true);
+      SHD_HIP(hipEventSynchronize(ev_scan));
+    } else {
+      SHD_HIP(hipStreamSynchronize(s));
+    }
     const ScanOut so = h_agg.scan;
     const uint32_t m = h_agg.n_match;
     const uint32_t n_open = h_agg.n_open;
@@ -2286,10 +2336,129 @@
       have_horizon = true;
       horizon = std::max(horizon, t_end);
     }
-    fin_sts32 = sts32;
-    fin_sts64 = sts64;
     finish(b, x, n_ext, tile, ntile, spv, skey32, skey64, sorted64, keyed, grouped, key64, m, n_open, so, t_end,
            pg.n_cand);
+  }
+
+  ProjArgs proj_args(const ExtRows& x) {
+    ProjArgs pr{};
+    pr.x = x;
+    pr.es = dset();
+    pr.nout = (int)outs.size();
+    pr.fast = 1;
+    for (size_t c = 0; c < outs.size(); c++) {
+      pr.outs[c] = dexpr(outs[c]);
+      if (!fast_atom(outs[c], pr.oat[c])) pr.fast = 0;
+    }
+    pr.multi = (sA == sB);
+    pr.logical = logical;
+    pr.s_first = s_first;
+    pr.s_second = s_second;
+    pr.se1 = d_se1.as<uint32_t>();
+    pr.sot = d_sot.as<int32_t>();
+    pr.chunk0 = chunk_seq;
+    pr.row0 = out.count;
+    return pr;
+  }
+
+  const GatherArgs* d_gather = nullptr;
+  const uint32_t* gather_k32 = nullptr;
+  const uint64_t* gather_k64 = nullptr;
+  void gather_open(const Staged& b, const ExtRows& x, int64_t n_ext, int64_t tile, int ntile, const uint32_t* spv,
+                   const uint32_t* skey32, const uint64_t* skey64, bool sorted64, bool keyed, bool grouped, bool key64,
+                   int64_t rows, bool early) {
+    const int nxt = cur ^ 1;
+    carry[nxt].reserve(rows, typesA);
+    d_gather = nullptr;
+    if (rows > 0) {
+      GatherArgs ga{};
+      ga.x = x;
+      ga.ncols = (int)typesA.size();
+      ga.partitioned = keyed;
+      ga.key64 = sorted64;
+      for (size_t c = 0; c < typesA.size(); c++) {
+        ga.types[c] = (int32_t)typesA[c];
+        ga.dcol[c] = carry[nxt].col[c].p;
+        ga.dnul[c] = carry[nxt].nul[c].as<uint8_t>();
+      }
+      ga.dts = carry[nxt].ts.as<int64_t>();
+      ga.dkey = carry[nxt].key.as<uint64_t>();
+      ga.dseq = carry[nxt].seq.as<int64_t>();
+      carry[cur].pend.reserve(std::max<int64_t>(C, 1));
+      ga.dpend = carry[nxt].pend.as<uint8_t>();
+      ga.pend_old = carry[cur].pend.as<uint8_t>();
+      if (logical == 2) {
+        carry[nxt].reserve_b(rows, typesB);
+        ga.and_mode = 1;
+        ga.match_row = d_match.as<int32_t>();
+        ga.dhalf = carry[nxt].half.as<uint8_t>();
+        ga.ncolsB = (int)typesB.size();
+        for (size_t c = 0; c < typesB.size(); c++) {
+          ga.typesB[c] = (int32_t)typesB[c];
+          ga.dcolB[c] = carry[nxt].bcol[c].p;
+          ga.dnulB[c] = carry[nxt].bnul[c].as<uint8_t>();
+        }
+        ga.dtsB = carry[nxt].bts.as<int64_t>();
+        ga.dseqB = carry[nxt].bseq.as<int64_t>();
+      }
+      if (keyed && !grouped) {
+        ga.key64 = key64;
+        skey32 = d_k32.as<uint32_t>();
+        skey64 = d_k64.as<uint64_t>();
+      }
+      gather_k32 = skey32;
+      gather_k64 = skey64;
+      if (logical != 2) {
+        ga.amask = carry_mask;
+        if (grouped) {
+          ga.sts32 = fin_sts32;
+          ga.sts64 = fin_sts64;
+          ga.key_attr = (partitioned && !sorted64 && key_col[0] >= 0 &&
+                         (key_type[0] == SHD_T_STRING || key_type[0] == SHD_T_INT)) ? key_col[0] : -1;
+        } else {
+          ga.key_attr = -1;
+        }
+        if (!fin_rec.on) d_olist.reserve((size_t)rows * 4);
+      }
+      d_gather = args_stage(ga);
+    }
+    if (early) d_proj = gmembers.empty() ? args_stage(proj_args(x)) : nullptr;
+    args_send();
+    if (early && rows > 0) {
+      launch_gather(n_ext, tile, ntile, spv, skey32, skey64, rows);
+      mark("carry");
+    }
+  }
+
+  void launch_gather(int64_t n_ext, int64_t tile, int ntile, const uint32_t* spv, const uint32_t*, const uint64_t*,
+                     int64_t n_open) {
+    hipStream_t s = stream;
+    const uint32_t* skey32 = gather_k32;
+    const uint64_t* skey64 = gather_k64;
+    if (logical != 2) {
+      if (fin_rec.on) {
+#define SHD_LAUNCH_GATHER_REC(LEAN)                                                                               \
+  hipLaunchKernelGGL(k_gather_rec<LEAN>, dim3(ntile), dim3(kBlock), 0, s, d_gather, fin_rec.sub, fin_rec.nsub,     \
+                     (const uint32_t*)fin_rec.key, (const uint32_t*)fin_rec.pv, (const int32_t*)fin_rec.ts,        \
+                     (const uint32_t*)fin_rec.pos, (const uint32_t*)(d_bcnt.as<uint32_t>() + 3 * ntile),           \
+                     (const uint32_t*)(d_boff.as<uint32_t>() + 3 * ntile), (const uint8_t*)d_pst.as<uint8_t>())
+        if (fin_rec.lean) SHD_LAUNCH_GATHER_REC(true); else SHD_LAUNCH_GATHER_REC(false);
+#undef SHD_LAUNCH_GATHER_REC
+      } else {
+        hipLaunchKernelGGL(k_open_list, dim3(ntile), dim3(kBlock), 0, s, (const uint8_t*)d_pst.as<uint8_t>(),
+                           (const uint32_t*)d_boff.as<uint32_t>(), n_ext, tile, d_olist.as<uint32_t>(),
+                           (uint32_t)PS_OPEN, 1);
+        SHD_CHECK_LAUNCH();
+        hipLaunchKernelGGL(k_gather_list, dim3(grid_cover(n_open)), dim3(kBlock), 0, s, d_gather,
+                           (const uint32_t*)d_olist.as<uint32_t>(), n_open, (const uint8_t*)d_pst.as<uint8_t>(), spv,
+                           skey32, skey64);
+      }
+    } else {
+      hipLaunchKernelGGL(k_gather_carry, dim3(ntile), dim3(kBlock), 0, s, d_gather,
+                         (const uint8_t*)d_pst.as<uint8_t>(), (const uint32_t*)d_boff.as<uint32_t>(), spv, skey32,
+                         skey64, n_ext, tile);
+    }
+    SHD_CHECK_LAUNCH();
   }
 
   void finish(const Staged& b, const ExtRows& x, int64_t n_ext, int64_t tile, int ntile, const uint32_t* spv,
@@ -2297,6 +2466,7 @@
               uint32_t m, uint32_t n_open, const ScanOut& so, int64_t t_end, uint64_t n_cand) {
     hipStream_t s = stream;
     const int64_t n = b.n;
+    const bool gathered = fin_rec.on;
     if (m > 0) {
       d_pj.reserve((int64_t)m * 4);
       d_pi.reserve((int64_t)m * 4);
@@ -2306,6 +2476,13 @@
         d_se1.reserve((int64_t)m * 4);
         d_sot.reserve((int64_t)m * 4);
       }
+    }
+    if (!gathered) {
+      d_proj = nullptr;
+      if (m > 0 && gmembers.empty()) d_proj = args_stage(proj_args(x));
+      gather_open(b, x, n_ext, tile, ntile, spv, skey32, skey64, sorted64, keyed, grouped, key64, n_open, false);
+    }
+    if (m > 0) {
       hipLaunchKernelGGL(k_emit_pairs, dim3(ntile), dim3(kBlock), 0, s, (const uint8_t*)d_pst.as<uint8_t>(),
                          (const uint32_t*)d_boff.as<uint32_t>(), (const int32_t*)d_match.as<int32_t>(), spv, n_ext,
                          tile, logical, (const int32_t*)d_mother.as<int32_t>(), d_pj.as<uint32_t>(),
@@ -2324,24 +2501,7 @@
         mark("order_project");
       } else {
         out.ensure(m, s);
-        ProjArgs pr{};
-        pr.x = x;
-        pr.es = dset();
-        pr.nout = (int)outs.size();
-        pr.fast = 1;
-        for (size_t c = 0; c < outs.size(); c++) {
-          pr.outs[c] = dexpr(outs[c]);
-          if (!fast_atom(outs[c], pr.oat[c])) pr.fast = 0;
-        }
-        pr.multi = (sA == sB);
-        pr.logical = logical;
-        pr.s_first = s_first;
-        pr.s_second = s_second;
-        pr.se1 = d_se1.as<uint32_t>();
-        pr.sot = d_sot.as<int32_t>();
-        pr.chunk0 = chunk_seq;
-        pr.row0 = out.count;
-        hipLaunchKernelGGL(k_project, dim3(grid_cover(m)), dim3(kBlock), 0, s, dev_args(pr), pj, pi, (int64_t)m,
+        hipLaunchKernelGGL(k_project, dim3(grid_cover(m)), dim3(kBlock), 0, s, d_proj, pj, pi, (int64_t)m,
                            out.d_chunk(), out.d_type(), out.d_ts(), out.d_vals(), out.d_nulls(), out.d_seq(),
                            out.d_sidx());
         SHD_CHECK_LAUNCH();
@@ -2351,78 +2511,9 @@
       }
     }
 
-    int nxt = cur ^ 1;
-    carry[nxt].reserve(n_open, typesA);
-    if (n_open > 0) {
-      GatherArgs ga{};
-      ga.x = x;
-      ga.ncols = (int)typesA.size();
-      ga.partitioned = keyed;
-      ga.key64 = sorted64;
-      for (size_t c = 0; c < typesA.size(); c++) {
-        ga.types[c] = (int32_t)typesA[c];
-        ga.dcol[c] = carry[nxt].col[c].p;
-        ga.dnul[c] = carry[nxt].nul[c].as<uint8_t>();
-      }
-      ga.dts = carry[nxt].ts.as<int64_t>();
-      ga.dkey = carry[nxt].key.as<uint64_t>();
-      ga.dseq = carry[nxt].seq.as<int64_t>();
-      carry[cur].pend.reserve(std::max<int64_t>(C, 1));
-      ga.dpend = carry[nxt].pend.as<uint8_t>();
-      ga.pend_old = carry[cur].pend.as<uint8_t>();
-      if (logical == 2) {
-        carry[nxt].reserve_b(n_open, typesB);
-        ga.and_mode = 1;
-        ga.match_row = d_match.as<int32_t>();
-        ga.dhalf = carry[nxt].half.as<uint8_t>();
-        ga.ncolsB = (int)typesB.size();
-        for (size_t c = 0; c < typesB.size(); c++) {
-          ga.typesB[c] = (int32_t)typesB[c];
-          ga.dcolB[c] = carry[nxt].bcol[c].p;
-          ga.dnulB[c] = carry[nxt].bnul[c].as<uint8_t>();
-        }
-        ga.dtsB = carry[nxt].bts.as<int64_t>();
-        ga.dseqB = carry[nxt].bseq.as<int64_t>();
-      }
-      if (keyed && !grouped) {
-        ga.key64 = key64;
-        skey32 = d_k32.as<uint32_t>();
-        skey64 = d_k64.as<uint64_t>();
-      }
-      if (logical != 2) {
-        ga.amask = carry_mask;
-        if (grouped) {
-          ga.sts32 = fin_sts32;
-          ga.sts64 = fin_sts64;
-          ga.key_attr = (partitioned && !sorted64 && key_col[0] >= 0 &&
-                         (key_type[0] == SHD_T_STRING || key_type[0] == SHD_T_INT)) ? key_col[0] : -1;
-        } else {
-          ga.key_attr = -1;
-        }
-        if (fin_rec.on) {
-#define SHD_LAUNCH_GATHER_REC(LEAN)                                                                               \
-  hipLaunchKernelGGL(k_gather_rec<LEAN>, dim3(ntile), dim3(kBlock), 0, s, dev_args(ga), fin_rec.sub, fin_rec.nsub, \
-                     (const uint32_t*)fin_rec.key, (const uint32_t*)fin_rec.pv, (const int32_t*)fin_rec.ts,        \
-                     (const uint32_t*)fin_rec.pos, (const uint32_t*)(d_bcnt.as<uint32_t>() + 3 * ntile),           \
-                     (const uint32_t*)(d_boff.as<uint32_t>() + 3 * ntile), (const uint8_t*)d_pst.as<uint8_t>())
-          if (fin_rec.lean) SHD_LAUNCH_GATHER_REC(true); else SHD_LAUNCH_GATHER_REC(false);
-#undef SHD_LAUNCH_GATHER_REC
-        } else {
-          d_olist.reserve((size_t)n_open * 4);
-          hipLaunchKernelGGL(k_open_list, dim3(ntile), dim3(kBlock), 0, s, (const uint8_t*)d_pst.as<uint8_t>(),
-                             (const uint32_t*)d_boff.as<uint32_t>(), n_ext, tile, d_olist.as<uint32_t>(),
-                             (uint32_t)PS_OPEN, 1);
-          SHD_CHECK_LAUNCH();
-          hipLaunchKernelGGL(k_gather_list, dim3(grid_cover((int64_t)n_open)), dim3(kBlock), 0, s, dev_args(ga),
-                             (const uint32_t*)d_olist.as<uint32_t>(), (int64_t)n_open,
-                             (const uint8_t*)d_pst.as<uint8_t>(), spv, skey32, skey64);
-        }
-      } else {
-        hipLaunchKernelGGL(k_gather_carry, dim3(ntile), dim3(kBlock), 0, s, dev_args(ga),
-                           (const uint8_t*)d_pst.as<uint8_t>(), (const uint32_t*)d_boff.as<uint32_t>(), spv, skey32,
-                           skey64, n_ext, tile);
-      }
-      SHD_CHECK_LAUNCH();
+    const int nxt = cur ^ 1;
+    if (!gathered && n_open > 0) {
+      launch_gather(n_ext, tile, ntile, spv, skey32, skey64, n_open);
       mark("carry");
     }
     SHD_HIP(hipEventRecord(ev1, s));
diff --git a/siddhi_amd/csrc/knobs.h b/siddhi_amd/csrc/knobs.h
--- a/siddhi_amd/csrc/knobs.h
+++ b/siddhi_amd/csrc/knobs.h
@@ -28,6 +28,7 @@
   X(NO_IMPLICIT_KEY, "SHD_NO_IMPLICIT_KEY", FLAG, LOAD, "pattern: a key equality in f2 does not partition the plan")  \
   X(NO_LEAN_SORT, "SHD_NO_LEAN_SORT", FLAG, PUSH, "pattern: never the lean (two-word) key sort (wins over SHD_LEAN_SORT)") \
   X(LEAN_SORT, "SHD_LEAN_SORT", FLAG, PUSH, "pattern: the lean key sort wherever it can run, at any key density")     \
+  X(SCAN_ROW_WALK, "SHD_SCAN_ROW_WALK", FLAG, PUSH, "pattern: the lean scan walks its undecided candidates itself, from their rows") \
                                                                                                   \
   X(KS_GENERIC_F1, "SHD_KS_GENERIC_F1", FLAG, PUSH, "fused sort: f1 through eval_fpred per row, not pre-decoded")     \
                                                                                                   \
diff --git a/siddhi_amd/csrc/pattern_common.h b/siddhi_amd/csrc/pattern_common.h
--- a/siddhi_amd/csrc/pattern_common.h
+++ b/siddhi_amd/csrc/pattern_common.h
@@ -310,19 +310,18 @@
   char scan_pad_[64 - sizeof(ScanOut)];
   uint32_t n_match;
   uint32_t n_open;
-  uint32_t tail_[2];
+  long long t_last;
   char pad_[232 - 144];
   KsInfo ks;
   uint32_t n_deferred;
 };
 static_assert(offsetof(PatternTotals, prep) == 0 && offsetof(PatternTotals, scan) == 64 &&
                   offsetof(PatternTotals, n_match) == 128 && offsetof(PatternTotals, n_open) == 132 &&
-                  offsetof(PatternTotals, tail_) + sizeof(uint32_t[2]) == 64 + 80 &&
+                  offsetof(PatternTotals, t_last) + sizeof(long long) == 64 + 80 &&
                   offsetof(PatternTotals, ks) == 232 && offsetof(PatternTotals, n_deferred) == 248 &&
                   sizeof(PatternTotals) <= 256,
               "PatternTotals device layout");
 struct PatternTotalsHost : PatternTotals {
-  int64_t t_last;
   PrepAgg prep_pass0;
 };
 
```

Result: faster. 26.79 billion events/s, median of 6 (+6.9%).
